# zju3dv/street_gaussians

Measured on AMD Instinct MI355X. Metric: train iters/s (fwd+bwd) @1M Gaussians 1920x1280 SH3, higher is better.
Workload: dtype f32

## Files before the change

### include/sgr.h

```cpp
#ifndef SGR_H_INCLUDED
#define SGR_H_INCLUDED

#include <stddef.h>
#include <stdint.h>

#ifdef __cplusplus
extern "C" {
#endif

#define SGR_E_INVALID 1
#define SGR_E_HIP 2
#define SGR_E_ALLOC 3
#define SGR_E_PREFILTER 4
#define SGR_E_LAZY 5

typedef char* (*sgr_alloc_fn)(size_t nbytes, void* user);

const char* sgr_last_error(void);
int sgr_version(void);

int sgr_forward(sgr_alloc_fn geometry_buffer, void* geometry_user, sgr_alloc_fn binning_buffer, void* binning_user,
                sgr_alloc_fn image_buffer, void* image_user, int P, int D, int M, int S, const float* background,
                int width, int height, const float* means3D, const float* shs, const float* colors_precomp,
                const float* semantics, const float* opacities, const float* scales, float scale_modifier,
                const float* rotations, const float* cov3D_precomp, const float* viewmatrix, const float* projmatrix,
                const float* cam_pos, float tan_fovx, float tan_fovy, int prefiltered, float* out_color,
                float* out_depth, float* out_alpha, float* out_semantic, int* radii, int debug, void* stream);

typedef struct sgr_forward_extras {
    int color_jacobian;
} sgr_forward_extras;
int sgr_forward_ex(sgr_alloc_fn geometry_buffer, void* geometry_user, sgr_alloc_fn binning_buffer, void* binning_user,
                   sgr_alloc_fn image_buffer, void* image_user, int P, int D, int M, int S, const float* background,
                   int width, int height, const float* means3D, const float* shs, const float* colors_precomp,
                   const float* semantics, const float* opacities, const float* scales, float scale_modifier,
                   const float* rotations, const float* cov3D_precomp, const float* viewmatrix, const float* projmatrix,
                   const float* cam_pos, float tan_fovx, float tan_fovy, int prefiltered, float* out_color,
                   float* out_depth, float* out_alpha, float* out_semantic, int* radii, int debug, void* stream,
                   const sgr_forward_extras* extras);

int sgr_backward(int P, int D, int M, int R, int S, const float* background, int width, int height,
                 const float* means3D, const float* shs, const float* colors_precomp, const float* semantics,
                 const float* alphas, const float* scales, float scale_modifier, const float* rotations,
                 const float* cov3D_precomp, const float* viewmatrix, const float* projmatrix, const float* campos,
                 float tan_fovx, float tan_fovy, const int* radii, char* geom_buffer, char* binning_buffer,
                 char* image_buffer, const float* dL_dpix, const float* dL_dpix_depth, const float* dL_dalphas,
                 const float* dL_dpix_semantic, float* dL_dmean2D, float* dL_dopacity, float* dL_dcolor,
                 float* dL_dmean3D, float* dL_dcov3D, float* dL_dsh, float* dL_dscale, float* dL_drot,
                 float* dL_dsemantic, sgr_alloc_fn scratch, void* scratch_user, int debug, void* stream);

#define SGR_MAX_STAT_SEGMENTS 128
typedef struct sgr_stat_segment {
    int src_start;
    int count;
    int dst_offset;
} sgr_stat_segment;
typedef struct sgr_backward_extras {
    float* xyz_gradient_accum;
    float* denom;
    float* max_radii2D;
    const sgr_stat_segment* segments;
    int n_segments;
    void* color_ready_event;
    int rows;
    float* masked_color_out;
    int skip_sh_grad;
    int skip_cov3d_grad;
} sgr_backward_extras;
int sgr_backward_ex(int P, int D, int M, int R, int S, const float* background, int width, int height,
                    const float* means3D, const float* shs, const float* colors_precomp, const float* semantics,
                    const float* alphas, const float* scales, float scale_modifier, const float* rotations,
                    const float* cov3D_precomp, const float* viewmatrix, const float* projmatrix, const float* campos,
                    float tan_fovx, float tan_fovy, const int* radii, char* geom_buffer, char* binning_buffer,
                    char* image_buffer, const float* dL_dpix, const float* dL_dpix_depth, const float* dL_dalphas,
                    const float* dL_dpix_semantic, float* dL_dmean2D, float* dL_dopacity, float* dL_dcolor,
                    float* dL_dmean3D, float* dL_dcov3D, float* dL_dsh, float* dL_dscale, float* dL_drot,
                    float* dL_dsemantic, sgr_alloc_fn scratch, void* scratch_user, int debug, void* stream,
                    const sgr_backward_extras* extras);

int sgr_masked_color_grad(int P, const char* geom_buffer, const float* dL_dcolor, float* dL_drgb, void* stream);
int sgr_sh_grad_from_views(int P, int D, int M, int V, const float* means3D, const float* campos, const float* dL_drgb,
                           float* dL_dsh, void* stream);
int sgr_sh_grad_from_views_ex(int P, int D, int M, int V, const float* means3D, size_t means_view_stride,
                              const float* campos, size_t campos_view_stride, const float* dL_drgb,
                              size_t drgb_view_stride, float* dL_dsh, void* stream);

int sgr_mark_visible(int P, const float* means3D, const float* viewmatrix, const float* projmatrix, uint8_t* present,
                     void* stream);

int sgr_visible_filter(int P, int width, int height, const float* means3D, const float* scales, float scale_modifier,
                       const float* rotations, const float* cov3D_precomp, const float* viewmatrix,
                       const float* projmatrix, float tan_fovx, float tan_fovy, int prefiltered, int* radii,
                       float* means2D, int debug, void* stream);

int sgr_knn(int P, const float* points, float* meanDists, sgr_alloc_fn scratch, void* scratch_user, void* stream);

size_t sgr_geometry_bytes(int P);
size_t sgr_binning_bytes(int R);
size_t sgr_image_bytes(int width, int height);
int sgr_partial_row_floats(int S);
size_t sgr_geometry_jac_offset(int P);

int sgr_profile_enable(int on);
int sgr_profile_read(double* sum_ms, int* counts);
int sgr_profile_select(int stage_mask);
int sgr_profile_sample(int every);

int sgr_export_internal(int which, int P, int R, int width, int height, char* geom_buffer, char* binning_buffer,
                        char* image_buffer, void* dst, void* stream);
int sgr_export_cov3d(int P, const float* scales, float scale_modifier, const float* rotations, float* dst, void* stream);

enum {
    SGR_SW_NO_CULL = 1 << 0,
    SGR_SW_NO_DPP = 1 << 1,
    SGR_SW_NO_DET = 1 << 2,
    SGR_SW_NO_HITS = 1 << 3,
    SGR_SW_USE_V2 = 1 << 4,
    SGR_SW_USE_ONESWEEP = 1 << 5,
    SGR_SW_PRE_STAGE_SH = 1 << 6,
    SGR_SW_EXACT = 1 << 7,
    SGR_SW_USE_SW = 1 << 8,
    SGR_SW_USE_RS_WAVE = 1 << 9,
    SGR_SW_REF_RECT = 1 << 10,
    SGR_SW_NO_TILE_MASK = 1 << 11,
    SGR_SW_TILE_SORT = 1 << 12,
    SGR_SW_REF_RECT_PLAIN = 1 << 13,
    SGR_SW_LPT = 1 << 14,
    SGR_SW_NO_LPT = 1 << 15,
    SGR_SW_NO_HLIST = 1 << 16,
    SGR_SW_HLIST_ALWAYS = 1 << 17,
    SGR_SW_KEY32 = 1 << 18
};
int sgr_test_switches(int mask);
int sgr_has_variants(void);
int sgr_set_lazy(int on);
int sgr_lazy_status(int* num_rendered, int* capacity, int* flags);

int sgr_profile_host_wait_us(int reset);

int sgr_test_scan(const uint32_t* in, uint32_t* out, size_t n, int inclusive, uint32_t* tmp, void* stream);
int sgr_test_sort(uint64_t* keys0, uint64_t* keys1, uint32_t* vals0, uint32_t* vals1, uint32_t n, int end_bit,
                  uint32_t* hist, uint32_t* scan_tmp, void* stream);
int sgr_test_sort32(uint32_t* keys0, uint32_t* keys1, uint32_t* vals0, uint32_t* vals1, uint32_t n, int end_bit,
                    int max_bits, uint32_t* hist, uint32_t* scan_tmp, void* stream);
size_t sgr_test_sort_hist_words(uint32_t n);
size_t sgr_test_scan_tmp_words(size_t n);
int sgr_test_wave_sum(const float* in, float* out_dpp, float* out_shfl, int nwaves, void* stream);
int sgr_test_lds_atomic_order(const uint32_t* pattern, uint32_t* out, int trials, void* stream);
int sgr_test_exact_math(int n, const float* x, float* exp_lib, float* exp_ref, const float* a, const float* b,
                        float* div_lib, float* div_ref, void* stream);

#ifdef __cplusplus
}
#endif
#endif
```

### street_gaussians_amd/_native.py

```python
from __future__ import annotations

import ctypes as C
import os

import torch

from . import _alloc

_HERE = os.path.dirname(os.path.abspath(__file__))
LIB_PATH = os.environ.get("SGR_LIB") or os.path.join(_HERE, "libsgr_hip.so")

ALLOC_FN = C.CFUNCTYPE(C.c_void_p, C.c_size_t, C.c_void_p)

_lib = None


def _signatures():
    vp, f, d, i, u32, i64, sz = C.c_void_p, C.c_float, C.c_double, C.c_int, C.c_uint32, C.c_int64, C.c_size_t
    i64p = C.POINTER(C.c_int64)
    bwd = [i, i, i, i, i, vp, i, i, vp, vp, vp, vp, vp, vp, f, vp, vp, vp, vp, vp, f, f, vp, vp, vp, vp, vp, vp, vp, vp,
           vp, vp, vp, vp, vp, vp, vp, vp, vp, ALLOC_FN, vp, i, vp]
    fwd = [ALLOC_FN, vp, ALLOC_FN, vp, ALLOC_FN, vp, i, i, i, i, vp, i, i, vp, vp, vp, vp, vp, vp, f, vp, vp, vp, vp, vp, f, f, i,
           vp, vp, vp, vp, vp, i, vp]
    return {
        "sgr_last_error": (C.c_char_p, []),
        "sgr_version": (i, []),
        "sgr_forward": (i, fwd),
        "sgr_forward_ex": (i, fwd + [vp]),
        "sgr_forward_layers": (i, fwd + [vp]),
        "sgr_layer_alpha_forward": (i, [i, i, i, i, i, vp, vp, vp, vp, vp, vp]),
        "sgr_layer_alpha_backward": (i, [i, i, i, i, i, vp, vp, f, vp, vp, vp] + [vp] * 11 + [ALLOC_FN, vp, i, vp]),
        "sgr_backward": (i, bwd),
        "sgr_backward_ex": (i, bwd + [vp]),
        "sgr_mark_visible": (i, [i, vp, vp, vp, vp, vp]),
        "sgr_visible_filter": (i, [i, i, i, vp, vp, f, vp, vp, vp, vp, f, f, i, vp, vp, i, vp]),
        "sgr_knn": (i, [i, vp, vp, ALLOC_FN, vp, vp]),
        "sgr_geometry_bytes": (sz, [i]),
        "sgr_binning_bytes": (sz, [i]),
        "sgr_image_bytes": (sz, [i, i]),
        "sgr_partial_row_floats": (i, [i]),
        "sgr_geometry_jac_offset": (sz, [i]),
        "sgr_export_internal": (i, [i, i, i, i, i, vp, vp, vp, vp, vp]),
        "sgr_export_cov3d": (i, [i, vp, f, vp, vp, vp]),
        "sgr_test_scan": (i, [vp, vp, sz, i, vp, vp]),
        "sgr_test_sort": (i, [vp, vp, vp, vp, u32, i, vp, vp, vp]),
        "sgr_test_sort32": (i, [vp, vp, vp, vp, u32, i, i, vp, vp, vp]),
        "sgr_test_sort_hist_words": (sz, [u32]),
        "sgr_test_scan_tmp_words": (sz, [sz]),
        "sgr_test_wave_sum": (i, [vp, vp, vp, i, vp]),
        "sgr_test_exact_math": (i, [i, vp, vp, vp, vp, vp, vp, vp, vp]),
        "sgr_test_lds_atomic_order": (i, [vp, vp, i, vp]),
        "sgr_test_switches": (i, [i]),
        "sgr_has_variants": (i, []),
        "sgr_set_lazy": (i, [i]),
        "sgr_lazy_status": (i, [vp, vp, vp]),
        "sgr_profile_host_wait_us": (i, [i]),
        "sgr_profile_enable": (i, [i]),
        "sgr_profile_select": (i, [i]),
        "sgr_profile_sample": (i, [i]),
        "sgr_profile_read": (i, [vp, vp]),
        "sgr_masked_color_grad": (i, [i, vp, vp, vp, vp]),
        "sgr_sh_grad_from_views": (i, [i, i, i, i, vp, vp, vp, vp, vp]),
        "sgr_sh_grad_from_views_ex": (i, [i, i, i, i, vp, sz, vp, sz, vp, sz, vp, vp]),
        "sgr_scene_compose_forward": (i, [i, vp, i, i, vp, vp, vp, vp, vp, vp, ALLOC_FN, vp, vp]),
        "sgr_scene_compose_backward": (i, [i, vp, vp, i, i, vp, vp, vp, vp, vp, vp, ALLOC_FN, vp, vp]),
        "sgr_scene_compose_forward_ex": (i, [i, vp, i, i, vp, vp, vp, vp, vp, vp, vp, ALLOC_FN, vp, vp]),
        "sgr_scene_compose_backward_ex": (i, [i, vp, vp, i, i, vp, vp, vp, vp, vp, vp, vp, ALLOC_FN, vp, vp]),
        "sgr_scene_compose_backward_step": (i, [i, vp, vp, vp, i, i, vp, vp, vp, vp, vp, vp, vp, d, d, f, ALLOC_FN, vp, vp]),
        "sgr_scene_densification_stats": (i, [i, vp, vp, vp, ALLOC_FN, vp, vp]),
        "sgr_ssim_workspace_floats": (sz, [i, i, i]),
        "sgr_ssim_forward": (i, [i, i, i, vp, vp, vp, vp, vp, vp, vp]),
        "sgr_ssim_backward": (i, [i, i, i, vp, vp, vp, vp, vp, vp, vp]),
        "sgr_l1_workspace_floats": (sz, [i, i, i]),
        "sgr_l1_forward": (i, [i, i, i, vp, vp, vp, vp, vp, vp]),
        "sgr_l1_backward": (i, [i, i, i, vp, vp, vp, vp, vp, vp, vp]),
        "sgr_color_loss_backward": (i, [i, i, i, vp, vp, vp, vp, vp, f, f, vp, vp, vp]),
        "sgr_bce_forward": (i, [i, i, vp, vp, vp, vp, vp]),
        "sgr_bce_backward": (i, [i, i, vp, vp, vp, vp, vp]),
        "sgr_lidar_work_bytes": (sz, [i]),
        "sgr_lidar_depth_forward": (i, [i, vp, vp, vp, vp, d, vp, vp, vp]),
        "sgr_lidar_depth_backward": (i, [i, vp, vp, vp, vp, vp, vp, vp, vp, vp]),
        "sgr_frame_loss_saved_bytes": (sz, [i, i, i]),
        "sgr_frame_loss_workspace_floats": (sz, [i, i, i]),
        "sgr_frame_loss_finish_span": (i, []),
        "sgr_frame_loss_forward": (i, [i, i, i, vp, vp, vp, vp, vp]),
        "sgr_frame_loss_backward": (i, [i, i, i] + [vp] * 10),
        "sgr_mse_workspace_floats": (sz, [i, i, i]),
        "sgr_mse_forward": (i, [i, i, i, vp, vp, vp, vp, vp, vp]),
        "sgr_densify_work_bytes": (sz, [i]),
        "sgr_densify_plan": (i, [i, vp, vp, vp, vp, vp, vp, i64p, vp]),
        "sgr_densify_map": (i, [i, vp, vp, vp, vp, vp, vp]),
        "sgr_densify_gather": (i, [i, i, vp, vp, vp, i, vp, vp]),
        "sgr_densify_split_children": (i, [i, i, vp, vp, vp, vp, vp, vp, vp, vp, vp, vp]),
        "sgr_densify_prune_mask": (i, [i, vp, i, vp, vp, vp, vp, vp, vp, vp, vp, i64p, vp]),
        "sgr_densify_compact": (i, [i, vp, vp, vp, i64p, vp]),
        "sgr_reset_opacity": (i, [i, vp, vp, vp, vp]),
        "sgr_densify_scene_work_bytes": (sz, [i, i]),
        "sgr_densify_scene_plan": (i, [i, i] + [vp] * 7 + [i64p, vp]),
        "sgr_densify_scene_layout": (i, [i, vp, i64p, i64p]),
        "sgr_densify_scene_map": (i, [i, i] + [vp] * 7),
        "sgr_densify_scene_prune": (i, [i, i] + [vp] * 14 + [i64p, vp]),
        "sgr_densify_scene_gather_ragged": (i, [i, vp, vp, i64p, vp, i, vp, vp, vp, i, vp, vp]),
        "sgr_texture_cube_workspace_bytes": (sz, [i, i, i, i, i64]),
        "sgr_texture_cube_forward": (i, [i, i, i, i, i64, vp, vp, vp, vp]),
        "sgr_texture_cube_backward": (i, [i, i, i, i, i64, vp, vp, vp, vp, vp]),
        "sgr_adam_span_elems": (i, []),
        "sgr_adam_max_blocks": (i, []),
        "sgr_adam_max_records": (i, []),
        "sgr_adam_step": (i, [vp, i, vp, i, i64, d, d, vp]),
        "sgr_sky_workspace_bytes": (sz, [i, i, i, i, i]),
        "sgr_sky_forward": (i, [i, i, i, i] + [vp] * 9 + [i, vp, vp, vp]),
        "sgr_sky_backward": (i, [i, i, i, i, vp, vp, vp, vp, i, vp, vp, vp, vp, vp, vp, vp]),
        "sgr_sky_step_block_texels": (i, []),
        "sgr_sky_step_workspace_bytes": (sz, [i, i, i]),
        "sgr_sky_backward_deferred": (i, [i, i, i, i, vp, vp, vp, vp, i, vp, vp, vp, vp, vp, vp, vp, vp]),
        "sgr_sky_adam_step": (i, [i, vp, vp, vp, vp, vp, f, f, f, d, d, vp]),
        "sgr_sky_test_rays": (i, [i, i, vp, vp, vp, vp, i, vp, vp, vp]),
        "sgr_actor_pose_forward": (i, [i, vp, i] + [vp] * 7 + [vp]),
        "sgr_actor_pose_backward_max_blocks": (i, []),
        "sgr_actor_pose_backward": (i, [i, vp, i] + [vp] * 9 + [vp]),
        "sgr_test_sort32_count": (i, [vp, vp, vp, vp, u32, i, i, vp, vp, vp, vp]),
    }


SIGNATURES = _signatures()
SYMBOLS = list(SIGNATURES)


class SgrError(RuntimeError):
    pass


class SgrLazyError(SgrError):
    """-SGR_E_LAZY (lazy mode, sgr_set_lazy): the PREVIOUS lazy forward of this thread was invalid (list capacity overflow,
    prefilter violation, a depth beyond the narrow depth sort) -- ITS outputs and the gradients computed from them must be
    discarded (redo that step; do not apply its optimiser update).  The call that raised this rendered nothing; the thread's
    next forward is a blocking one that re-seeds the capacity.  Check ``_C.lazy_status()`` after a synchronisation and BEFORE
    applying gradients when a one-step-late report is not acceptable."""


SGR_E_LAZY = 5


def lib():
    global _lib
    if _lib is None:
        if not os.path.exists(LIB_PATH):
            raise SgrError(f"{LIB_PATH} not found: build it with `python -m street_gaussians_amd.build` "
                           "(there is no CPU fallback)")
        L = C.CDLL(LIB_PATH)
        for name, (restype, argtypes) in SIGNATURES.items():
            fn = getattr(L, name)
            fn.restype, fn.argtypes = restype, argtypes
        _lib = L
    return _lib


def check(rc: int) -> int:
    if rc < 0:
        raise (SgrLazyError if rc == -SGR_E_LAZY else SgrError)(lib().sgr_last_error().decode())
    return rc


def stream(device) -> C.c_void_p:
    return C.c_void_p(torch.cuda.current_stream(device).cuda_stream)


def ptr(t):
    return None if t is None else C.c_void_p(t.data_ptr())


def launch(name: str, stream_, *args) -> int:
    return check(getattr(lib(), name)(*[ptr(a) if isinstance(a, torch.Tensor) else a for a in args], stream_))


def call(name: str, device, *args) -> int:
    with torch.cuda.device(device):
        return launch(name, stream(device), *args)


def require_hip(message: str, *tensors) -> None:
    if not all(t.is_cuda for t in tensors):
        raise SgrError(message)


class Grow:

    def __init__(self, device):
        holder = [torch.empty(0, dtype=torch.uint8, device=device)]

        def alloc(nbytes, _user, holder=holder, device=device):
            holder[0] = torch.empty(_alloc.ladder(int(nbytes)), dtype=torch.uint8, device=device)
            return holder[0].data_ptr()

        self._holder = holder
        self.cb = ALLOC_FN(alloc)

    @property
    def tensor(self):
        return self._holder[0]
```

### street_gaussians_amd/csrc/sgr_api.hip

```cpp
#include <cstdio>
#include <cstdlib>
#include <cstring>
#include <algorithm>
#include <atomic>
#include <chrono>
#include <mutex>
#include <string>
#include <thread>

#include "../../include/sgr.h"
#include "../../include/sgr_layers.h"
#include "../../include/sgr_object_alpha.h"
#include "sgr_launch.h"

static thread_local std::string g_err;

static bool env_flag(const char* name) {
    const char* v = getenv(name);
    return v && v[0] && v[0] != '0';
}

static std::atomic<int> g_switches{-1};
#ifndef SGR_WITH_VARIANTS
#define SGR_WITH_VARIANTS 0
#endif
#define SGR_VARIANT_BITS (SGR_SW_USE_V2 | SGR_SW_USE_ONESWEEP | SGR_SW_USE_SW | SGR_SW_USE_RS_WAVE)
static int switches() {
    int v = g_switches.load(std::memory_order_relaxed);
    if (v < 0) {
        static const struct { int bit; const char* names[2]; } env[] = {
            {SGR_SW_NO_CULL, {"SGR_NO_CULL"}}, {SGR_SW_NO_DPP, {"SGR_NO_DPP"}}, {SGR_SW_NO_DET, {"SGR_NO_DET"}},
            {SGR_SW_NO_HITS, {"SGR_NO_HITS"}}, {SGR_SW_USE_V2, {"SGR_V2"}}, {SGR_SW_PRE_STAGE_SH, {"SGR_PRE_STAGE"}},
            {SGR_SW_EXACT, {"SGR_EXACT"}}, {SGR_SW_USE_SW, {"SGR_SW", "SGR_SW8"}},
            {SGR_SW_USE_RS_WAVE, {"SGR_RS_WAVE", "SGR_SW9"}}, {SGR_SW_REF_RECT, {"SGR_REF_RECT"}},
            {SGR_SW_NO_TILE_MASK, {"SGR_NO_TILE_MASK"}}, {SGR_SW_TILE_SORT, {"SGR_TILE_SORT"}},
            {SGR_SW_REF_RECT_PLAIN, {"SGR_REF_RECT_PLAIN"}}, {SGR_SW_LPT, {"SGR_LPT"}}, {SGR_SW_NO_LPT, {"SGR_NO_LPT"}},
            {SGR_SW_NO_HLIST, {"SGR_NO_HLIST"}}, {SGR_SW_HLIST_ALWAYS, {"SGR_HLIST_ALWAYS"}}, {SGR_SW_KEY32, {"SGR_KEY32"}},
        };
        v = 0;
        for (const auto& e : env)
            for (const char* name : e.names)
                if (name && env_flag(name)) v |= e.bit;
        if (!SGR_WITH_VARIANTS) v &= ~SGR_VARIANT_BITS;
        g_switches.store(v, std::memory_order_relaxed);
    }
    return v;
}

#define SGR_PROF_STAGES 9
#define SGR_PROF_SLOTS 1024
struct SgrProf {
    std::atomic<bool> on{false};
    std::atomic<int> mask{(1 << SGR_PROF_STAGES) - 1};
    std::atomic<int> n{0};
    std::atomic<int> every{1};
    std::atomic<unsigned> seen[SGR_PROF_STAGES];
    hipEvent_t ev[SGR_PROF_SLOTS][2];
    int stage[SGR_PROF_SLOTS];
    bool created = false;
};
static SgrProf g_prof;
static thread_local int t_prof_slot = -1;
static void prof_begin(int stage, hipStream_t s) {
    t_prof_slot = -1;
    if (!g_prof.on.load(std::memory_order_relaxed)) return;
    if (!((g_prof.mask.load(std::memory_order_relaxed) >> stage) & 1)) return;
    const int every = g_prof.every.load(std::memory_order_relaxed);
    if (every > 1 && g_prof.seen[stage].fetch_add(1u, std::memory_order_relaxed) % (unsigned)every != 0) return;
    const int i = g_prof.n.fetch_add(1, std::memory_order_relaxed);
    if (i >= SGR_PROF_SLOTS) return;
    g_prof.stage[i] = stage;
    (void)hipEventRecord(g_prof.ev[i][0], s);
    t_prof_slot = i;
}
static void prof_end(hipStream_t s) {
    if (t_prof_slot < 0) return;
    (void)hipEventRecord(g_prof.ev[t_prof_slot][1], s);
    t_prof_slot = -1;
}

static int fail(int code, const std::string& msg) {
    g_err = msg;
    return -code;
}
int sgr_set_error(int code, const std::string& msg) { return fail(code, msg); }

#define SGR_STAGE(name)                                                                                   \
    do {                                                                                                  \
        if (debug && env_flag("SGR_TRACE")) { fprintf(stderr, "[sgr] stage %s launched\n", name); fflush(stderr); } \
        hipError_t e__ = hipGetLastError();                                                               \
        if (e__ == hipSuccess && debug) e__ = hipStreamSynchronize(stream);                               \
        if (e__ != hipSuccess) return fail(SGR_E_HIP, std::string("stage ") + name + ": " + hipGetErrorString(e__)); \
    } while (0)

static uint32_t* pinned_pair(int slot = 0) {
    static thread_local uint32_t* p[2] = {nullptr, nullptr};
    if (!p[slot] && hipHostMalloc((void**)&p[slot], 64, hipHostMallocPortable | hipHostMallocCoherent) != hipSuccess) p[slot] = nullptr;
    return p[slot];
}
static hipEvent_t readback_event(int slot = 0) {
    static thread_local hipEvent_t ev[2][64] = {};
    int dev = 0;
    if (hipGetDevice(&dev) != hipSuccess || dev < 0 || dev >= 64) return nullptr;
    if (!ev[slot][dev] && hipEventCreateWithFlags(&ev[slot][dev], hipEventDisableTiming) != hipSuccess) ev[slot][dev] = nullptr;
    return ev[slot][dev];
}

#define SGR_READBACK_PENDING 0xffffffffu
static std::atomic<unsigned long long> g_wait_ns{0};
static hipError_t wait_for_readback_(uint32_t* host_vals, hipEvent_t landed);
static hipError_t wait_for_readback(uint32_t* host_vals, hipEvent_t landed) {
    const auto t0 = std::chrono::steady_clock::now();
    const hipError_t e = wait_for_readback_(host_vals, landed);
    g_wait_ns.fetch_add((unsigned long long)std::chrono::duration_cast<std::chrono::nanoseconds>(std::chrono::steady_clock::now() - t0).count(),
                        std::memory_order_relaxed);
    return e;
}
static hipError_t wait_for_readback_(uint32_t* host_vals, hipEvent_t landed) {
    static const long spin_us = [] { const char* e = getenv("SGR_SPIN_US"); return e ? atol(e) : 2000L; }();
    if (spin_us > 0) {
        volatile uint32_t* hv = host_vals;
        const auto t0 = std::chrono::steady_clock::now();
        for (;;) {
            for (int i = 0; i < 256; i++) {
                if (hv[0] != SGR_READBACK_PENDING && hv[2] != SGR_READBACK_PENDING && hv[4] != SGR_READBACK_PENDING &&
                    hv[5] != SGR_READBACK_PENDING) {
                    std::atomic_thread_fence(std::memory_order_acquire);
                    return hipSuccess;
                }
#if defined(__x86_64__) || defined(__i386__)
                __builtin_ia32_pause();
#else
                std::this_thread::yield();
#endif
            }
            if (std::chrono::duration_cast<std::chrono::microseconds>(std::chrono::steady_clock::now() - t0).count() > spin_us)
                break;
        }
    }
    return hipEventSynchronize(landed);
}

static int depth9_max_p() {
    static const int v = [] { const char* e = getenv("SGR_DEPTH9_MAX_P"); return e ? atoi(e) : 750000; }();
    return v;
}
static int pre_stage_min_p() {
    static const int v = [] { const char* e = getenv("SGR_PRE_STAGE_MIN_P"); return e ? atoi(e) : 3000000; }();
    return v;
}

static std::atomic<int> g_lazy{-1};
static std::atomic<int> g_lazy_epoch{0};
static bool lazy_on() {
    int v = g_lazy.load(std::memory_order_relaxed);
    if (v < 0) {
        v = env_flag("SGR_LAZY") ? 1 : 0;
        g_lazy.store(v, std::memory_order_relaxed);
    }
    return v != 0;
}
struct ThreadState {
    int wide_left = 0;
    size_t r_hint = 0;
    int epoch = 0;
    bool pending = false;
    uint32_t cap = 0;
    uint32_t* host_vals = nullptr;
    hipEvent_t landed = nullptr;
    bool wide = false;
    int lazy_flags() const {
        return (host_vals[4] > cap ? 1 : 0) | ((host_vals[0] & 1u) ? 2 : 0) | (((host_vals[2] & 1u) && !wide) ? 4 : 0);
    }
};
static thread_local ThreadState t_state;

struct Switches {
    bool cull, dpp, det;
    bool use_hits;
    bool exact;
    bool v2, quad, rs_wave;
    int rect_mode;
    bool hit_list;
    bool hlist_walk;
    bool lazy_mode;
    bool tile_sort;
    bool lpt, lpt_force;
    bool pre_stage_forced, key32;
    bool pre_stage(int P) const { return pre_stage_forced || P >= pre_stage_min_p(); }
    int key16(size_t T) const { return (T < 65535u && !key32) ? 1 : 0; }
};
static Switches resolve_switches() {
    const int m = switches();
    const auto on = [m](int bits) { return (m & bits) != 0; };
    Switches s;
    s.cull = !on(SGR_SW_NO_CULL); s.dpp = !on(SGR_SW_NO_DPP); s.det = !on(SGR_SW_NO_DET); s.use_hits = !on(SGR_SW_NO_HITS);
    s.exact = on(SGR_SW_EXACT); s.v2 = on(SGR_SW_USE_V2); s.rs_wave = on(SGR_SW_USE_RS_WAVE);
    s.quad = SGR_WITH_VARIANTS && on(SGR_SW_USE_SW) &&
             !on(SGR_SW_NO_CULL | SGR_SW_NO_DPP | SGR_SW_NO_DET | SGR_SW_NO_HITS | SGR_SW_USE_V2);
    s.rect_mode = on(SGR_SW_REF_RECT) ? (on(SGR_SW_REF_RECT_PLAIN) ? 0 : 3) : (on(SGR_SW_NO_TILE_MASK) ? 1 : 2);
    s.hlist_walk = SGR_HLIST && !on(SGR_SW_NO_HLIST);
    s.hit_list = s.hlist_walk && on(SGR_SW_REF_RECT | SGR_SW_HLIST_ALWAYS);
    s.lazy_mode = lazy_on();
    s.tile_sort = on(SGR_SW_TILE_SORT) && !s.lazy_mode;
    s.lpt = !on(SGR_SW_NO_LPT); s.lpt_force = on(SGR_SW_LPT);
    s.pre_stage_forced = on(SGR_SW_PRE_STAGE_SH); s.key32 = on(SGR_SW_KEY32);
    return s;
}

static uint32_t getHigherMsb(uint32_t n) {
    uint32_t msb = sizeof(n) * 4;
    uint32_t step = msb;
    while (step > 1) {
        step /= 2;
        if (n >> msb) msb += step;
        else msb -= step;
    }
    if (n >> msb) msb++;
    return msb;
}

static uint32_t binning_ladder(size_t r) {
    size_t step = 1;
    while ((step << 1) <= r) step <<= 1;
    step = std::max<size_t>(step >> 4, 1024);
    return (uint32_t)std::min<size_t>((r + step - 1) / step * step, 0x7fffffffu);
}

struct TileGrid {
    int W, H, gx, gy;
    size_t N, T;
    bool too_large() const { return gx > SGR_MAX_GRID_DIM || gy > SGR_MAX_GRID_DIM; }
};
static TileGrid tile_grid(int W, int H) {
    const int gx = (W + SGR_BLOCK_X - 1) / SGR_BLOCK_X, gy = (H + SGR_BLOCK_Y - 1) / SGR_BLOCK_Y;
    return {W, H, gx, gy, (size_t)W * H, (size_t)gx * gy};
}

struct Frame {
    TileGrid g;
    SgrGeomView gv;
    SgrImgView iv;
    SgrBinView bv;
    const int* radii;
    int key16;
    int pair;
    const void* keys;
    const uint32_t* list;
    SgrTileLists tiles(bool frame_order) const { return {g.gx, frame_order ? -g.gy : g.gy, g.W, g.H, iv.ranges, list, gv.rec}; }
};
static Frame make_frame(int P, int R, int W, int H, char* geom, char* binning, char* image, const int* radii, const Switches& sw,
                        bool carve_empty_list = false) {
    Frame f = {};
    f.g = tile_grid(W, H);
    f.gv = sgr_geom_carve(geom, (size_t)P);
    f.iv = sgr_img_carve(image, f.g.N, f.g.T);
    f.radii = radii ? radii : f.gv.internal_radii;
    f.key16 = sw.key16(f.g.T);
    if (R > 0 || carve_empty_list) {
        f.bv = sgr_bin_carve(binning, (size_t)R);
        f.pair = R > 0 ? (sgr_sort_pass_count((int)getHigherMsb((uint32_t)f.g.T)) & 1) : 0;
        f.keys = f.bv.keys[f.pair];
        f.list = f.bv.vals[f.pair ^ (sw.tile_sort ? 1 : 0)];
    }
    return f;
}

struct BwdScratch { float4* cd; float* partials; char* extra; };
static bool bwd_scratch(sgr_alloc_fn scratch, void* user, int P, size_t rows, int stride, size_t extra_bytes, BwdScratch& out) {
    const size_t cd_bytes = sgr_align_up((size_t)P * sizeof(float4), 256);
    const size_t row_bytes = sgr_align_up(rows * stride * sizeof(float), 256);
    char* base = scratch(cd_bytes + row_bytes + extra_bytes, user);
    out = {reinterpret_cast<float4*>(base), reinterpret_cast<float*>(base + cd_bytes), base + cd_bytes + row_bytes};
    return base != nullptr;
}
static int clear_touched(const Frame& f, int R, bool odd_set, hipStream_t stream) {
    uint8_t* const touched = f.bv.touched;
    if (R > 0 && odd_set) SGR_HIP(hipMemsetAsync(touched, 0, (size_t)R, stream));
    return 0;
}
__global__ void __launch_bounds__(256)
sgr_pack_camera_kernel(SgrCam* cam, const float* view, const float* proj, const float* campos, float tan_fovx,
                       float tan_fovy, float focal_x, float focal_y, int W, int H, int gx, int gy, float scale_modifier,
                       uint32_t* header, uint2* ranges, int T, uint32_t rect_mode) {
    const int t = threadIdx.x;
    for (int i = blockIdx.x * 256 + t; i < T; i += gridDim.x * 256) ranges[i] = make_uint2(0u, 0u);
    if (blockIdx.x != 0) return;
    if (t < 16) {
        header[t] = t == 6 ? (rect_mode & 0xffu) : (t == 7 ? ((rect_mode >> 8) & 1u) : (t == SGR_HDR_JAC ? ((rect_mode >> 9) & 1u) : 0u));
        cam->view[t] = view[t];
        cam->proj[t] = proj ? proj[t] : 0.f;
    }
    if (t < 3) cam->campos[t] = campos ? campos[t] : 0.f;
    if (t == 0) {
        reinterpret_cast<uint32_t*>(ranges + T)[T] = 0u;
        cam->tan_fovx = tan_fovx; cam->tan_fovy = tan_fovy;
        cam->focal_x = focal_x; cam->focal_y = focal_y;
        cam->W = W; cam->H = H; cam->gx = gx; cam->gy = gy;
        cam->scale_modifier = scale_modifier;
    }
}

static SgrCam* cam_slot(const SgrGeomView& gv) { return reinterpret_cast<SgrCam*>(gv.header + 16); }
static_assert(sizeof(SgrCam) <= 48 * 4, "SgrCam must fit the geometry header");
static_assert(SGR_STAT_SEG_MAX == SGR_MAX_STAT_SEGMENTS, "sgr_common.h and include/sgr.h disagree");

static void pack_camera(const SgrGeomView& gv, const float* view, const float* proj, const float* campos,
                        float tan_fovx, float tan_fovy, int W, int H, float scale_modifier, uint2* ranges,
                        const TileGrid& g, const Switches& sw, bool jac, hipStream_t s) {
    const float focal_y = H / (2.0f * tan_fovy);
    const float focal_x = W / (2.0f * tan_fovx);
    const int T = (int)g.T, nb = std::max(1, std::min(64, (T + 255) / 256));
    sgr_pack_camera_kernel<<<nb, 256, 0, s>>>(cam_slot(gv), view, proj, campos, tan_fovx, tan_fovy, focal_x, focal_y, W, H,
                                             g.gx, g.gy, scale_modifier, gv.header, ranges, T,
                                             (uint32_t)sw.rect_mode | (sw.hit_list ? 0x100u : 0u) | (jac ? 0x200u : 0u));
}

static int gauss_bwd(const Switches& sw, SgrGaussBwdArgs& a, const Frame& f, hipStream_t stream) {
    a.cam = cam_slot(f.gv);
    a.gv = f.gv; a.radii = f.radii; a.W = f.g.W; a.H = f.g.H;
    a.exact = sw.exact ? 1 : 0; a.rs_wave = sw.rs_wave ? 1 : 0;
    return (sw.exact ? sgr_launch_gauss_bwd_strict : sgr_launch_gauss_bwd)(a, stream);
}

SgrFlagBlock sgr_acquire_flag_block() {
    static std::mutex mu;
    static uint32_t* blk[64] = {};
    SgrFlagBlock b;
    b.lock = std::unique_lock<std::mutex>(mu);
    int dev = 0;
    if (hipGetDevice(&dev) != hipSuccess || dev < 0 || dev >= 64) return b;
    if (!blk[dev] && hipMalloc((void**)&blk[dev], 256) != hipSuccess) blk[dev] = nullptr;
    b.ptr = blk[dev];
    return b;
}

extern "C" {

const char* sgr_last_error(void) { return g_err.c_str(); }
int sgr_version(void) { return 105; }

size_t sgr_geometry_bytes(int P) {
    return sgr_required([&](char* b, char** e) { sgr_geom_carve(b, (size_t)P, e); });
}
size_t sgr_binning_bytes(int R) {
    return sgr_required([&](char* b, char** e) { sgr_bin_carve(b, (size_t)R, e); });
}
size_t sgr_image_bytes(int width, int height) {
    const TileGrid g = tile_grid(width, height);
    return sgr_required([&](char* b, char** e) { sgr_img_carve(b, g.N, g.T, e); });
}
int sgr_partial_row_floats(int S) { return sgr_partial_row_stride(S); }
size_t sgr_geometry_jac_offset(int P) {
    char* base = (char*)4096;
    return (size_t)((char*)sgr_geom_carve(base, (size_t)P).jac - base);
}

static int queue_readback(int slot, const SgrGeomView& gv, bool watched, hipStream_t stream, uint32_t*& host_vals, hipEvent_t& landed) {
    host_vals = pinned_pair(slot);
    landed = readback_event(slot);
    if (!host_vals || !landed) return fail(SGR_E_HIP, "pinned readback slot / event creation failed");
    if (watched) host_vals[0] = host_vals[2] = host_vals[4] = host_vals[5] = SGR_READBACK_PENDING;
    SGR_HIP(hipMemcpyAsync(host_vals, gv.header, 6 * sizeof(uint32_t), hipMemcpyDeviceToHost, stream));
    if (watched) SGR_HIP(hipEventRecord(landed, stream));
    return 0;
}

static int forward_impl(sgr_alloc_fn geometry_buffer, void* geometry_user, sgr_alloc_fn binning_buffer, void* binning_user,
                        sgr_alloc_fn image_buffer, void* image_user, int P, int D, int M, int S, const float* background,
                        int width, int height, const float* means3D, const float* shs, const float* colors_precomp,
                        const float* semantics, const float* opacities, const float* scales, float scale_modifier,
                        const float* rotations, const float* cov3D_precomp, const float* viewmatrix, const float* projmatrix,
                        const float* cam_pos, float tan_fovx, float tan_fovy, int prefiltered, float* out_color,
                        float* out_depth, float* out_alpha, float* out_semantic, int* radii, int debug, void* stream_,
                        const sgr_layer_images* layers, const sgr_forward_extras* fx) {
    hipStream_t stream = (hipStream_t)stream_;
    const Switches sw = resolve_switches();
    const bool want_jac = fx && fx->color_jacobian && shs != nullptr && colors_precomp == nullptr;
    const int W = width, H = height;
    if (P < 0 || W <= 0 || H <= 0) return fail(SGR_E_INVALID, "P, width and height must be positive");
    const TileGrid g = tile_grid(W, H);
    if (g.too_large()) return fail(SGR_E_INVALID, "image larger than 16368 px per side is not supported");
    if (S < 0 || S > SGR_SEM_MAX) return fail(SGR_E_INVALID, "semantic channels must be in [0, 32]");
    if (D < 0 || D > 3) return fail(SGR_E_INVALID, "SH degree must be in [0, 3]");
    const size_t N = g.N, T = g.T;

    if (P == 0) {
        SGR_HIP(hipMemsetAsync(out_color, 0, 3 * N * sizeof(float), stream));
        SGR_HIP(hipMemsetAsync(out_depth, 0, N * sizeof(float), stream));
        SGR_HIP(hipMemsetAsync(out_alpha, 0, N * sizeof(float), stream));
        if (S) SGR_HIP(hipMemsetAsync(out_semantic, 0, (size_t)S * N * sizeof(float), stream));
        if (layers) {
            sgr_launch_layers_fill(W, H, layers->background, layers->clamp, layers->color, layers->alpha, stream);
            SGR_STAGE("layers_fill");
        }
        return 0;
    }
    if (!means3D || !opacities || !viewmatrix || !projmatrix || !background)
        return fail(SGR_E_INVALID, "means3D, opacities, viewmatrix, projmatrix and background are required");
    if ((shs == nullptr) == (colors_precomp == nullptr))
        return fail(SGR_E_INVALID, "provide exactly one of shs / colors_precomp");
    if (((scales == nullptr) || (rotations == nullptr)) == (cov3D_precomp == nullptr))
        return fail(SGR_E_INVALID, "provide exactly one of scales+rotations / cov3D_precomp");
    if (shs && (!cam_pos || M < (D + 1) * (D + 1))) return fail(SGR_E_INVALID, "shs need campos and M >= (D+1)^2");
    if (S > 0 && !semantics) return fail(SGR_E_INVALID, "S > 0 but semantics is NULL");

    char* gbase = geometry_buffer(sgr_geometry_bytes(P), geometry_user);
    if (!gbase) return fail(SGR_E_ALLOC, "geometry buffer allocation failed");
    const SgrGeomView gv = sgr_geom_carve(gbase, (size_t)P);
    char* ibase = image_buffer(sgr_image_bytes(W, H), image_user);
    if (!ibase) return fail(SGR_E_ALLOC, "image buffer allocation failed");
    uint2* const ranges = sgr_img_carve(ibase, N, T).ranges;
    int* radii_ptr = radii ? radii : gv.internal_radii;

    ThreadState& ts = t_state;
    bool wide_depth = ts.wide_left > 0;
    if (wide_depth) ts.wide_left--;
    uint32_t* host_vals = nullptr;
    hipEvent_t landed = nullptr;
    const uint32_t* order = nullptr;
    char* bbase = nullptr;

    hipStreamCaptureStatus cap_status = hipStreamCaptureStatusNone;
    (void)hipStreamIsCapturing(stream, &cap_status);
    const bool capturing = cap_status != hipStreamCaptureStatusNone;
    if (ts.pending) {
        ts.pending = false;
        SGR_HIP(wait_for_readback(ts.host_vals, ts.landed));
        const int fl = ts.lazy_flags();
        if (ts.host_vals[2] & 1u) ts.wide_left = 64;
        if (fl) {
            ts.r_hint = 0;
            return fail(SGR_E_LAZY, std::string("the PREVIOUS lazy forward of this thread was invalid (") +
                        ((fl & 1) ? "more tile instances than the list capacity; " : "") +
                        ((fl & 2) ? "a Gaussian failed the frustum test although prefiltered is set; " : "") +
                        ((fl & 4) ? "a view depth beyond the 27-bit depth keys; " : "") + "its outputs must be discarded)");
        }
        const size_t Rp = ts.host_vals[4];
        ts.r_hint = std::max(Rp + Rp / 16 + 1024, ts.r_hint - ts.r_hint / 64);
    }
    if (const int e = g_lazy_epoch.load(std::memory_order_relaxed); ts.epoch != e) {
        ts.epoch = e;
        ts.r_hint = 0;
    }
    const bool lazy = sw.lazy_mode && ts.r_hint > 0;
    const int aux16 = sw.rect_mode == 3 ? 1 : 0;
    const uint2* aux_emit = aux16 ? reinterpret_cast<const uint2*>(gv.aux_ref) : gv.aux;

    const auto preprocess = [&]() -> int {
        prof_begin(0, stream);
        pack_camera(gv, viewmatrix, projmatrix, cam_pos, tan_fovx, tan_fovy, W, H, scale_modifier, ranges, g, sw, want_jac, stream);
        SGR_STAGE("pack_camera");
        sgr_launch_preprocess(P, D, M, means3D, scales, rotations, opacities, shs, cov3D_precomp, colors_precomp,
                              cam_slot(gv), gv, radii_ptr, prefiltered, sw.pre_stage(P), sw.rect_mode, want_jac, stream);
        SGR_STAGE("preprocess");
        prof_end(stream);
        return 0;
    };
    const auto depth_sort_scan = [&]() -> int {
        prof_begin(1, stream);
        order = nullptr;
        const uint2* scanned = aux_emit;
        if (!sw.tile_sort) {
            const int dcur = sgr_launch_sort_pairs32(gv.dkeys, gv.dvals, (uint32_t)P, wide_depth ? 32 : SGR_DEPTH_KEY_BITS, gv.dhist,
                                                     gv.scan_tmp, stream, true, aux_emit, gv.aux_sorted, P < depth9_max_p() ? 9 : 8, aux16);
            order = gv.dvals[dcur];
            scanned = gv.aux_sorted;
        }
        sgr_launch_scan_head(reinterpret_cast<const uint32_t*>(scanned), reinterpret_cast<const uint32_t*>(gv.aux), (size_t)P,
                             aux16 ? 4 : 2, gv.scan_tmp, gv.sub_sums, stream, 2);
        SGR_STAGE("depth_sort+scan");
        prof_end(stream);
        return 0;
    };

    int R = 0;
    uint32_t cap = 0;
    if (lazy) {
        if (const int rc = preprocess()) return rc;
        if (const int rc = queue_readback(1, gv, !capturing, stream, host_vals, landed)) return rc;
        ts.pending = !capturing;
        ts.host_vals = host_vals;
        ts.landed = landed;
        ts.wide = wide_depth;
        ts.cap = 0x7fffffffu;
        if (const int rc = depth_sort_scan()) return rc;
        cap = binning_ladder(ts.r_hint);
        bbase = binning_buffer(sgr_binning_bytes((int)cap), binning_user);
        if (!bbase) return fail(SGR_E_ALLOC, "binning buffer allocation failed");
        R = (int)cap;
        ts.cap = cap;
    } else {
        size_t have_bytes = 0;
        for (int attempt = 0; attempt < 2; attempt++) {
            if (const int rc = preprocess()) return rc;
            if (const int rc = queue_readback(0, gv, true, stream, host_vals, landed)) return rc;
            struct ReadbackDrain {
                hipEvent_t ev;
                ~ReadbackDrain() { if (ev) (void)hipEventSynchronize(ev); }
            } drain{landed};
            if (const int rc = depth_sort_scan()) return rc;
            have_bytes = 0;
            bbase = nullptr;
            if (ts.r_hint > 0) {
                have_bytes = sgr_binning_bytes((int)binning_ladder(ts.r_hint));
                bbase = binning_buffer(have_bytes, binning_user);
                if (!bbase) return fail(SGR_E_ALLOC, "binning buffer allocation failed");
            }
            SGR_HIP(wait_for_readback(host_vals, landed));
            drain.ev = nullptr;

            if (!(host_vals[2] & 1u) || wide_depth || sw.tile_sort) break;
            wide_depth = true;
            ts.wide_left = 64;
        }
        if (host_vals[0] & 1u)
            return fail(SGR_E_PREFILTER, "Point is filtered although prefiltered is set. This shouldn't happen!");
        if (host_vals[4] > 0x7fffffffu) return fail(SGR_E_INVALID, "more than 2^31 tile instances");
        R = (int)host_vals[4];

        if (!bbase || sgr_binning_bytes(R) > have_bytes) {
            bbase = binning_buffer(sgr_binning_bytes(R), binning_user);
            if (!bbase) return fail(SGR_E_ALLOC, "binning buffer allocation failed");
        }
        ts.r_hint = std::max((size_t)R + (size_t)R / 4 + 1024, ts.r_hint - ts.r_hint / 16);
    }
    const Frame f = make_frame(P, R, W, H, gbase, bbase, ibase, radii, sw, true);
    const SgrBinView& bv = f.bv;
    prof_begin(2, stream);
    SgrGeomView gv_dup = gv;
    if (sw.tile_sort) gv_dup.aux_sorted = const_cast<uint2*>(aux_emit);
    sgr_launch_duplicate(P, gv_dup, order, gv.scan_tmp, gv.sub_sums, bv.keys[0], f.key16, bv.vals[0], g.gx, cap, aux16, stream);
    SGR_STAGE("duplicate");
    prof_end(stream);
    if (R > 0) {
        prof_begin(3, stream);
        const int bit = (int)getHigherMsb((uint32_t)T);
        if (f.key16) {
            uint16_t* const k16[2] = {reinterpret_cast<uint16_t*>(bv.keys[0]), reinterpret_cast<uint16_t*>(bv.keys[1])};
            sgr_launch_sort_pairs16(k16, bv.vals, (uint32_t)R, bit, bv.hist, bv.scan_tmp, stream);
        } else {
            sgr_launch_sort_pairs32(bv.keys, bv.vals, (uint32_t)R, bit, bv.hist, bv.scan_tmp, stream);
        }
        SGR_STAGE("sort");
        prof_end(stream);
        prof_begin(4, stream);
        sgr_launch_tile_ranges(R, f.keys, f.key16, f.iv.ranges, bv.touched, lazy ? (uint32_t)T : 0xffffffffu, stream);
        SGR_STAGE("tile_ranges");
        if (sw.tile_sort) {
            sgr_launch_tile_sort((int)T, f.iv.ranges, bv.vals[f.pair], bv.vals[f.pair ^ 1], gv.dkeys[0], gv.header, bv.keys[f.pair ^ 1], bv.tkeys, stream);
            SGR_STAGE("tile_sort");
        }
        prof_end(stream);
    }
    const SgrTileLists tl = f.tiles(sw.lpt);
    prof_begin(5, stream);
    if (sw.lpt) {
        sgr_launch_tile_order(f.iv.ranges, (int)T, sw.lpt_force ? 1 : 0, stream);
        SGR_STAGE("tile_order");
    }
    sgr_launch_blend_fwd(sw.cull, sw.exact, tl, S, semantics, background, out_color, out_depth, out_alpha, out_semantic,
                         f.iv.n_contrib, bv.hit4, sw.hit_list ? bv.hlist : nullptr, f.iv.n_contrib_k, stream);
    SGR_STAGE("blend_fwd");
    prof_end(stream);
    if (layers) {
        sgr_launch_blend_layers(sw.exact, tl, layers->split, P, layers->background, layers->clamp, layers->color, layers->alpha, stream);
        SGR_STAGE("blend_layers");
    }
    return R;
}

#define SGR_FORWARD_ARGS                                 \
    geometry_buffer, geometry_user, binning_buffer, binning_user, image_buffer, image_user, P, D, M, S, background, width, height, \
        means3D, shs, colors_precomp, semantics, opacities, scales, scale_modifier, rotations, cov3D_precomp, viewmatrix,        \
        projmatrix, cam_pos, tan_fovx, tan_fovy, prefiltered, out_color, out_depth, out_alpha, out_semantic, radii, debug, stream_
int sgr_forward(sgr_alloc_fn geometry_buffer, void* geometry_user, sgr_alloc_fn binning_buffer, void* binning_user,
                sgr_alloc_fn image_buffer, void* image_user, int P, int D, int M, int S, const float* background,
                int width, int height, const float* means3D, const float* shs, const float* colors_precomp,
                const float* semantics, const float* opacities, const float* scales, float scale_modifier,
                const float* rotations, const float* cov3D_precomp, const float* viewmatrix, const float* projmatrix,
                const float* cam_pos, float tan_fovx, float tan_fovy, int prefiltered, float* out_color,
                float* out_depth, float* out_alpha, float* out_semantic, int* radii, int debug, void* stream_) {
    return sgr_forward_ex(SGR_FORWARD_ARGS, nullptr);
}

int sgr_forward_ex(sgr_alloc_fn geometry_buffer, void* geometry_user, sgr_alloc_fn binning_buffer, void* binning_user,
                   sgr_alloc_fn image_buffer, void* image_user, int P, int D, int M, int S, const float* background,
                   int width, int height, const float* means3D, const float* shs, const float* colors_precomp,
                   const float* semantics, const float* opacities, const float* scales, float scale_modifier,
                   const float* rotations, const float* cov3D_precomp, const float* viewmatrix, const float* projmatrix,
                   const float* cam_pos, float tan_fovx, float tan_fovy, int prefiltered, float* out_color,
                   float* out_depth, float* out_alpha, float* out_semantic, int* radii, int debug, void* stream_,
                   const sgr_forward_extras* extras) {
    return forward_impl(SGR_FORWARD_ARGS, nullptr, extras);
}

int sgr_forward_layers(sgr_alloc_fn geometry_buffer, void* geometry_user, sgr_alloc_fn binning_buffer, void* binning_user,
                       sgr_alloc_fn image_buffer, void* image_user, int P, int D, int M, int S, const float* background,
                       int width, int height, const float* means3D, const float* shs, const float* colors_precomp,
                       const float* semantics, const float* opacities, const float* scales, float scale_modifier,
                       const float* rotations, const float* cov3D_precomp, const float* viewmatrix, const float* projmatrix,
                       const float* cam_pos, float tan_fovx, float tan_fovy, int prefiltered, float* out_color,
                       float* out_depth, float* out_alpha, float* out_semantic, int* radii, int debug, void* stream_,
                       const sgr_layer_images* layers) {
    if (layers) {
        if (layers->split < 0 || layers->split > P) return fail(SGR_E_INVALID, "layers: split must lie in [0, P]");
        if (!layers->background) return fail(SGR_E_INVALID, "layers: background is NULL");
        for (int l = 0; l < 2; l++) {
            if (!layers->color[l]) return fail(SGR_E_INVALID, "layers: color[" + std::to_string(l) + "] is NULL");
            if (!layers->alpha[l]) return fail(SGR_E_INVALID, "layers: alpha[" + std::to_string(l) + "] is NULL");
        }
    }
    return forward_impl(SGR_FORWARD_ARGS, layers, nullptr);
}
#undef SGR_FORWARD_ARGS

int sgr_backward(int P, int D, int M, int R, int S, const float* background, int width, int height,
                 const float* means3D, const float* shs, const float* colors_precomp, const float* semantics,
                 const float* alphas, const float* scales, float scale_modifier, const float* rotations,
                 const float* cov3D_precomp, const float* viewmatrix, const float* projmatrix, const float* campos,
                 float tan_fovx, float tan_fovy, const int* radii, char* geom_buffer, char* binning_buffer,
                 char* image_buffer, const float* dL_dpix, const float* dL_dpix_depth, const float* dL_dalphas,
                 const float* dL_dpix_semantic, float* dL_dmean2D, float* dL_dopacity, float* dL_dcolor,
                 float* dL_dmean3D, float* dL_dcov3D, float* dL_dsh, float* dL_dscale, float* dL_drot,
                 float* dL_dsemantic, sgr_alloc_fn scratch, void* scratch_user, int debug, void* stream_) {
    return sgr_backward_ex(P, D, M, R, S, background, width, height, means3D, shs, colors_precomp, semantics, alphas, scales,
                           scale_modifier, rotations, cov3D_precomp, viewmatrix, projmatrix, campos, tan_fovx, tan_fovy,
                           radii, geom_buffer, binning_buffer, image_buffer, dL_dpix, dL_dpix_depth, dL_dalphas,
                           dL_dpix_semantic, dL_dmean2D, dL_dopacity, dL_dcolor, dL_dmean3D, dL_dcov3D, dL_dsh, dL_dscale,
                           dL_drot, dL_dsemantic, scratch, scratch_user, debug, stream_, nullptr);
}

int sgr_backward_ex(int P, int D, int M, int R, int S, const float* background, int width, int height,
                    const float* means3D, const float* shs, const float* colors_precomp, const float* semantics,
                    const float* alphas, const float* scales, float scale_modifier, const float* rotations,
                    const float* cov3D_precomp, const float* viewmatrix, const float* projmatrix, const float* campos,
                    float tan_fovx, float tan_fovy, const int* radii, char* geom_buffer, char* binning_buffer,
                    char* image_buffer, const float* dL_dpix, const float* dL_dpix_depth, const float* dL_dalphas,
                    const float* dL_dpix_semantic, float* dL_dmean2D, float* dL_dopacity, float* dL_dcolor,
                    float* dL_dmean3D, float* dL_dcov3D, float* dL_dsh, float* dL_dscale, float* dL_drot,
                    float* dL_dsemantic, sgr_alloc_fn scratch, void* scratch_user, int debug, void* stream_,
                    const sgr_backward_extras* extras) {
    hipStream_t stream = (hipStream_t)stream_;
    const Switches sw = resolve_switches();
    SgrGaussBwdArgs ga;
    SgrStatSink& sink = ga.sink;
    if (extras && (extras->xyz_gradient_accum || extras->denom || extras->max_radii2D)) {
        if (!extras->xyz_gradient_accum || !extras->denom || !extras->max_radii2D)
            return fail(SGR_E_INVALID, "the statistics sink needs xyz_gradient_accum, denom and max_radii2D together");
        sink.accum = extras->xyz_gradient_accum;
        sink.denom = extras->denom;
        sink.max_radii = extras->max_radii2D;
        if (extras->segments != nullptr) {
            const int n = extras->n_segments;
            if (n < 0 || n > SGR_STAT_SEG_MAX)
                return fail(SGR_E_INVALID, "statistics sink: at most 128 segments per call");
            int end = 0;
            for (int i = 0; i < n; i++) {
                const sgr_stat_segment& sg = extras->segments[i];
                if (sg.src_start < end || sg.count < 0 || sg.dst_offset < 0 || (long)sg.src_start + sg.count > (long)P)
                    return fail(SGR_E_INVALID, "statistics sink: segments must be sorted, non-overlapping and inside [0, P)");
                end = sg.src_start + sg.count;
                sink.start[i] = sg.src_start;
                sink.count[i] = sg.count;
                sink.shift[i] = sg.dst_offset - sg.src_start;
            }
            for (int i = 0; i < n; i++) {
                const sgr_stat_segment& a = extras->segments[i];
                if (extras->rows > 0 && (long)a.dst_offset + a.count > (long)extras->rows)
                    return fail(SGR_E_INVALID, "statistics sink: a segment's destination lies outside the persistent arrays");
                for (int j = 0; j < i; j++) {
                    const sgr_stat_segment& b = extras->segments[j];
                    if (a.count > 0 && b.count > 0 && a.dst_offset < b.dst_offset + b.count && b.dst_offset < a.dst_offset + a.count)
                        return fail(SGR_E_INVALID, "statistics sink: two segments write the same persistent rows");
                }
            }
            sink.nseg = n;
            if (n == 0) sink.accum = sink.denom = sink.max_radii = nullptr;
        }
    }
    (void)colors_precomp; (void)scale_modifier; (void)viewmatrix; (void)projmatrix; (void)campos;
    (void)tan_fovx; (void)tan_fovy;
    if (P <= 0) return 0;
    const int W = width, H = height;
    if (S < 0 || S > SGR_SEM_MAX) return fail(SGR_E_INVALID, "semantic channels must be in [0, 32]");
    if (!geom_buffer || !image_buffer || (R > 0 && !binning_buffer))
        return fail(SGR_E_INVALID, "backward needs the buffers produced by forward");
    if (!means3D || !background || !alphas || !dL_dpix || !dL_dpix_depth || !dL_dalphas)
        return fail(SGR_E_INVALID, "means3D, background, alphas, dL_dpix, dL_dpix_depth and dL_dalphas are required");
    if (S > 0 && (!semantics || !dL_dpix_semantic || !dL_dsemantic))
        return fail(SGR_E_INVALID, "S > 0 needs semantics, dL_dpix_semantic and dL_dsemantic");
    const int skip_sh = (extras && extras->skip_sh_grad) ? 1 : 0;
    const int skip_cov = (extras && extras->skip_cov3d_grad) ? 1 : 0;
    if (!dL_dmean2D || !dL_dopacity || !dL_dcolor || !dL_dmean3D || (!dL_dcov3D && !skip_cov) || !dL_dscale || !dL_drot)
        return fail(SGR_E_INVALID, "all gradient outputs except dL_dsh / dL_dsemantic are required");
    if (shs && !dL_dsh && !skip_sh) return fail(SGR_E_INVALID, "shs given but dL_dsh is NULL");
    const Frame f = make_frame(P, R, W, H, geom_buffer, binning_buffer, image_buffer, radii, sw);
    const int stride = sgr_partial_row_stride(S);
    const bool quad = sw.quad && S == 0 && R > 0;
    BwdScratch sc;
    if (!bwd_scratch(scratch, scratch_user, P, (size_t)R * (quad ? 4u : 1u), stride, 0, sc))
        return fail(SGR_E_ALLOC, "backward scratch allocation failed");
    const bool odd_set = !sw.cull || !sw.use_hits || quad;
    if (R > 0) {
        prof_begin(6, stream);
        if (const int rc = clear_touched(f, R, odd_set, stream)) return rc;
        prof_end(stream);
        prof_begin(7, stream);
        SgrBlendBwdArgs ba;
        ba.cull = sw.cull; ba.dpp = sw.dpp; ba.det = sw.det; ba.v2 = sw.v2; ba.exact = sw.exact;
        ba.S = S; ba.bg = background; ba.u0 = f.gv.u0; ba.tmask = f.gv.tmask; ba.semantics = semantics; ba.alphas = alphas;
        ba.n_contrib = f.iv.n_contrib;
        ba.hit4 = sw.use_hits ? f.bv.hit4 : nullptr;
        ba.dL_dpix = dL_dpix; ba.dL_ddepth = dL_dpix_depth; ba.dL_dalpha = dL_dalphas; ba.dL_dsem = dL_dpix_semantic;
        ba.partials = sc.partials; ba.touched = f.bv.touched; ba.row_limit = (uint32_t)R;
        ba.hlist = sw.hlist_walk ? f.bv.hlist : nullptr; ba.n_contrib_k = f.iv.n_contrib_k; ba.hl_flag = f.gv.header + 7;
#if SGR_WITH_VARIANTS
        if (quad) sgr_launch_blend_bwd_sw(f.tiles(false), ba, stride, stream);
        else
#endif
            sgr_launch_blend_bwd(f.tiles(true), ba, stream);
        SGR_STAGE("blend_bwd");
        prof_end(stream);
    }
    prof_begin(8, stream);
    ga.P = P; ga.D = D; ga.M = M; ga.S = S;
    ga.means3D = means3D; ga.shs = shs; ga.scales = scales; ga.rotations = rotations; ga.cov3D_precomp = cov3D_precomp;
    ga.partials = sc.partials; ga.row_stride = stride; ga.touched = f.bv.touched; ga.cd = sc.cd;
    ga.dL_dmean2D = dL_dmean2D; ga.dL_dopacity = dL_dopacity; ga.dL_dcolor = dL_dcolor; ga.dL_dmean3D = dL_dmean3D;
    ga.dL_dcov3D = dL_dcov3D; ga.dL_dsh = dL_dsh; ga.dL_dscale = dL_dscale; ga.dL_drot = dL_drot; ga.dL_dsemantic = dL_dsemantic;
    ga.quad = quad ? 1 : 0; ga.row_limit = (uint32_t)R; ga.skip_sh = skip_sh; ga.skip_cov = skip_cov;
    if (extras) { ga.after_rows = (hipEvent_t)extras->color_ready_event; ga.masked_color_out = extras->masked_color_out; }
    const int ev_failed = gauss_bwd(sw, ga, f, stream);
    SGR_STAGE("gauss_bwd");
    prof_end(stream);
    if (ev_failed) return fail(SGR_E_HIP, "hipEventRecord(color_ready_event) failed: is it a valid event of this device?");
    return clear_touched(f, R, odd_set, stream);
}

static int layer_alpha_check(int P, int R, int width, int height, int split, const void* geom, const void* binning,
                             const void* image) {
    if (P < 0 || R < 0 || width <= 0 || height <= 0) return fail(SGR_E_INVALID, "layer alpha: P, R must not be negative, width and height positive");
    if (split < 0 || split > P) return fail(SGR_E_INVALID, "layer alpha: split must lie in [0, P]");
    if (tile_grid(width, height).too_large()) return fail(SGR_E_INVALID, "layer alpha: image larger than 16368 px per side is not supported");
    if (P > 0 && (!geom || !image || (R > 0 && !binning)))
        return fail(SGR_E_INVALID, "layer alpha: the buffers produced by sgr_forward are required");
    return 0;
}

int sgr_layer_alpha_forward(int P, int R, int width, int height, int split, const char* geom_buffer,
                            const char* binning_buffer, const char* image_buffer, float* out_alpha, uint32_t* out_last,
                            void* stream_) {
    hipStream_t stream = (hipStream_t)stream_;
    const int debug = 0;
    if (const int rc = layer_alpha_check(P, R, width, height, split, geom_buffer, binning_buffer, image_buffer)) return rc;
    if (!out_alpha || !out_last) return fail(SGR_E_INVALID, "layer alpha: out_alpha and out_last are required");
    const Switches sw = resolve_switches();
    const size_t N = tile_grid(width, height).N;
    if (P == 0 || split == P || R == 0) {
        SGR_HIP(hipMemsetAsync(out_alpha, 0, N * sizeof(float), stream));
        SGR_HIP(hipMemsetAsync(out_last, 0, N * sizeof(uint32_t), stream));
        return 0;
    }
    const Frame f = make_frame(P, R, width, height, const_cast<char*>(geom_buffer), const_cast<char*>(binning_buffer),
                               const_cast<char*>(image_buffer), nullptr, sw);
    sgr_launch_object_alpha_fwd(sw.exact, f.tiles(true), split, out_alpha, out_last, stream);
    SGR_STAGE("object_alpha_fwd");
    return 0;
}

int sgr_layer_alpha_backward(int P, int R, int width, int height, int split, const float* means3D, const float* scales,
                             float scale_modifier, const float* rotations, const float* cov3D_precomp, const int* radii,
                             char* geom_buffer, char* binning_buffer, char* image_buffer, const float* layer_alpha,
                             const uint32_t* layer_last, const float* dL_dlayer_alpha, float* dL_dmean3D,
                             float* dL_dopacity, float* dL_dscale, float* dL_drot, float* dL_dcov3D, sgr_alloc_fn scratch,
                             void* scratch_user, int debug, void* stream_) {
    hipStream_t stream = (hipStream_t)stream_;
    (void)scale_modifier;
    if (const int rc = layer_alpha_check(P, R, width, height, split, geom_buffer, binning_buffer, image_buffer)) return rc;
    if (P == 0) return 0;
    if (!means3D || !layer_alpha || !layer_last || !dL_dlayer_alpha)
        return fail(SGR_E_INVALID, "layer alpha: means3D, layer_alpha, layer_last and dL_dlayer_alpha are required");
    if (((scales == nullptr) || (rotations == nullptr)) == (cov3D_precomp == nullptr))
        return fail(SGR_E_INVALID, "layer alpha: provide exactly one of scales+rotations / cov3D_precomp");
    if (!dL_dmean3D || !dL_dopacity || !dL_dscale || !dL_drot)
        return fail(SGR_E_INVALID, "layer alpha: dL_dmean3D, dL_dopacity, dL_dscale and dL_drot are required");
    if (!scratch) return fail(SGR_E_INVALID, "layer alpha: the scratch callback is required");
    const Switches sw = resolve_switches();
    const Frame f = make_frame(P, R, width, height, geom_buffer, binning_buffer, image_buffer, radii, sw);
    const int stride = sgr_partial_row_stride(0);
    const size_t p3_bytes = sgr_align_up((size_t)P * 3 * sizeof(float), 256);
    BwdScratch sc;
    if (!bwd_scratch(scratch, scratch_user, P, (size_t)R, stride, 2 * p3_bytes, sc))
        return fail(SGR_E_ALLOC, "layer alpha: backward scratch allocation failed");
    if (const int rc = clear_touched(f, R, true, stream)) return rc;
    if (R > 0 && split < P) {
        sgr_launch_object_alpha_bwd(sw.exact, f.tiles(true), f.gv.u0, f.gv.tmask, split, layer_alpha, layer_last, dL_dlayer_alpha,
                                    sc.partials, stride, f.bv.touched, (uint32_t)R, stream);
        SGR_STAGE("object_alpha_bwd");
    }
    SgrGaussBwdArgs ga;
    ga.P = P; ga.means3D = means3D; ga.scales = scales; ga.rotations = rotations; ga.cov3D_precomp = cov3D_precomp;
    ga.partials = sc.partials; ga.row_stride = stride; ga.touched = f.bv.touched; ga.cd = sc.cd;
    ga.dL_dmean2D = reinterpret_cast<float*>(sc.extra); ga.dL_dcolor = reinterpret_cast<float*>(sc.extra + p3_bytes);
    ga.dL_dopacity = dL_dopacity; ga.dL_dmean3D = dL_dmean3D; ga.dL_dcov3D = dL_dcov3D; ga.dL_dscale = dL_dscale; ga.dL_drot = dL_drot;
    ga.row_limit = (uint32_t)R; ga.skip_sh = 1; ga.skip_cov = dL_dcov3D ? 0 : 1;
    gauss_bwd(sw, ga, f, stream);
    SGR_STAGE("object_alpha gauss_bwd");
    return clear_touched(f, R, true, stream);
}

int sgr_masked_color_grad(int P, const char* geom_buffer, const float* dL_dcolor, float* dL_drgb, void* stream_) {
    hipStream_t stream = (hipStream_t)stream_;
    const int debug = 0;
    if (P <= 0) return 0;
    if (!geom_buffer || !dL_dcolor || !dL_drgb) return fail(SGR_E_INVALID, "geom_buffer, dL_dcolor and dL_drgb are required");
    const SgrGeomView gv = sgr_geom_carve(const_cast<char*>(geom_buffer), (size_t)P);
    sgr_launch_masked_color_grad(P, gv.clamped, dL_dcolor, dL_drgb, stream);
    SGR_STAGE("masked_color_grad");
    return 0;
}

int sgr_sh_grad_from_views(int P, int D, int M, int V, const float* means3D, const float* campos, const float* dL_drgb,
                           float* dL_dsh, void* stream_) {
    hipStream_t stream = (hipStream_t)stream_;
    const int debug = 0;
    if (P <= 0) return 0;
    if (D < 0 || D > 3 || M < (D + 1) * (D + 1) || V < 0) return fail(SGR_E_INVALID, "need 0 <= D <= 3, M >= (D+1)^2, V >= 0");
    if (!means3D || !campos || !dL_drgb || !dL_dsh) return fail(SGR_E_INVALID, "means3D, campos, dL_drgb and dL_dsh are required");
    sgr_launch_sh_grad_from_views(P, D, M, V, means3D, 0, campos, 3, dL_drgb, (size_t)3 * P, dL_dsh, stream);
    SGR_STAGE("sh_grad_from_views");
    return 0;
}

int sgr_sh_grad_from_views_ex(int P, int D, int M, int V, const float* means3D, size_t means_view_stride,
                              const float* campos, size_t campos_view_stride, const float* dL_drgb,
                              size_t drgb_view_stride, float* dL_dsh, void* stream_) {
    hipStream_t stream = (hipStream_t)stream_;
    const int debug = 0;
    if (P <= 0) return 0;
    if (D < 0 || D > 3 || M < (D + 1) * (D + 1) || V < 0) return fail(SGR_E_INVALID, "need 0 <= D <= 3, M >= (D+1)^2, V >= 0");
    if (!means3D || !campos || !dL_drgb || !dL_dsh) return fail(SGR_E_INVALID, "means3D, campos, dL_drgb and dL_dsh are required");
    sgr_launch_sh_grad_from_views(P, D, M, V, means3D, means_view_stride, campos, campos_view_stride, dL_drgb,
                                  drgb_view_stride, dL_dsh, stream);
    SGR_STAGE("sh_grad_from_views_ex");
    return 0;
}

int sgr_set_lazy(int on) {
    const int prev = lazy_on() ? 1 : 0;
    if (on >= 0) {
        g_lazy.store(on ? 1 : 0, std::memory_order_relaxed);
        g_lazy_epoch.fetch_add(1, std::memory_order_relaxed);
    }
    return prev;
}

int sgr_lazy_status(int* num_rendered, int* capacity, int* flags) {
    const ThreadState& ts = t_state;
    if (!ts.host_vals || ts.cap == 0) return fail(SGR_E_INVALID, "no lazy forward has run on this thread");
    if (num_rendered) *num_rendered = (int)ts.host_vals[4];
    if (capacity) *capacity = (int)ts.cap;
    if (flags) *flags = ts.lazy_flags();
    return 0;
}

int sgr_profile_host_wait_us(int reset) {
    const unsigned long long ns = reset ? g_wait_ns.exchange(0, std::memory_order_relaxed) : g_wait_ns.load(std::memory_order_relaxed);
    return (int)std::min<unsigned long long>(ns / 1000ull, 0x7fffffffull);
}

int sgr_has_variants(void) { return SGR_WITH_VARIANTS ? 1 : 0; }

int sgr_test_switches(int mask) {
    const int prev = switches() | ((SGR_WITH_VARIANTS && sgr_sort_get_one_sweep()) ? SGR_SW_USE_ONESWEEP : 0);
    if (mask >= 0) {
        if (!SGR_WITH_VARIANTS) mask &= ~SGR_VARIANT_BITS;
        g_switches.store(mask & ~SGR_SW_USE_ONESWEEP, std::memory_order_relaxed);
        sgr_sort_set_one_sweep((mask & SGR_SW_USE_ONESWEEP) != 0);
    }
    return prev;
}

int sgr_profile_enable(int on) {
    if (on && !g_prof.created) {
        for (int i = 0; i < SGR_PROF_SLOTS; i++)
            for (int k = 0; k < 2; k++)
                if (hipEventCreate(&g_prof.ev[i][k]) != hipSuccess) return fail(SGR_E_HIP, "hipEventCreate failed");
        for (int i = 0; i < SGR_PROF_SLOTS; i++)
            for (int k = 0; k < 2; k++) (void)hipEventRecord(g_prof.ev[i][k], nullptr);
        (void)hipDeviceSynchronize();
        g_prof.created = true;
    }
    g_prof.n.store(0);
    g_prof.on.store(on != 0);
    return 0;
}

int sgr_profile_sample(int every) {
    const int prev = g_prof.every.load();
    if (every >= 1) {
        g_prof.every.store(every);
        for (int i = 0; i < SGR_PROF_STAGES; i++) g_prof.seen[i].store(0u);
    }
    return prev;
}

int sgr_profile_select(int stage_mask) {
    const int prev = g_prof.mask.load();
    if (stage_mask >= 0) g_prof.mask.store(stage_mask & ((1 << SGR_PROF_STAGES) - 1));
    return prev;
}

int sgr_profile_read(double* sum_ms, int* counts) {
    for (int i = 0; i < SGR_PROF_STAGES; i++) { sum_ms[i] = 0.0; counts[i] = 0; }
    if (!g_prof.created) return 0;
    SGR_HIP(hipDeviceSynchronize());
    const int n = std::min(g_prof.n.load(), SGR_PROF_SLOTS);
    for (int i = 0; i < n; i++) {
        float ms = 0.f;
        if (hipEventElapsedTime(&ms, g_prof.ev[i][0], g_prof.ev[i][1]) != hipSuccess) continue;
        sum_ms[g_prof.stage[i]] += ms;
        counts[g_prof.stage[i]]++;
    }
    g_prof.n.store(0);
    return n;
}

int sgr_mark_visible(int P, const float* means3D, const float* viewmatrix, const float* projmatrix, uint8_t* present,
                     void* stream_) {
    hipStream_t stream = (hipStream_t)stream_;
    const int debug = 0;
    (void)projmatrix;
    if (P <= 0) return 0;
    if (!means3D || !viewmatrix || !present) return fail(SGR_E_INVALID, "means3D, viewmatrix and present are required");
    sgr_launch_mark_visible(P, means3D, viewmatrix, present, stream);
    SGR_STAGE("mark_visible");
    return 0;
}

int sgr_visible_filter(int P, int width, int height, const float* means3D, const float* scales, float scale_modifier,
                       const float* rotations, const float* cov3D_precomp, const float* viewmatrix,
                       const float* projmatrix, float tan_fovx, float tan_fovy, int prefiltered, int* radii,
                       float* means2D, int debug, void* stream_) {
    hipStream_t stream = (hipStream_t)stream_;
    if (P <= 0) return 0;
    const int W = width, H = height;
    const TileGrid g = tile_grid(W, H);
    if (g.too_large()) return fail(SGR_E_INVALID, "image too large");
    if (!means3D || !viewmatrix || !projmatrix || !radii || !means2D)
        return fail(SGR_E_INVALID, "means3D, viewmatrix, projmatrix, radii and means2D are required");
    if (((scales == nullptr) || (rotations == nullptr)) == (cov3D_precomp == nullptr))
        return fail(SGR_E_INVALID, "provide exactly one of scales+rotations / cov3D_precomp");
    SgrCamArgs ca;
    ca.view = viewmatrix; ca.proj = projmatrix;
    ca.tan_fovx = tan_fovx; ca.tan_fovy = tan_fovy;
    ca.focal_y = H / (2.0f * tan_fovy); ca.focal_x = W / (2.0f * tan_fovx);
    ca.W = W; ca.H = H; ca.gx = g.gx; ca.gy = g.gy; ca.scale_modifier = scale_modifier;
    SgrGeomView gv;
    memset(&gv, 0, sizeof(gv));
    uint32_t* flag = nullptr;
    SgrFlagBlock fb;
    if (prefiltered) {
        fb = sgr_acquire_flag_block();
        flag = fb.ptr;
        if (!flag) return fail(SGR_E_HIP, "flag block allocation failed");
        SGR_HIP(hipMemsetAsync(flag, 0, 4, stream));
        gv.header = flag;
    }
    SGR_HIP(hipMemsetAsync(means2D, 0, (size_t)P * 2 * sizeof(float), stream));
    sgr_launch_filter(P, means3D, scales, rotations, cov3D_precomp, ca, gv, radii, means2D, prefiltered, stream);
    SGR_STAGE("filter");
    if (prefiltered) {
        uint32_t* host = pinned_pair();
        if (!host) return fail(SGR_E_HIP, "pinned readback slot creation failed");
        SGR_HIP(hipMemcpyAsync(host, flag, 4, hipMemcpyDeviceToHost, stream));
        SGR_HIP(hipStreamSynchronize(stream));
        if (host[0] & 1u) return fail(SGR_E_PREFILTER, "Point is filtered although prefiltered is set. This shouldn't happen!");
    }
    return 0;
}

int sgr_knn(int P, const float* points, float* meanDists, sgr_alloc_fn scratch, void* scratch_user, void* stream_) {
    std::string err;
    const int rc = sgr_knn_impl(P, points, meanDists, scratch, scratch_user, (hipStream_t)stream_, err);
    if (rc < 0) g_err = err;
    return rc;
}

__global__ void sgr_strip_dead_kernel(uint32_t* v, int n) {
    const int i = blockIdx.x * 256 + threadIdx.x;
    if (i < n) v[i] &= ~SGR_DEAD;
}
__global__ void sgr_export_kernel(int which, int P, SgrGeomView gv, void* dst) {
    const int i = blockIdx.x * 256 + threadIdx.x;
    if (i >= P) return;
    switch (which) {
        case 0: ((float*)dst)[i] = gv.rec[4 * (size_t)i + 2].w; break;
        case 1: {
            const uint32_t c = gv.clamped[i];
            ((uint8_t*)dst)[3 * i] = c & 1u; ((uint8_t*)dst)[3 * i + 1] = (c >> 1) & 1u; ((uint8_t*)dst)[3 * i + 2] = (c >> 2) & 1u;
        } break;
        case 2: { const float4 a = gv.rec[4 * (size_t)i]; ((float*)dst)[2 * i] = a.x; ((float*)dst)[2 * i + 1] = a.y; } break;
        case 4: ((float4*)dst)[i] = gv.rec[4 * (size_t)i + 1]; break;
        case 5: { const float4 c = gv.rec[4 * (size_t)i + 2]; ((float*)dst)[3 * i] = c.x; ((float*)dst)[3 * i + 1] = c.y; ((float*)dst)[3 * i + 2] = c.z; } break;
        case 6: ((uint32_t*)dst)[i] = gv.header[6] == 3u ? gv.aux_ref[i].x : gv.aux[i].x; break;
        case 7: ((uint32_t*)dst)[i] = gv.u0[i] + gv.aux[i].x; break;
        case 14: { const float4 a = gv.rec[4 * (size_t)i]; ((float*)dst)[2 * i] = a.z; ((float*)dst)[2 * i + 1] = a.w; } break;
        case 16: {
            const uint2 a = gv.header[6] == 3u ? make_uint2(gv.aux_ref[i].x, gv.aux_ref[i].y) : gv.aux[i];
            const uint32_t x0 = a.y & 1023u, y0 = (a.y >> 10) & 1023u, w = (a.y >> 20) & 1023u;
            uint32_t h = w ? a.x / w : 0u;
            if (a.y & SGR_RECT_MASKED) h = (63u - (uint32_t)__clzll((long long)gv.tmask[i])) / w + 1u;
            ((uint4*)dst)[i] = a.x ? make_uint4(x0, y0, x0 + w, y0 + h) : make_uint4(0u, 0u, 0u, 0u);
        } break;
        case 18:
            ((uint64_t*)dst)[i] = (gv.header[6] != 3u && gv.aux[i].x && (gv.aux[i].y & SGR_RECT_MASKED)) ? gv.tmask[i] : 0ull;
            break;
    }
}

int sgr_export_internal(int which, int P, int R, int width, int height, char* geom_buffer, char* binning_buffer,
                        char* image_buffer, void* dst, void* stream_) {
    hipStream_t stream = (hipStream_t)stream_;
    const Switches sw = resolve_switches();
    const int debug = 1;
    const Frame f = make_frame(std::max(P, 0), R, width, height, geom_buffer, binning_buffer, image_buffer, nullptr, sw);
    const SgrGeomView& gv = f.gv;
    const size_t N = f.g.N, T = f.g.T;
    if (which <= 7 || which == 14 || which == 16 || which == 17 || which == 18) {
        if (P <= 0) return 0;
        if (which == 17) { SGR_HIP(hipMemcpyAsync(dst, gv.header + 5, 4, hipMemcpyDeviceToDevice, stream)); return 0; }
        if (which == 3) return fail(SGR_E_INVALID, "cov3D is not materialised (the backward recomputes it): sgr_export_cov3d");
        if (which == 7) {
            uint32_t mode = 0;
            SGR_HIP(hipMemcpyAsync(&mode, gv.header + 6, 4, hipMemcpyDeviceToHost, stream));
            SGR_HIP(hipStreamSynchronize(stream));
            if (mode == 3u) {
                sgr_launch_scan(reinterpret_cast<const uint32_t*>(gv.aux_ref), (uint32_t*)dst, (size_t)P, gv.scan_tmp, true, stream,
                                nullptr, nullptr, 4);
                SGR_STAGE("export scan");
                return 0;
            }
        }
        sgr_export_kernel<<<(P + 255) / 256, 256, 0, stream>>>(which, P, gv, dst);
        SGR_STAGE("export");
        return 0;
    }
    if (which == 8 || which == 9 || which == 15 || which == 19) {
        if (R <= 0) return 0;
        if (which == 19) { SGR_HIP(hipMemcpyAsync(dst, f.bv.hlist, (size_t)R * 4, hipMemcpyDeviceToDevice, stream)); return 0; }
        if (which == 15) { SGR_HIP(hipMemcpyAsync(dst, f.bv.hit4, (size_t)R, hipMemcpyDeviceToDevice, stream)); return 0; }
        if (which == 8) {
            SGR_HIP(hipMemcpyAsync(dst, f.list, (size_t)R * 4, hipMemcpyDeviceToDevice, stream));
            sgr_strip_dead_kernel<<<(R + 255) / 256, 256, 0, stream>>>((uint32_t*)dst, R);
            SGR_STAGE("export point_list");
        } else {
            sgr_launch_compose_keys(R, f.keys, f.key16, f.list, gv.rec, (uint64_t*)dst, stream);
            SGR_STAGE("export keys");
        }
        return 0;
    }
    if (which == 12) { SGR_HIP(hipMemcpyAsync(dst, f.iv.ranges, T * 8, hipMemcpyDeviceToDevice, stream)); return 0; }
    if (which == 13) { SGR_HIP(hipMemcpyAsync(dst, f.iv.n_contrib, N * 4, hipMemcpyDeviceToDevice, stream)); return 0; }
    if (which == 20) { SGR_HIP(hipMemcpyAsync(dst, f.iv.n_contrib_k, N * 4, hipMemcpyDeviceToDevice, stream)); return 0; }
    return fail(SGR_E_INVALID, "unknown internal array");
}

__global__ void sgr_export_cov3d_kernel(int P, const float* __restrict__ scales, float mod, const float* __restrict__ rotations,
                                        float* __restrict__ dst) {
    const int i = blockIdx.x * 256 + threadIdx.x;
    if (i >= P) return;
    const float sc[3] = {scales[3 * (size_t)i], scales[3 * (size_t)i + 1], scales[3 * (size_t)i + 2]};
    const float rot[4] = {rotations[4 * (size_t)i], rotations[4 * (size_t)i + 1], rotations[4 * (size_t)i + 2],
                          rotations[4 * (size_t)i + 3]};
    float cov3D[6];
    sgr_cov3d(sc, mod, rot, cov3D);
#pragma unroll
    for (int k = 0; k < 6; k++) dst[6 * (size_t)i + k] = cov3D[k];
}
int sgr_export_cov3d(int P, const float* scales, float scale_modifier, const float* rotations, float* dst, void* stream_) {
    hipStream_t stream = (hipStream_t)stream_;
    const int debug = 1;
    if (P <= 0) return 0;
    if (!scales || !rotations || !dst) return fail(SGR_E_INVALID, "sgr_export_cov3d needs scales, rotations and a destination");
    sgr_export_cov3d_kernel<<<(P + 255) / 256, 256, 0, stream>>>(P, scales, scale_modifier, rotations, dst);
    SGR_STAGE("export cov3D");
    return 0;
}

static int sort_gave_up(uint32_t n, const uint32_t* hist, hipStream_t stream) {
    uint32_t e = 0;
    if (!sgr_sort_get_one_sweep() || !n) return 0;
    SGR_HIP(hipMemcpyAsync(&e, hist + SGR_SORT_MAX_PASS * 256 + SGR_SORT_MAX_PASS, 4, hipMemcpyDeviceToHost, stream));
    SGR_HIP(hipStreamSynchronize(stream));
    return e ? sgr_set_error(SGR_E_HIP, "radix sort: look-back gave up") : 0;
}
int sgr_test_scan(const uint32_t* in, uint32_t* out, size_t n, int inclusive, uint32_t* tmp, void* stream_) {
    hipStream_t stream = (hipStream_t)stream_;
    const int debug = 1;
    sgr_launch_scan(in, out, n, tmp, inclusive != 0, stream);
    SGR_STAGE("scan");
    return 0;
}
int sgr_test_sort(uint64_t* keys0, uint64_t* keys1, uint32_t* vals0, uint32_t* vals1, uint32_t n, int end_bit,
                  uint32_t* hist, uint32_t* scan_tmp, void* stream_) {
    hipStream_t stream = (hipStream_t)stream_;
    const int debug = 1;
    uint64_t* keys[2] = {keys0, keys1};
    uint32_t* vals[2] = {vals0, vals1};
    const int cur = sgr_launch_sort_pairs(keys, vals, n, end_bit, hist, scan_tmp, stream);
    SGR_STAGE("sort");
    if (const int rc = sort_gave_up(n, hist, stream)) return rc;
    return cur;
}
int sgr_test_sort32(uint32_t* keys0, uint32_t* keys1, uint32_t* vals0, uint32_t* vals1, uint32_t n, int end_bit,
                    int max_bits, uint32_t* hist, uint32_t* scan_tmp, void* stream_) {
    if (max_bits != 8 && max_bits != 9) return sgr_set_error(SGR_E_INVALID, "sgr_test_sort32: max_bits must be 8 or 9");
    hipStream_t stream = (hipStream_t)stream_;
    const int debug = 1;
    uint32_t* keys[2] = {keys0, keys1};
    uint32_t* vals[2] = {vals0, vals1};
    const int cur = sgr_launch_sort_pairs32(keys, vals, n, end_bit, hist, scan_tmp, stream, false, nullptr, nullptr, max_bits);
    SGR_STAGE("sort32");
    if (const int rc = sort_gave_up(n, hist, stream)) return rc;
    return cur;
}
size_t sgr_test_sort_hist_words(uint32_t n) { return sgr_sort_hist_words(n ? n : 1); }
size_t sgr_test_scan_tmp_words(size_t n) { return sgr_scan_tmp_count(n ? n : 1); }
__global__ void sgr_exact_math_test_kernel(int n, const float* x, float* exp_lib, float* exp_ref, const float* a,
                                           const float* b, float* div_lib, float* div_ref) {
    const int i = blockIdx.x * 256 + threadIdx.x;
    if (i >= n) return;
    exp_lib[i] = expf(x[i]);
    exp_ref[i] = sgr_expf_ref(x[i]);
    const SgrRcp rc = sgr_rcp_refined(b[i]);
    div_lib[i] = a[i] / b[i];
    div_ref[i] = sgr_div_by(a[i], b[i], rc.y);
}
int sgr_test_exact_math(int n, const float* x, float* exp_lib, float* exp_ref, const float* a, const float* b,
                        float* div_lib, float* div_ref, void* stream_) {
    hipStream_t stream = (hipStream_t)stream_;
    const int debug = 1;
    if (n <= 0) return 0;
    sgr_exact_math_test_kernel<<<(n + 255) / 256, 256, 0, stream>>>(n, x, exp_lib, exp_ref, a, b, div_lib, div_ref);
    SGR_STAGE("exact_math");
    return 0;
}
int sgr_test_lds_atomic_order(const uint32_t* pattern, uint32_t* out, int trials, void* stream_) {
    hipStream_t stream = (hipStream_t)stream_;
    const int debug = 1;
    sgr_launch_lds_atomic_order_test(pattern, out, trials, stream);
    SGR_STAGE("lds_atomic_order");
    return 0;
}
int sgr_test_wave_sum(const float* in, float* out_dpp, float* out_shfl, int nwaves, void* stream_) {
    hipStream_t stream = (hipStream_t)stream_;
    const int debug = 1;
    sgr_launch_wave_sum_test(in, out_dpp, out_shfl, nwaves, stream);
    SGR_STAGE("wave_sum");
    return 0;
}

}
```

### street_gaussians_amd/csrc/sgr_common.h

```cpp
#pragma once
#include <hip/hip_runtime.h>
#include <stdint.h>

#define SGR_BLOCK_X 16
#define SGR_BLOCK_Y 16
#define SGR_WAVE 64
#define SGR_MAX_GRID_DIM 1023
#define SGR_SEM_MAX 32
#define SGR_ROW_BASE_N 11
#define SGR_DEAD 0x80000000u
#define SGR_RECT_MASKED 0x80000000u

#define SGR_ALPHA_MIN (1.0f / 255.0f)
#define SGR_DEPTH_KEY_BIAS 0x3E4CCCCDu
#define SGR_DEPTH_KEY_BITS 27
#define SGR_LOG2E 1.4426950408889634f

struct SgrGeomView {
    float4* rec;
    uint2* aux;
    uint64_t* tmask;
    uint4* aux_ref;
    uint2* aux_sorted;
    uint32_t* u0;
    uint32_t* dkeys[2];
    uint32_t* dvals[2];
    uint32_t* sub_sums;
    uint32_t* dhist;
    uint32_t* clamped;
    int* internal_radii;
    uint32_t* scan_tmp;
    float* jac;
    uint32_t* header;
};

#ifndef SGR_HLIST
#define SGR_HLIST 1
#endif

struct SgrBinView {
    uint32_t* keys[2];
    uint32_t* vals[2];
    uint32_t* hist;
    uint32_t* scan_tmp;
    uint32_t* header;
    uint8_t* hit4;
    uint8_t* touched;
    uint32_t* hlist;
    uint32_t* tkeys;
};

#define SGR_STAT_SEG_MAX 128
struct SgrStatSink {
    float* accum = nullptr;
    float* denom = nullptr;
    float* max_radii = nullptr;
    int nseg = 0;
    int start[SGR_STAT_SEG_MAX];
    int count[SGR_STAT_SEG_MAX];
    int shift[SGR_STAT_SEG_MAX];
};

struct SgrImgView {
    uint32_t* n_contrib;
    uint2* ranges;
    uint32_t* n_contrib_k;
};

#define SGR_HDR_JAC 8

static inline size_t sgr_align_up(size_t v, size_t a) { return (v + a - 1) / a * a; }

template <typename T>
static inline void sgr_carve(char*& p, T*& out, size_t count) {
    p = (char*)sgr_align_up((size_t)p, 256);
    out = (T*)p;
    p += count * sizeof(T);
}

#define SGR_SCAN_ITEMS 2048
#ifndef SGR_SORT_IPT
#define SGR_SORT_IPT 8
#endif
#define SGR_SORT_ITEMS (256 * SGR_SORT_IPT)
#define SGR_SORT_MAX_PASS 8

static inline size_t sgr_scan_tmp_count(size_t n) { return (n + SGR_SCAN_ITEMS - 1) / SGR_SCAN_ITEMS + 1; }
#define SGR_SORT_CTRL_WORDS (SGR_SORT_MAX_PASS * 256 + 64)
static inline size_t sgr_sort_hist_words(size_t n) {
    return (size_t)SGR_SORT_CTRL_WORDS + (size_t)512 * ((n + SGR_SORT_ITEMS - 1) / SGR_SORT_ITEMS);
}

static inline SgrGeomView sgr_geom_carve(char* base, size_t P, char** end = nullptr) {
    SgrGeomView v;
    char* p = base;
    size_t Pn = P ? P : 1;
    sgr_carve(p, v.header, 64);
    sgr_carve(p, v.rec, Pn * 4);
    sgr_carve(p, v.aux, Pn);
    sgr_carve(p, v.aux_sorted, 2 * Pn);
    sgr_carve(p, v.aux_ref, Pn);
    sgr_carve(p, v.tmask, Pn);
    sgr_carve(p, v.u0, Pn);
    sgr_carve(p, v.clamped, Pn);
    sgr_carve(p, v.internal_radii, Pn);
    sgr_carve(p, v.dkeys[0], Pn);
    sgr_carve(p, v.dkeys[1], Pn);
    sgr_carve(p, v.dvals[0], Pn);
    sgr_carve(p, v.dvals[1], Pn);
    sgr_carve(p, v.sub_sums, 2 * 8 * ((Pn + SGR_SCAN_ITEMS - 1) / SGR_SCAN_ITEMS));
    {
        const size_t nh = sgr_sort_hist_words(Pn);
        sgr_carve(p, v.dhist, nh);
        sgr_carve(p, v.scan_tmp, 2 * sgr_scan_tmp_count(nh > Pn ? nh : Pn));
    }
    sgr_carve(p, v.jac, 9 * Pn);
    if (end) *end = p;
    return v;
}

static inline SgrBinView sgr_bin_carve(char* base, size_t R, char** end = nullptr) {
    SgrBinView v;
    char* p = base;
    size_t Rn = R ? R : 1;
    size_t nh = sgr_sort_hist_words(Rn);
    sgr_carve(p, v.header, 64);
    sgr_carve(p, v.keys[0], Rn);
    sgr_carve(p, v.keys[1], Rn);
    sgr_carve(p, v.vals[0], Rn);
    sgr_carve(p, v.vals[1], Rn);
    sgr_carve(p, v.hist, nh);
    sgr_carve(p, v.scan_tmp, sgr_scan_tmp_count(nh));
    sgr_carve(p, v.hit4, Rn);
    sgr_carve(p, v.touched, Rn);
    sgr_carve(p, v.tkeys, Rn);
    sgr_carve(p, v.hlist, Rn);
    if (end) *end = p;
    return v;
}

static inline SgrImgView sgr_img_carve(char* base, size_t N, size_t T, char** end = nullptr) {
    SgrImgView v;
    char* p = base;
    sgr_carve(p, v.n_contrib, N ? N : 1);
    sgr_carve(p, v.ranges, (T ? T : 1) + ((T ? T : 1) + 2) / 2);
    sgr_carve(p, v.n_contrib_k, N ? N : 1);
    if (end) *end = p;
    return v;
}

template <typename F>
static inline size_t sgr_required(F carve) {
    char* end = nullptr;
    char* base = (char*)4096;
    carve(base, &end);
    return (size_t)(end - base) + 256;
}

#ifdef __HIPCC__
#include <mutex>
#include <string>
#include <type_traits>

constexpr int sgr_smax(int S) { return S == 0 ? 0 : S <= 4 ? 4 : S <= 24 ? (S + 3) / 4 * 4 : SGR_SEM_MAX; }
template <int N = 0, typename F>
static inline void sgr_with_smax(int S, F&& f) {
    if (sgr_smax(S) == N) f(std::integral_constant<int, N>{});
    else if constexpr (N < SGR_SEM_MAX) sgr_with_smax<sgr_smax(N + 1)>(S, f);
}

int sgr_set_error(int code, const std::string& msg);
#define SGR_HIP(call)                                                                                                \
    do {                                                                                                             \
        hipError_t e__ = (call);                                                                                     \
        if (e__ != hipSuccess) return sgr_set_error(SGR_E_HIP, std::string(#call) + ": " + hipGetErrorString(e__)); \
    } while (0)

struct SgrFlagBlock {
    uint32_t* ptr = nullptr;
    std::unique_lock<std::mutex> lock;
};
SgrFlagBlock sgr_acquire_flag_block();
void sgr_launch_scan(const uint32_t* in, uint32_t* out, size_t n, uint32_t* tmp, bool inclusive, hipStream_t s,
                     uint32_t* total_out = nullptr, const uint32_t* gather = nullptr, int in_stride = 1,
                     const uint32_t* in2 = nullptr, uint32_t* out2 = nullptr);
void sgr_launch_scan_head(const uint32_t* in, const uint32_t* in2, size_t n, int in_stride, uint32_t* tmp, uint32_t* sub,
                          hipStream_t s, int in2_stride = 0);
int sgr_sort_get_one_sweep();
void sgr_sort_set_one_sweep(int on);
int sgr_launch_sort_pairs(uint64_t* const keys[2], uint32_t* const vals[2], uint32_t n, int end_bit, uint32_t* hist,
                          uint32_t* scan_tmp, hipStream_t s);
int sgr_launch_sort_pairs32(uint32_t* const keys[2], uint32_t* const vals[2], uint32_t n, int end_bit, uint32_t* hist,
                            uint32_t* scan_tmp, hipStream_t s, bool iota = false, const uint2* aux_in = nullptr,
                            uint2* aux_out = nullptr, int max_bits = 8, int aux16 = 0,
                            const uint32_t* dev_n = nullptr);
int sgr_launch_sort_pairs16(uint16_t* const keys[2], uint32_t* const vals[2], uint32_t n, int end_bit, uint32_t* hist,
                            uint32_t* scan_tmp, hipStream_t s);
int sgr_sort_pass_count(int end_bit);
void sgr_launch_tile_sort(int T, const uint2* ranges, uint32_t* vals_in, uint32_t* vals_out, const uint32_t* dkeys,
                          const uint32_t* header, uint32_t* gk0, uint32_t* gk1, hipStream_t s);

__device__ __forceinline__ uint32_t sgr_wave_incl_scan(uint32_t v, int lane) {
#pragma unroll
    for (int d = 1; d < 64; d <<= 1) {
        uint32_t t = __shfl_up(v, d, 64);
        if (lane >= d) v += t;
    }
    return v;
}

__device__ __forceinline__ uint32_t sgr_block_excl_scan256(uint32_t v, uint32_t* lds4, uint32_t& total) {
    const int lane = threadIdx.x & 63, wave = threadIdx.x >> 6;
    const uint32_t inc = sgr_wave_incl_scan(v, lane);
    if (lane == 63) lds4[wave] = inc;
    __syncthreads();
    const uint32_t w0 = lds4[0], w1 = lds4[1], w2 = lds4[2], w3 = lds4[3];
    __syncthreads();
    const uint32_t base = (wave > 0 ? w0 : 0) + (wave > 1 ? w1 : 0) + (wave > 2 ? w2 : 0);
    total = w0 + w1 + w2 + w3;
    return base + inc - v;
}

#define SGR_ST 8
static inline unsigned sgr_xcd_grid_blocks(int gx, int gy) {
    const unsigned nst = (unsigned)((gx + SGR_ST - 1) / SGR_ST) * (unsigned)((gy + SGR_ST - 1) / SGR_ST);
    return ((nst + 7u) / 8u) * 8u * (SGR_ST * SGR_ST);
}
__device__ __forceinline__ bool sgr_xcd_tile(uint32_t b, uint32_t gx, uint32_t gy, uint32_t& tx, uint32_t& ty) {
    const uint32_t x = b & 7u, q = b >> 3;
    const uint32_t st = (q / (SGR_ST * SGR_ST)) * 8u + x, within = q % (SGR_ST * SGR_ST);
    const uint32_t sgx = (gx + SGR_ST - 1) / SGR_ST;
    tx = (st % sgx) * SGR_ST + (within % SGR_ST);
    ty = (st / sgx) * SGR_ST + (within / SGR_ST);
    return tx < gx && ty < gy;
}

__device__ __forceinline__ bool sgr_wg_tile(uint32_t b, int gx, int gy, const uint2* __restrict__ ranges, uint32_t& tx, uint32_t& ty) {
    if (gy >= 0) return sgr_xcd_tile(b, (uint32_t)gx, (uint32_t)gy, tx, ty);
    const uint32_t T = (uint32_t)gx * (uint32_t)(-gy);
    const uint32_t* order = reinterpret_cast<const uint32_t*>(ranges + T);
    if (order[T] == 0u) return sgr_xcd_tile(b, (uint32_t)gx, (uint32_t)(-gy), tx, ty);
    if (b >= T) return false;
    const uint32_t t = order[b];
    tx = t % (uint32_t)gx;
    ty = t / (uint32_t)gx;
    return true;
}

__device__ __forceinline__ uint64_t sgr_uniform_u64(uint64_t v) {
    const uint32_t lo = (uint32_t)__builtin_amdgcn_readfirstlane((int)(uint32_t)v);
    const uint32_t hi = (uint32_t)__builtin_amdgcn_readfirstlane((int)(uint32_t)(v >> 32));
    return ((uint64_t)hi << 32) | (uint64_t)lo;
}
__device__ __forceinline__ int sgr_pop_lowest(uint64_t& m) {
    const int b = __builtin_ctzll(m);
    asm("s_bitset0_b64 %0, %1" : "+s"(m) : "s"(b));
    return b;
}
__device__ __forceinline__ uint64_t sgr_bitset1(uint64_t m, int b) {
    asm("s_bitset1_b64 %0, %1" : "+s"(m) : "s"(b));
    return m;
}
#endif
```

### street_gaussians_amd/csrc/sgr_launch.h

```cpp
#pragma once
#include "../../include/sgr.h"
#include "sgr_math.h"

struct SgrTileLists {
    int gx = 0, gy = 0;
    int W = 0, H = 0;
    const uint2* ranges = nullptr;
    const uint32_t* point_list = nullptr;
    const float4* rec = nullptr;
    unsigned blocks() const { return (gx <= 0 || gy == 0) ? 0u : sgr_xcd_grid_blocks(gx, gy < 0 ? -gy : gy); }
};
template <typename F> static inline void sgr_with_flag(bool on, F&& f) { if (on) f(std::true_type{}); else f(std::false_type{}); }

void sgr_launch_mark_visible(int P, const float* means3D, const float* viewmatrix, uint8_t* present, hipStream_t s);
void sgr_launch_preprocess(int P, int D, int M, const float* means3D, const float* scales, const float* rotations,
                           const float* opacities, const float* shs, const float* cov3D_precomp, const float* colors_precomp,
                           const SgrCam* cam, const SgrGeomView& gv, int* radii, int prefiltered, bool stage_sh, int tight,
                           bool want_jac, hipStream_t s);
void sgr_launch_filter(int P, const float* means3D, const float* scales, const float* rotations, const float* cov3D_precomp,
                       const SgrCamArgs& ca, const SgrGeomView& gv, int* radii, float* means2D, int prefiltered, hipStream_t s);
void sgr_launch_duplicate(int P, const SgrGeomView& gv, const uint32_t* order, const uint32_t* bsum, const uint32_t* sub, void* keys,
                          int key16, uint32_t* vals, int gx, uint32_t cap, int marks, hipStream_t s);
void sgr_launch_tile_ranges(int L, const void* keys, int key16, uint2* ranges, uint8_t* touched, uint32_t T, hipStream_t s);
void sgr_launch_tile_order(const uint2* ranges, int T, int force, hipStream_t s);
void sgr_launch_compose_keys(int L, const void* tile_keys, int key16, const uint32_t* point_list, const float4* rec, uint64_t* out,
                             hipStream_t s);
void sgr_launch_blend_fwd(bool cull, bool exact, const SgrTileLists& tl, int S, const float* semantics, const float* bg,
                          float* out_color, float* out_depth, float* out_alpha, float* out_semantic, uint32_t* n_contrib,
                          uint8_t* hit4, uint32_t* hlist, uint32_t* n_contrib_k, hipStream_t s);
void sgr_launch_blend_layers(bool exact, const SgrTileLists& tl, int split, int P, const float* bg, int clamp,
                             float* const color[2], float* const alpha[2], hipStream_t s);
void sgr_launch_layers_fill(int W, int H, const float* bg, int clamp, float* const color[2], float* const alpha[2], hipStream_t s);
void sgr_launch_object_alpha_fwd(bool exact, const SgrTileLists& tl, int split, float* out_alpha, uint32_t* out_last, hipStream_t s);
void sgr_launch_object_alpha_bwd(bool exact, const SgrTileLists& tl, const uint32_t* u0, const uint64_t* tmask, int split,
                                 const float* layer_alpha, const uint32_t* layer_last, const float* dL_dlayer_alpha,
                                 float* partials, int row_stride, uint8_t* touched, uint32_t row_limit, hipStream_t s);

int sgr_partial_row_stride(int S);
struct SgrBlendBwdArgs {
    bool cull = true, dpp = true, det = true;
    bool v2 = false, exact = false;
    int S = 0;
    const float *bg = nullptr, *semantics = nullptr, *alphas = nullptr;
    const uint64_t* tmask = nullptr;
    const uint32_t *u0 = nullptr, *n_contrib = nullptr, *n_contrib_k = nullptr;
    const uint8_t* hit4 = nullptr;
    const uint32_t* hlist = nullptr;
    const uint32_t* hl_flag = nullptr;
    const float *dL_dpix = nullptr, *dL_ddepth = nullptr, *dL_dalpha = nullptr, *dL_dsem = nullptr;
    float* partials = nullptr;
    uint8_t* touched = nullptr;
    uint32_t row_limit = 0;
};
void sgr_launch_blend_bwd(const SgrTileLists& tl, const SgrBlendBwdArgs& a, hipStream_t s);
void sgr_launch_blend_bwd_sw(const SgrTileLists& tl, const SgrBlendBwdArgs& a, int row_stride, hipStream_t s);

struct SgrGaussBwdArgs {
    int P = 0, D = 0, M = 0, S = 0;
    const float *means3D = nullptr, *shs = nullptr, *scales = nullptr, *rotations = nullptr, *cov3D_precomp = nullptr;
    const int* radii = nullptr;
    const SgrCam* cam = nullptr;
    SgrGeomView gv = {};
    const float* partials = nullptr;
    int row_stride = 0, W = 0, H = 0;
    const uint8_t* touched = nullptr;
    float4* cd = nullptr;
    float *dL_dmean2D = nullptr, *dL_dopacity = nullptr, *dL_dcolor = nullptr, *dL_dmean3D = nullptr, *dL_dcov3D = nullptr,
          *dL_dsh = nullptr, *dL_dscale = nullptr, *dL_drot = nullptr, *dL_dsemantic = nullptr;
    SgrStatSink sink;
    int quad = 0;
    int exact = 0, rs_wave = 0;
    hipEvent_t after_rows = nullptr;
    uint32_t row_limit = 0;
    float* masked_color_out = nullptr;
    int skip_sh = 0, skip_cov = 0;
};
typedef int SgrGaussBwdLauncher(const SgrGaussBwdArgs& a, hipStream_t s);
SgrGaussBwdLauncher sgr_launch_gauss_bwd, sgr_launch_gauss_bwd_strict;
void sgr_launch_masked_color_grad(int P, const uint32_t* clamped, const float* dL_dcolor, float* out, hipStream_t s);
void sgr_launch_sh_grad_from_views(int P, int D, int M, int V, const float* means3D, size_t means_stride, const float* campos,
                                   size_t campos_stride, const float* drgb, size_t drgb_stride, float* dL_dsh, hipStream_t s);
void sgr_launch_wave_sum_test(const float* in, float* out_dpp, float* out_shfl, int nwaves, hipStream_t s);
void sgr_launch_lds_atomic_order_test(const uint32_t* pattern, uint32_t* out, int trials, hipStream_t s);
int sgr_knn_impl(int P, const float* points, float* meanDists, sgr_alloc_fn scratch, void* scratch_user, hipStream_t s,
                 std::string& err);
```

### street_gaussians_amd/csrc/sgr_preprocess.hip

```cpp
#include "sgr_math.h"
#include "sgr_launch.h"

#include <cstdlib>

#ifndef SGR_PRE_THREADS
#define SGR_PRE_THREADS 256
#endif

__device__ __forceinline__ uint32_t sgr_pack_rect(uint32_t x0, uint32_t y0, uint32_t w) {
    return x0 | (y0 << 10) | (w << 20);
}

__global__ void __launch_bounds__(SGR_PRE_THREADS)
sgr_mark_visible_kernel(int P, const float* __restrict__ means3D, const float* __restrict__ v, uint8_t* __restrict__ present) {
#pragma clang fp contract(off)
    const int idx = blockIdx.x * SGR_PRE_THREADS + threadIdx.x;
    if (idx >= P) return;
    const float x = means3D[3 * idx], y = means3D[3 * idx + 1], z = means3D[3 * idx + 2];
    const float tz = v[2] * x + v[6] * y + v[10] * z + v[14];
    present[idx] = tz <= 0.2f ? 0 : 1;
}

__device__ __forceinline__ SgrProj
sgr_preprocess_geom(const int idx, const float (&p)[3], const float* __restrict__ scales, const float* __restrict__ rotations,
                    const float* __restrict__ cov3D_precomp, const SgrCam& cam, uint32_t* __restrict__ header,
                    int prefiltered) {
    float tz;
    {
#pragma clang fp contract(off)
        const float* v = cam.view;
        tz = v[2] * p[0] + v[6] * p[1] + v[10] * p[2] + v[14];
    }
    SgrProj pr;
    pr.ok = false;
    if (tz > 0.2f) {
        float cov3D[6];
        if (cov3D_precomp != nullptr) {
#pragma unroll
            for (int i = 0; i < 6; i++) cov3D[i] = cov3D_precomp[6 * (size_t)idx + i];
        } else {
            const float sc[3] = {scales[3 * idx], scales[3 * idx + 1], scales[3 * idx + 2]};
            const float4 q = *reinterpret_cast<const float4*>(rotations + 4 * (size_t)idx);
            const float rot[4] = {q.x, q.y, q.z, q.w};
            sgr_cov3d(sc, cam.scale_modifier, rot, cov3D);
        }
        pr = sgr_project(p, cov3D, cam);
    } else if (prefiltered) {
        if (header) atomicOr(&header[0], 1u);
    }
    return pr;
}

__global__ void __launch_bounds__(SGR_PRE_THREADS)
sgr_filter_kernel(int P, const float* __restrict__ means3D, const float* __restrict__ scales,
                  const float* __restrict__ rotations, const float* __restrict__ cov3D_precomp, uint32_t* __restrict__ header,
                  int* __restrict__ radii, float* __restrict__ filter_means2D, int prefiltered, SgrCamArgs ca) {
    const int idx = blockIdx.x * SGR_PRE_THREADS + threadIdx.x;
    SgrCam cam;
#pragma unroll
    for (int i = 0; i < 16; i++) { cam.view[i] = ca.view[i]; cam.proj[i] = ca.proj[i]; }
    cam.campos[0] = cam.campos[1] = cam.campos[2] = 0.f;
    cam.tan_fovx = ca.tan_fovx; cam.tan_fovy = ca.tan_fovy; cam.focal_x = ca.focal_x; cam.focal_y = ca.focal_y;
    cam.W = ca.W; cam.H = ca.H; cam.gx = ca.gx; cam.gy = ca.gy; cam.scale_modifier = ca.scale_modifier;
    if (idx >= P) return;
    const float p[3] = {means3D[3 * idx], means3D[3 * idx + 1], means3D[3 * idx + 2]};
    const SgrProj pr = sgr_preprocess_geom(idx, p, scales, rotations, cov3D_precomp, cam, header, prefiltered);
    if (!pr.ok) { radii[idx] = 0; return; }
    radii[idx] = pr.radius;
    filter_means2D[2 * idx] = pr.px;
    filter_means2D[2 * idx + 1] = pr.py;
}

__device__ __forceinline__ void sgr_store_color_jacobian(int D, float x, float y, float z, const float* row,
                                                         float* __restrict__ dst) {
    float J[9];
    sgr_sh_color_jacobian(D, x, y, z, row, J);
#pragma unroll
    for (int e = 0; e < 9; e++) dst[e] = J[e];
}

__global__ void __launch_bounds__(SGR_PRE_THREADS)
sgr_preprocess_kernel(int P, int D, int M, const float* __restrict__ means3D, const float* __restrict__ scales,
                      const float* __restrict__ rotations, const float* __restrict__ opacities,
                      const float* __restrict__ shs, const float* __restrict__ cov3D_precomp,
                      const float* __restrict__ colors_precomp, const SgrCam* __restrict__ camp, SgrGeomView gv,
                      int* __restrict__ radii, int prefiltered, int stage_sh, int tight, int want_jac) {
    extern __shared__ float4 sSHdyn[];
    float4 (*sSH)[32 * 13] = reinterpret_cast<float4 (*)[32 * 13]>(sSHdyn);
    __shared__ uint32_t wave_sum[2 * (SGR_PRE_THREADS / 64)];
    const SgrCam& cam = *camp;
    const int gidx = blockIdx.x * SGR_PRE_THREADS + threadIdx.x;
    const bool live = gidx < P;
    const int idx = live ? gidx : P - 1;
    const int lane = threadIdx.x & 63, wave = threadIdx.x >> 6;
    const float p[3] = {means3D[3 * idx], means3D[3 * idx + 1], means3D[3 * idx + 2]};
    SgrProj pr = sgr_preprocess_geom(idx, p, scales, rotations, cov3D_precomp, cam, live ? gv.header : nullptr, prefiltered);
    const bool ok = live && pr.ok;

    const bool stage = stage_sh && shs != nullptr && colors_precomp == nullptr && M == 16;
    float rgb_s[3] = {0.f, 0.f, 0.f};
    if (stage) {
#pragma clang fp contract(off)
        float Y[16];
        float dx = p[0] - cam.campos[0], dy = p[1] - cam.campos[1], dz = p[2] - cam.campos[2];
        {
            const float t0 = dx * dx, t1 = dy * dy, t2 = dz * dz;
            const float len = sqrtf(t0 + t1 + t2);
            dx = dx / len; dy = dy / len; dz = dz / len;
            sgr_sh_basis(D, dx, dy, dz, Y);
        }
        const int ncoef = (D + 1) * (D + 1);
        const int n4 = (ncoef * 3 + 3) >> 2;
        const uint64_t vis = __ballot(ok);
        const int g0 = blockIdx.x * SGR_PRE_THREADS + wave * 64;
        const int nrow4 = max(0, min(64, P - g0)) * 12;
        const float4* src = reinterpret_cast<const float4*>(shs) + (size_t)g0 * 12;
#pragma unroll
        for (int h = 0; h < 2; h++) {
#pragma unroll
            for (int it = 0; it < 6; it++) {
                const int f = h * 384 + it * 64 + lane;
                const int row = f / 12;
                if (f < nrow4 && ((vis >> row) & 1ull)) sSH[wave][f - h * 384 + (row - 32 * h)] = src[f];
            }
            __builtin_amdgcn_wave_barrier();
            if ((lane >> 5) == h && ok) {
#pragma unroll
                for (int i = 0; i < 12; i++) {
                    if (i < n4) {
                        const float4 t = sSH[wave][(lane & 31) * 13 + i];
                        const float e[4] = {t.x, t.y, t.z, t.w};
#pragma unroll
                        for (int j = 0; j < 4; j++) {
                            const int k = (4 * i + j) / 3, ch = (4 * i + j) % 3;
                            if (k < ncoef) rgb_s[ch] = (k == 0) ? Y[0] * e[j] : rgb_s[ch] + Y[k] * e[j];
                        }
                    }
                }
                if (want_jac)
                    sgr_store_color_jacobian(D, dx, dy, dz, reinterpret_cast<const float*>(&sSH[wave][(lane & 31) * 13]),
                                             gv.jac + 9 * (size_t)idx);
            }
            __builtin_amdgcn_wave_barrier();
        }
    }

    uint32_t n = 0, nref = 0;
    if (live && !ok) {
        radii[idx] = 0;
        gv.aux[idx] = make_uint2(0u, 0u);
        if (tight == 3) gv.aux_ref[idx] = make_uint4(0u, 0u, 0u, 0u);
        gv.dkeys[0][idx] = 0xffffffffu;
    }
    if (ok) {
        float rgb[3];
        uint32_t clamped = 0;
        if (colors_precomp != nullptr) {
            rgb[0] = colors_precomp[3 * idx];
            rgb[1] = colors_precomp[3 * idx + 1];
            rgb[2] = colors_precomp[3 * idx + 2];
        } else {
#pragma clang fp contract(off)
            float dx = p[0] - cam.campos[0], dy = p[1] - cam.campos[1], dz = p[2] - cam.campos[2];
            const float t0 = dx * dx, t1 = dy * dy, t2 = dz * dz;
            const float len = sqrtf(t0 + t1 + t2);
            dx = dx / len; dy = dy / len; dz = dz / len;
            float Y[16];
            sgr_sh_basis(D, dx, dy, dz, Y);
            const int ncoef = (D + 1) * (D + 1);
            const float* sh = shs + (size_t)idx * M * 3;
            float r = 0.f, g = 0.f, b = 0.f;
            if (stage) {
                r = rgb_s[0]; g = rgb_s[1]; b = rgb_s[2];
            } else if (((M * 3) & 3) == 0 && M <= 16) {
                const float4* sh4 = reinterpret_cast<const float4*>(sh);
                const int n4 = (ncoef * 3 + 3) >> 2;
                float buf[48];
#pragma unroll
                for (int i = 0; i < 12; i++) {
                    if (i < n4) {
                        const float4 t = sh4[i];
                        buf[4 * i] = t.x; buf[4 * i + 1] = t.y; buf[4 * i + 2] = t.z; buf[4 * i + 3] = t.w;
                    }
                }
#pragma unroll
                for (int k = 0; k < 16; k++) {
                    if (k < ncoef) {
                        if (k == 0) { r = Y[0] * buf[0]; g = Y[0] * buf[1]; b = Y[0] * buf[2]; }
                        else { r = r + Y[k] * buf[3 * k]; g = g + Y[k] * buf[3 * k + 1]; b = b + Y[k] * buf[3 * k + 2]; }
                    }
                }
                if (want_jac) sgr_store_color_jacobian(D, dx, dy, dz, buf, gv.jac + 9 * (size_t)idx);
            } else {
                for (int k = 0; k < ncoef; k++) {
                    if (k == 0) { r = Y[0] * sh[0]; g = Y[0] * sh[1]; b = Y[0] * sh[2]; }
                    else { r = r + Y[k] * sh[3 * k]; g = g + Y[k] * sh[3 * k + 1]; b = b + Y[k] * sh[3 * k + 2]; }
                }
                if (want_jac) sgr_store_color_jacobian(D, dx, dy, dz, sh, gv.jac + 9 * (size_t)idx);
            }
            r += 0.5f; g += 0.5f; b += 0.5f;
            clamped = (r < 0 ? 1u : 0u) | (g < 0 ? 2u : 0u) | (b < 0 ? 4u : 0u);
            rgb[0] = fmaxf(r, 0.0f); rgb[1] = fmaxf(g, 0.0f); rgb[2] = fmaxf(b, 0.0f);
        }

        const float opacity = opacities[idx];
        float hx, hy;
        sgr_extent(opacity, pr.cov_a, pr.cov_c, pr.con_x, pr.con_y, pr.con_z, hx, hy);
        uint32_t x0 = pr.rx0, x1 = pr.rx1, y0 = pr.ry0, y1 = pr.ry1;
        const uint32_t rn = (x1 - x0) * (y1 - y0);
        if (tight) {
            const float inv = 1.0f / SGR_BLOCK_X;
            static_assert(SGR_BLOCK_X == SGR_BLOCK_Y, "square tiles");
            float fx0 = fmaxf(floorf((pr.px - hx) * inv), (float)x0), fx1 = fminf(floorf((pr.px + hx) * inv) + 1.0f, (float)x1);
            float fy0 = fmaxf(floorf((pr.py - hy) * inv), (float)y0), fy1 = fminf(floorf((pr.py + hy) * inv) + 1.0f, (float)y1);
            if (!(fx0 < fx1)) { fx0 = fminf(fmaxf(floorf(pr.px * inv), (float)x0), (float)(x1 - 1)); fx1 = fx0 + 1.0f; }
            if (!(fy0 < fy1)) { fy0 = fminf(fmaxf(floorf(pr.py * inv), (float)y0), (float)(y1 - 1)); fy1 = fy0 + 1.0f; }
            x0 = (uint32_t)fx0; x1 = (uint32_t)fx1; y0 = (uint32_t)fy0; y1 = (uint32_t)fy1;
        }
        const uint32_t w = x1 - x0, h = y1 - y0;
        uint32_t rect = sgr_pack_rect(x0, y0, w);
        uint32_t nemit = w * h;
        if (tight > 1 && w >= 2u && h >= 2u && nemit <= 64u) {
            uint64_t tm = sgr_tile_mask(pr.px, pr.py, pr.con_x, pr.con_y, pr.con_z, opacity, x0, y0, x1, y1);
            if (tm == 0) {
                const uint32_t cx = (uint32_t)fminf(fmaxf(floorf(pr.px * (1.0f / SGR_BLOCK_X)), (float)x0), (float)(x1 - 1));
                const uint32_t cy = (uint32_t)fminf(fmaxf(floorf(pr.py * (1.0f / SGR_BLOCK_Y)), (float)y0), (float)(y1 - 1));
                tm = 1ull << ((cy - y0) * w + (cx - x0));
            }
            const uint32_t cnt = (uint32_t)__builtin_popcountll(tm);
            if (cnt != nemit) {
                rect |= SGR_RECT_MASKED;
                gv.tmask[idx] = tm;
                nemit = cnt;
            }
        }
        nref = rn;
        float4* rec = gv.rec + 4 * (size_t)idx;
        rec[0] = make_float4(pr.px, pr.py, hx, hy);
        rec[1] = make_float4(pr.con_x, pr.con_y, pr.con_z, opacity);
        rec[2] = make_float4(rgb[0], rgb[1], rgb[2], pr.depth);
        const float4 st = sgr_stage_conic(make_float4(pr.con_x, pr.con_y, pr.con_z, opacity));
        rec[3] = make_float4(st.x, __uint_as_float(rect), st.y, st.z);
        gv.clamped[idx] = clamped;
        gv.aux[idx] = make_uint2(nemit, rect);
        if (tight == 3) gv.aux_ref[idx] = make_uint4(rn, sgr_pack_rect(pr.rx0, pr.ry0, pr.rx1 - pr.rx0), nemit, rect);
        const uint32_t dkey = __float_as_uint(pr.depth) - SGR_DEPTH_KEY_BIAS;
        if (dkey >> SGR_DEPTH_KEY_BITS) atomicOr(&gv.header[2], 1u);
        gv.dkeys[0][idx] = dkey;
        radii[idx] = pr.radius;
        n = tight == 3 ? rn : nemit;
    }
#pragma unroll
    for (int m = 32; m >= 1; m >>= 1) { n += __shfl_xor(n, m, 64); nref += __shfl_xor(nref, m, 64); }
    if (lane == 0) { wave_sum[wave] = n; wave_sum[SGR_PRE_THREADS / 64 + wave] = nref; }
    __syncthreads();
    if (threadIdx.x == 0) {
        uint32_t t = 0, tr = 0;
#pragma unroll
        for (int i = 0; i < SGR_PRE_THREADS / 64; i++) { t += wave_sum[i]; tr += wave_sum[SGR_PRE_THREADS / 64 + i]; }
        if (tr) atomicAdd(reinterpret_cast<unsigned long long*>(gv.header + 4), (unsigned long long)t | ((unsigned long long)tr << 32));
    }
}

static_assert(SGR_PRE_THREADS == 256 && SGR_SCAN_ITEMS == 8 * SGR_PRE_THREADS, "one workgroup = one sub-block of the scan");
template <typename K>
__global__ void __launch_bounds__(SGR_PRE_THREADS)
sgr_duplicate_kernel(int P, SgrGeomView gv, const uint32_t* __restrict__ order, const uint32_t* __restrict__ bsum,
                     const uint32_t* __restrict__ sub, uint32_t nb, K* __restrict__ keys, uint32_t* __restrict__ vals,
                     int gx, uint32_t cap, int marks) {
    if (cap != 0) {
        const uint32_t R = bsum[nb];
        for (uint32_t s = R + blockIdx.x * SGR_PRE_THREADS + threadIdx.x; s < cap; s += gridDim.x * SGR_PRE_THREADS) {
            keys[s] = (K)~(K)0;
            vals[s] = 0u;
        }
    }
    __shared__ uint32_t sOff[SGR_PRE_THREADS / 64][64];
    __shared__ uint32_t sRect[SGR_PRE_THREADS / 64][64];
    __shared__ uint32_t sIdx[SGR_PRE_THREADS / 64][64];
    __shared__ uint64_t sMask[SGR_PRE_THREADS / 64][64];
    __shared__ uint32_t sLive[SGR_PRE_THREADS / 64][64];
    __shared__ uint32_t sLiveN[SGR_PRE_THREADS / 64][64];
    __shared__ uint32_t lds4[4];
    const int i = blockIdx.x * SGR_PRE_THREADS + threadIdx.x;
    const int lane = threadIdx.x & 63, wave = threadIdx.x >> 6;
    uint32_t off = 0xffffffffu, incl = 0, idx = 0, rect = 0, live_rect = 0, live_n = 0;
    uint64_t tmask = 0;
    uint2 as = make_uint2(0u, 0u), lv = make_uint2(0u, 0u);
    if (i < P) {
        if (marks) {
            const uint4 t = reinterpret_cast<const uint4*>(gv.aux_sorted)[i];
            as = make_uint2(t.x, t.y);
            lv = make_uint2(t.z, t.w);
        } else as = gv.aux_sorted[i];
    }
    const uint32_t t2 = (i < P) ? gv.aux[i].x : 0u;
    uint32_t total;
    const uint32_t ex1 = sgr_block_excl_scan256(as.x, lds4, total) + bsum[blockIdx.x >> 3] + sub[blockIdx.x];
    const uint32_t ex2 = sgr_block_excl_scan256(t2, lds4, total) + bsum[nb + 1 + (blockIdx.x >> 3)] + sub[8 * nb + blockIdx.x];
    if (i < P) {
        gv.u0[i] = ex2;
        idx = order ? order[i] : (uint32_t)i;
        off = ex1;
        incl = ex1 + as.x;
        if (incl != off) {
            rect = as.y;
            if (marks) {
                live_rect = lv.y;
                live_n = lv.x;
                if (live_rect & SGR_RECT_MASKED) tmask = gv.tmask[idx];
            } else if (rect & SGR_RECT_MASKED) tmask = gv.tmask[idx];
        }
    }
    sOff[wave][lane] = off;
    sRect[wave][lane] = rect;
    sIdx[wave][lane] = idx;
    sMask[wave][lane] = tmask;
    if (marks) { sLive[wave][lane] = live_rect; sLiveN[wave][lane] = live_n; }
    const uint32_t start = __builtin_amdgcn_readfirstlane(off);
    const int last = min(63, P - 1 - (blockIdx.x * SGR_PRE_THREADS + wave * 64));
    if (last < 0) return;
    uint32_t end = __builtin_amdgcn_readlane(incl, last);
    if (cap != 0 && end > cap) end = cap;
    __builtin_amdgcn_wave_barrier();
    for (uint32_t s = start + lane; s < end; s += 64) {
        int o = 0;
#pragma unroll
        for (int step = 32; step >= 1; step >>= 1)
            if (sOff[wave][o + step] <= s) o += step;
        const uint32_t r = sRect[wave][o];
        const uint32_t x0 = r & 1023u, y0 = (r >> 10) & 1023u, w = (r >> 20) & 1023u;
        uint32_t k = s - sOff[wave][o];
        if (!marks && (r & SGR_RECT_MASKED)) k = sgr_select_bit(sMask[wave][o], k);
        uint32_t q = (uint32_t)((float)k * __builtin_amdgcn_rcpf((float)w));
        int rem = (int)k - (int)(q * w);
        if (rem < 0) { q--; rem += (int)w; }
        if (rem >= (int)w) { q++; rem -= (int)w; }
        const uint32_t tx = x0 + (uint32_t)rem, ty = y0 + q;
        keys[s] = (K)(ty * (uint32_t)gx + tx);
        uint32_t v = sIdx[wave][o];
        if (marks) {
            const uint32_t lr = sLive[wave][o];
            const uint32_t lx0 = lr & 1023u, ly0 = (lr >> 10) & 1023u, lw = (lr >> 20) & 1023u;
            const uint32_t dxl = tx - lx0, dyl = ty - ly0;
            const uint32_t j = dyl * lw + dxl;
            bool live = dxl < lw && ty >= ly0;
            if (lr & SGR_RECT_MASKED) live = live && j < 64u && ((sMask[wave][o] >> (j & 63u)) & 1ull);
            else live = live && j < sLiveN[wave][o];
            if (!live) v |= SGR_DEAD;
        }
        vals[s] = v;
    }
}

#define SGR_RANGES_PER_THREAD 8
template <typename K>
__global__ void __launch_bounds__(256)
sgr_tile_ranges_kernel(int L, const K* __restrict__ keys, uint2* __restrict__ ranges, uint8_t* __restrict__ touched,
                       uint32_t T) {
    constexpr int E = SGR_RANGES_PER_THREAD;
    const int i0 = (blockIdx.x * 256 + threadIdx.x) * E;
    if (i0 >= L) return;
    K k[E];
    if (i0 + E <= L) {
        struct alignas(sizeof(K) * E) Pack { K v[E]; };
        const Pack p = *reinterpret_cast<const Pack*>(keys + i0);
#pragma unroll
        for (int e = 0; e < E; e++) k[e] = p.v[e];
        *reinterpret_cast<uint2*>(touched + i0) = make_uint2(0u, 0u);
    } else {
#pragma unroll
        for (int e = 0; e < E; e++) {
            k[e] = i0 + e < L ? keys[i0 + e] : (K)0;
            if (i0 + e < L) touched[i0 + e] = 0;
        }
    }
    uint32_t prevtile = i0 > 0 ? (uint32_t)keys[i0 - 1] : 0u;
#pragma unroll
    for (int e = 0; e < E; e++) {
        const int idx = i0 + e;
        if (idx >= L) break;
        const uint32_t currtile = k[e];
        if (idx == 0) {
            if (currtile < T) ranges[currtile].x = 0;
        } else if (currtile != prevtile) {
            if (prevtile < T) ranges[prevtile].y = idx;
            if (currtile < T) ranges[currtile].x = idx;
        }
        if (idx == L - 1 && currtile < T) ranges[currtile].y = L;
        prevtile = currtile;
    }
}

__global__ void __launch_bounds__(1024)
sgr_tile_order_kernel(const uint2* __restrict__ ranges, uint32_t T, uint32_t* __restrict__ order, uint32_t ratio_x16, int force) {
    __shared__ uint32_t hist[1024];
    __shared__ uint32_t smax;
    __shared__ unsigned long long ssum;
    __shared__ uint32_t sw[16];
    const int tid = threadIdx.x, lane = tid & 63, wave = tid >> 6;
    hist[tid] = 0u;
    if (tid == 0) { smax = 0u; ssum = 0ull; }
    __syncthreads();
    uint32_t mx = 0;
    unsigned long long sm = 0;
    for (uint32_t t = tid; t < T; t += 1024) {
        const uint32_t len = ranges[t].y - ranges[t].x;
        mx = max(mx, len);
        sm += len;
    }
#pragma unroll
    for (int o = 32; o >= 1; o >>= 1) {
        mx = max(mx, (uint32_t)__shfl_xor((int)mx, o, 64));
        sm += (unsigned long long)__shfl_xor((long long)sm, o, 64);
    }
    if (lane == 0) { atomicMax(&smax, mx); atomicAdd(&ssum, sm); }
    __syncthreads();
    const bool lpt = force || (unsigned long long)smax * T * 16ull > (unsigned long long)ratio_x16 * ssum;
    if (tid == 0) order[T] = lpt ? 1u : 0u;
    if (!lpt) return;
    const float sc = 1023.0f / (float)max(smax, 1u);
    for (uint32_t t = tid; t < T; t += 1024) {
        const uint32_t len = ranges[t].y - ranges[t].x;
        atomicAdd(&hist[1023u - min(1023u, (uint32_t)((float)len * sc))], 1u);
    }
    __syncthreads();
    const uint32_t c = hist[tid];
    const uint32_t inc = sgr_wave_incl_scan(c, lane);
    if (lane == 63) sw[wave] = inc;
    __syncthreads();
    uint32_t base = 0;
    for (int w = 0; w < wave; w++) base += sw[w];
    __syncthreads();
    hist[tid] = base + inc - c;
    __syncthreads();
    for (uint32_t t = tid; t < T; t += 1024) {
        const uint32_t len = ranges[t].y - ranges[t].x;
        order[atomicAdd(&hist[1023u - min(1023u, (uint32_t)((float)len * sc))], 1u)] = t;
    }
}
void sgr_launch_tile_order(const uint2* ranges, int T, int force, hipStream_t s) {
    if (T <= 0) return;
    static const uint32_t ratio_x16 = [] { const char* e = getenv("SGR_LPT_RATIO_X16"); return e ? (uint32_t)atoi(e) : 40u; }();
    sgr_tile_order_kernel<<<1, 1024, 0, s>>>(ranges, (uint32_t)T, reinterpret_cast<uint32_t*>(const_cast<uint2*>(ranges) + T), ratio_x16, force);
}

template <typename K>
__global__ void __launch_bounds__(256)
sgr_compose_keys_kernel(int L, const K* __restrict__ tile_keys, const uint32_t* __restrict__ point_list,
                        const float4* __restrict__ rec, uint64_t* __restrict__ out) {
    const int i = blockIdx.x * 256 + threadIdx.x;
    if (i >= L) return;
    out[i] = ((uint64_t)tile_keys[i] << 32) | (uint64_t)__float_as_uint(rec[4 * (size_t)(point_list[i] & ~SGR_DEAD) + 2].w);
}

void sgr_launch_mark_visible(int P, const float* means3D, const float* viewmatrix, uint8_t* present, hipStream_t s) {
    if (P <= 0) return;
    sgr_mark_visible_kernel<<<(P + SGR_PRE_THREADS - 1) / SGR_PRE_THREADS, SGR_PRE_THREADS, 0, s>>>(P, means3D, viewmatrix,
                                                                                                 present);
}

void sgr_launch_preprocess(int P, int D, int M, const float* means3D, const float* scales, const float* rotations,
                           const float* opacities, const float* shs, const float* cov3D_precomp,
                           const float* colors_precomp, const SgrCam* cam, const SgrGeomView& gv, int* radii,
                           int prefiltered, bool stage_sh, int tight, bool want_jac, hipStream_t s) {
    if (P <= 0) return;
    const bool stage = stage_sh && shs != nullptr && colors_precomp == nullptr && M == 16;
    const size_t lds = stage ? (size_t)(SGR_PRE_THREADS / 64) * 32 * 13 * sizeof(float4) : 0;
    sgr_preprocess_kernel<<<(P + SGR_PRE_THREADS - 1) / SGR_PRE_THREADS, SGR_PRE_THREADS, lds, s>>>(
        P, D, M, means3D, scales, rotations, opacities, shs, cov3D_precomp, colors_precomp, cam, gv, radii, prefiltered,
        stage ? 1 : 0, tight, (want_jac && shs != nullptr && colors_precomp == nullptr) ? 1 : 0);
}

void sgr_launch_filter(int P, const float* means3D, const float* scales, const float* rotations,
                       const float* cov3D_precomp, const SgrCamArgs& ca, const SgrGeomView& gv, int* radii,
                       float* means2D, int prefiltered, hipStream_t s) {
    if (P <= 0) return;
    sgr_filter_kernel<<<(P + SGR_PRE_THREADS - 1) / SGR_PRE_THREADS, SGR_PRE_THREADS, 0, s>>>(
        P, means3D, scales, rotations, cov3D_precomp, gv.header, radii, means2D, prefiltered, ca);
}

void sgr_launch_duplicate(int P, const SgrGeomView& gv, const uint32_t* order, const uint32_t* bsum, const uint32_t* sub,
                          void* keys, int key16, uint32_t* vals, int gx, uint32_t cap, int marks, hipStream_t s) {
    if (P <= 0) return;
    const uint32_t nb = (uint32_t)(((size_t)P + SGR_SCAN_ITEMS - 1) / SGR_SCAN_ITEMS);
    const unsigned grid = (P + SGR_PRE_THREADS - 1) / SGR_PRE_THREADS;
    if (key16) sgr_duplicate_kernel<uint16_t><<<grid, SGR_PRE_THREADS, 0, s>>>(P, gv, order, bsum, sub, nb, (uint16_t*)keys, vals, gx, cap, marks);
    else sgr_duplicate_kernel<uint32_t><<<grid, SGR_PRE_THREADS, 0, s>>>(P, gv, order, bsum, sub, nb, (uint32_t*)keys, vals, gx, cap, marks);
}

void sgr_launch_tile_ranges(int L, const void* keys, int key16, uint2* ranges, uint8_t* touched, uint32_t T, hipStream_t s) {
    if (L <= 0) return;
    const unsigned grid = (unsigned)((L + 256 * SGR_RANGES_PER_THREAD - 1) / (256 * SGR_RANGES_PER_THREAD));
    if (key16) sgr_tile_ranges_kernel<uint16_t><<<grid, 256, 0, s>>>(L, (const uint16_t*)keys, ranges, touched, T);
    else sgr_tile_ranges_kernel<uint32_t><<<grid, 256, 0, s>>>(L, (const uint32_t*)keys, ranges, touched, T);
}

void sgr_launch_compose_keys(int L, const void* tile_keys, int key16, const uint32_t* point_list, const float4* rec, uint64_t* out,
                             hipStream_t s) {
    if (L <= 0) return;
    if (key16) sgr_compose_keys_kernel<uint16_t><<<(L + 255) / 256, 256, 0, s>>>(L, (const uint16_t*)tile_keys, point_list, rec, out);
    else sgr_compose_keys_kernel<uint32_t><<<(L + 255) / 256, 256, 0, s>>>(L, (const uint32_t*)tile_keys, point_list, rec, out);
}
```

### street_gaussians_amd/csrc/sgr_scan_sort.hip

```cpp
#include "sgr_common.h"

#include <atomic>
#include <cstdlib>

#ifndef SGR_WITH_VARIANTS
#define SGR_WITH_VARIANTS 0
#endif


__global__ void __launch_bounds__(256) sgr_scan_reduce_kernel(const uint32_t* __restrict__ in, size_t n,
                                                              uint32_t* __restrict__ block_sums,
                                                              const uint32_t* __restrict__ gather, int stride,
                                                              const uint32_t* __restrict__ in2, unsigned nb,
                                                              uint32_t* __restrict__ sub, int stride2) {
    __shared__ uint32_t lds4[4];
    unsigned b = blockIdx.x;
    if (b >= nb) { b -= nb; in = in2; gather = nullptr; block_sums += nb + 1; if (sub) sub += 8 * nb; stride = stride2; }
    const size_t base = (size_t)b * SGR_SCAN_ITEMS + (size_t)threadIdx.x * 8;
    uint32_t s = 0;
#pragma unroll
    for (int i = 0; i < 8; i++)
        if (base + i < n) s += gather ? in[(size_t)gather[base + i] * stride] : in[(base + i) * stride];
    uint32_t total;
    const uint32_t ex = sgr_block_excl_scan256(s, lds4, total);
    if (threadIdx.x == 0) block_sums[b] = total;
    if (sub != nullptr && (threadIdx.x & 31) == 0) sub[8 * b + (threadIdx.x >> 5)] = ex;
}

__global__ void __launch_bounds__(256) sgr_scan_spine_kernel(uint32_t* __restrict__ block_sums, size_t nb,
                                                             uint32_t* __restrict__ total_out) {
    __shared__ uint32_t lds4[4];
    if (blockIdx.x) { block_sums += nb + 1; total_out = nullptr; }
    uint32_t carry = 0;
    for (size_t start = 0; start < nb; start += 256) {
        const size_t i = start + threadIdx.x;
        const uint32_t v = i < nb ? block_sums[i] : 0;
        uint32_t total;
        const uint32_t ex = sgr_block_excl_scan256(v, lds4, total);
        if (i < nb) block_sums[i] = carry + ex;
        carry += total;
    }
    if (threadIdx.x == 0) {
        block_sums[nb] = carry;
        if (total_out) *total_out = carry;
    }
}

__global__ void __launch_bounds__(256) sgr_scan_final_kernel(const uint32_t* __restrict__ in, uint32_t* __restrict__ out,
                                                             size_t n, const uint32_t* __restrict__ block_sums,
                                                             const uint32_t* __restrict__ gather, int stride, bool inclusive,
                                                             const uint32_t* __restrict__ in2, uint32_t* __restrict__ out2,
                                                             unsigned nb) {
    __shared__ uint32_t lds4[4];
    unsigned b = blockIdx.x;
    if (b >= nb) { b -= nb; in = in2; out = out2; gather = nullptr; block_sums += nb + 1; inclusive = false; }
    const size_t base = (size_t)b * SGR_SCAN_ITEMS + (size_t)threadIdx.x * 8;
    uint32_t v[8];
    uint32_t s = 0;
#pragma unroll
    for (int i = 0; i < 8; i++) {
        v[i] = (base + i < n) ? (gather ? in[(size_t)gather[base + i] * stride] : in[(base + i) * stride]) : 0;
        s += v[i];
    }
    uint32_t total;
    uint32_t run = sgr_block_excl_scan256(s, lds4, total) + block_sums[b];
#pragma unroll
    for (int i = 0; i < 8; i++) {
        if (inclusive) run += v[i];
        if (base + i < n) out[base + i] = run;
        if (!inclusive) run += v[i];
    }
}

void sgr_launch_scan(const uint32_t* in, uint32_t* out, size_t n, uint32_t* tmp, bool inclusive, hipStream_t s,
                     uint32_t* total_out, const uint32_t* gather, int in_stride, const uint32_t* in2, uint32_t* out2) {
    if (n == 0) return;
    const size_t nb = (n + SGR_SCAN_ITEMS - 1) / SGR_SCAN_ITEMS;
    const unsigned seqs = in2 ? 2u : 1u;

    sgr_scan_reduce_kernel<<<(unsigned)nb * seqs, 256, 0, s>>>(in, n, tmp, gather, in_stride, in2, (unsigned)nb, nullptr, in_stride);
    sgr_scan_spine_kernel<<<seqs, 256, 0, s>>>(tmp, nb, total_out);
    sgr_scan_final_kernel<<<(unsigned)nb * seqs, 256, 0, s>>>(in, out, n, tmp, gather, in_stride, inclusive, in2, out2,
                                                             (unsigned)nb);
}

void sgr_launch_scan_head(const uint32_t* in, const uint32_t* in2, size_t n, int in_stride, uint32_t* tmp, uint32_t* sub,
                          hipStream_t s, int in2_stride) {
    if (in2_stride <= 0) in2_stride = in_stride;
    if (n == 0) return;
    const size_t nb = (n + SGR_SCAN_ITEMS - 1) / SGR_SCAN_ITEMS;
    sgr_scan_reduce_kernel<<<(unsigned)nb * 2u, 256, 0, s>>>(in, n, tmp, nullptr, in_stride, in2, (unsigned)nb, sub, in2_stride);
    sgr_scan_spine_kernel<<<2, 256, 0, s>>>(tmp, nb, nullptr);
}

template <typename K, int IPT>
__global__ void __launch_bounds__(256)
sgr_sort_hist_kernel(const K* __restrict__ keys, uint32_t n, int shift, uint32_t mask, uint32_t nblocks,
                     uint32_t* __restrict__ hist, const uint32_t* __restrict__ dev_n) {
    if (dev_n) {
        n = min(n, *dev_n);
        if (blockIdx.x * (256u * IPT) >= n) {
            for (uint32_t d = threadIdx.x; d <= mask; d += 256) hist[(size_t)d * nblocks + blockIdx.x] = 0u;
            return;
        }
    }
    __shared__ uint32_t h[4][512];
#pragma unroll
    for (int w = 0; w < 4; w++) { h[w][threadIdx.x] = 0; h[w][256 + threadIdx.x] = 0; }
    __syncthreads();
    const int wave = threadIdx.x >> 6;
    const uint32_t base = blockIdx.x * (256u * IPT);
    constexpr int V = 16 / (int)sizeof(K);
    static_assert(IPT % V == 0, "keys per thread must be a multiple of the vector width");
    struct alignas(16) Vec { K k[V]; };
#pragma unroll
    for (int s = 0; s < IPT / V; s++) {
        const uint32_t i = base + (s * 256 + threadIdx.x) * V;
        if (i + V <= n) {
            const Vec v = *reinterpret_cast<const Vec*>(keys + i);
#pragma unroll
            for (int e = 0; e < V; e++) atomicAdd(&h[wave][(uint32_t)(v.k[e] >> shift) & mask], 1u);
        } else {
#pragma unroll
            for (int e = 0; e < V; e++)
                if (i + e < n) atomicAdd(&h[wave][(uint32_t)(keys[i + e] >> shift) & mask], 1u);
        }
    }
    __syncthreads();
    for (uint32_t d = threadIdx.x; d <= mask; d += 256)
        hist[(size_t)d * nblocks + blockIdx.x] = h[0][d] + h[1][d] + h[2][d] + h[3][d];
}

__global__ void __launch_bounds__(256)
sgr_sort_rowscan_kernel(uint32_t* __restrict__ hist, uint32_t nblocks, uint32_t* __restrict__ totals) {
    __shared__ uint32_t lds4[4];
    uint32_t* row = hist + (size_t)blockIdx.x * nblocks;
    uint32_t carry = 0;
    for (uint32_t start = 0; start < nblocks; start += 256 * 8) {
        const uint32_t base = start + threadIdx.x * 8;
        uint32_t v[8], s = 0;
#pragma unroll
        for (int i = 0; i < 8; i++) {
            v[i] = (base + i < nblocks) ? row[base + i] : 0u;
            s += v[i];
        }
        uint32_t total;
        uint32_t run = carry + sgr_block_excl_scan256(s, lds4, total);
#pragma unroll
        for (int i = 0; i < 8; i++) {
            if (base + i < nblocks) row[base + i] = run;
            run += v[i];
        }
        carry += total;
    }
    if (threadIdx.x == 0) totals[blockIdx.x] = carry;
}

#define SGR_OS_AGG (1ull << 48)
#define SGR_OS_PREFIX (2ull << 48)
#define SGR_OS_VALUE ((1ull << 48) - 1ull)
template <typename K, int BITS, int IPT, bool ONE>
__global__ void __launch_bounds__(256)
sgr_sort_scatter_kernel(const K* __restrict__ kin, const uint32_t* __restrict__ vin, K* __restrict__ kout,
                        uint32_t* __restrict__ vout, uint32_t n, int shift, uint32_t nblocks,
                        const uint32_t* __restrict__ hist_scanned, const uint32_t* __restrict__ totals,
                        unsigned long long* __restrict__ status, uint32_t* __restrict__ ticket, uint32_t* __restrict__ err,
                        uint32_t pass_tag, const uint2* __restrict__ aux_in, uint2* __restrict__ aux_out, int aux16,
                        const uint32_t* __restrict__ dev_n) {
    constexpr int NB = 1 << BITS;
    constexpr int BPT = NB > 256 ? NB / 256 : 1;
    static_assert(!(ONE && NB > 256), "the one-sweep form has one status word per thread");
    constexpr uint32_t ITEMS = 256u * IPT;
    __shared__ uint32_t cnt[4][NB];
    __shared__ uint32_t lstart[NB];
    __shared__ uint32_t gbase[NB];
    __shared__ uint32_t lds4[4];
    __shared__ K sK[ITEMS];
    __shared__ uint32_t sV[ITEMS];
    const int tid = threadIdx.x, lane = tid & 63, wave = tid >> 6;
    if (!ONE && dev_n) {
        n = min(n, *dev_n);
        if (blockIdx.x * ITEMS >= n) return;
    }
    if (ONE && tid == 0) lds4[0] = atomicAdd(ticket, 1u);
    for (int b = tid; b < NB; b += 256) {
#pragma unroll
        for (int w = 0; w < 4; w++) cnt[w][b] = 0;
    }
    __syncthreads();
    const uint32_t block = ONE ? lds4[0] : blockIdx.x;

    constexpr int BPL = NB > 64 ? NB / 64 : 1;
    uint32_t pre_before[BPL], pre_total[BPL];
    if (!ONE && wave == 0) {
#pragma unroll
        for (int j = 0; j < BPL; j++) {
            const int bin = lane * BPL + j;
            pre_before[j] = bin < NB ? hist_scanned[(size_t)bin * nblocks + block] : 0u;
            pre_total[j] = bin < NB ? totals[bin] : 0u;
        }
    }

    const uint32_t base = block * ITEMS + wave * (64 * IPT);
    K key[IPT];
    uint32_t val[IPT], rnk[IPT];
#pragma unroll
    for (int s = 0; s < IPT; s++) {
        const uint32_t i = base + s * 64 + lane;
        const bool valid = i < n;
        key[s] = valid ? kin[i] : (K)0;
        val[s] = valid ? (vin ? vin[i] : i) : 0u;
    }
#pragma unroll
    for (int s = 0; s < IPT; s++) {
        const bool valid = base + s * 64 + lane < n;
        const uint32_t d = (uint32_t)(key[s] >> shift) & (uint32_t)(NB - 1);
        const uint64_t vm = __builtin_amdgcn_ballot_w64(valid);
        uint32_t mlo = (uint32_t)vm, mhi = (uint32_t)(vm >> 32);
#pragma unroll
        for (int b = 0; b < BITS; b++) {
            const int y = __builtin_amdgcn_sbfe((int)d, b, 1);
            const uint64_t bal = __builtin_amdgcn_ballot_w64(y != 0);
            mlo &= ~((uint32_t)bal ^ (uint32_t)y);
            mhi &= ~((uint32_t)(bal >> 32) ^ (uint32_t)y);
        }
        const uint32_t prefix = __builtin_amdgcn_mbcnt_hi(mhi, __builtin_amdgcn_mbcnt_lo(mlo, 0u));
        const uint32_t prev = valid ? cnt[wave][d] : 0u;
        __builtin_amdgcn_wave_barrier();
        if (valid && prefix == 0) cnt[wave][d] = prev + (uint32_t)(__builtin_popcount(mlo) + __builtin_popcount(mhi));
        rnk[s] = prev + prefix;
        __builtin_amdgcn_wave_barrier();
    }
    __syncthreads();
    if constexpr (!ONE) {
        if (wave == 0) {
            uint32_t c[BPL][4], tot[BPL];
            uint32_t sum_t = 0, sum_g = 0;
#pragma unroll
            for (int j = 0; j < BPL; j++) {
                const int bin = lane * BPL + j;
#pragma unroll
                for (int w = 0; w < 4; w++) c[j][w] = bin < NB ? cnt[w][bin] : 0u;
                tot[j] = c[j][0] + c[j][1] + c[j][2] + c[j][3];
                sum_t += tot[j];
                sum_g += pre_total[j];
            }
            uint32_t g = sgr_wave_incl_scan(sum_g, lane) - sum_g;
            uint32_t ls = sgr_wave_incl_scan(sum_t, lane) - sum_t;
#pragma unroll
            for (int j = 0; j < BPL; j++) {
                const int bin = lane * BPL + j;
                if (bin < NB) {
                    gbase[bin] = pre_before[j] + g;
                    lstart[bin] = ls;
                    cnt[0][bin] = ls;
                    cnt[1][bin] = ls + c[j][0];
                    cnt[2][bin] = ls + c[j][0] + c[j][1];
                    cnt[3][bin] = ls + c[j][0] + c[j][1] + c[j][2];
                }
                g += pre_total[j];
                ls += tot[j];
            }
        }
    } else
    if constexpr (BPT == 1) {
        const bool bin = tid < NB;
        const uint32_t c0 = bin ? cnt[0][tid] : 0u, c1 = bin ? cnt[1][tid] : 0u, c2 = bin ? cnt[2][tid] : 0u,
                       c3 = bin ? cnt[3][tid] : 0u;
        uint32_t all;
        uint32_t before = 0;
        if (ONE) {
            const unsigned long long tag = (unsigned long long)pass_tag << 56;
            const uint32_t c = c0 + c1 + c2 + c3;
            unsigned long long* mine = status + (size_t)block * 256 + tid;
            __hip_atomic_store(mine, tag | (block == 0 ? SGR_OS_PREFIX : SGR_OS_AGG) | c, __ATOMIC_RELAXED,
                               __HIP_MEMORY_SCOPE_AGENT);
            unsigned long long sum = 0;
            uint32_t spins = 0;
            for (uint32_t pb = block; pb > 0;) {
                const unsigned long long w = __hip_atomic_load(status + (size_t)(pb - 1) * 256 + tid, __ATOMIC_RELAXED,
                                                               __HIP_MEMORY_SCOPE_AGENT);
                if ((w >> 56) != pass_tag) {
                    __builtin_amdgcn_s_sleep(1);
                    if (++spins > (1u << 22)) { atomicOr(err, 1u); break; }
                    continue;
                }
                sum += w & SGR_OS_VALUE;
                if (w & SGR_OS_PREFIX) break;
                pb--;
            }
            if (block > 0)
                __hip_atomic_store(mine, tag | SGR_OS_PREFIX | (sum + c), __ATOMIC_RELAXED, __HIP_MEMORY_SCOPE_AGENT);
            before = (uint32_t)sum;
        } else if (bin) {
            before = hist_scanned[(size_t)tid * nblocks + block];
        }
        const uint32_t g = before + sgr_block_excl_scan256(bin ? totals[tid] : 0u, lds4, all);
        const uint32_t ls = sgr_block_excl_scan256(c0 + c1 + c2 + c3, lds4, all);
        if (bin) {
            gbase[tid] = g;
            lstart[tid] = ls;
            cnt[0][tid] = ls;
            cnt[1][tid] = ls + c0;
            cnt[2][tid] = ls + c0 + c1;
            cnt[3][tid] = ls + c0 + c1 + c2;
        }
    } else {
        uint32_t c[BPT][4], tot[BPT], gt[BPT], before[BPT];
        uint32_t sum_t = 0, sum_g = 0, all;
#pragma unroll
        for (int j = 0; j < BPT; j++) {
            const int bin = tid * BPT + j;
#pragma unroll
            for (int w = 0; w < 4; w++) c[j][w] = cnt[w][bin];
            tot[j] = c[j][0] + c[j][1] + c[j][2] + c[j][3];
            gt[j] = totals[bin];
            before[j] = hist_scanned[(size_t)bin * nblocks + block];
            sum_t += tot[j];
            sum_g += gt[j];
        }
        uint32_t g = sgr_block_excl_scan256(sum_g, lds4, all);
        uint32_t ls = sgr_block_excl_scan256(sum_t, lds4, all);
#pragma unroll
        for (int j = 0; j < BPT; j++) {
            const int bin = tid * BPT + j;
            gbase[bin] = before[j] + g;
            lstart[bin] = ls;
            cnt[0][bin] = ls;
            cnt[1][bin] = ls + c[j][0];
            cnt[2][bin] = ls + c[j][0] + c[j][1];
            cnt[3][bin] = ls + c[j][0] + c[j][1] + c[j][2];
            g += gt[j];
            ls += tot[j];
        }
    }
    __syncthreads();
#pragma unroll
    for (int s = 0; s < IPT; s++) {
        const uint32_t i = base + s * 64 + lane;
        if (i < n) {
            const uint32_t d = (uint32_t)(key[s] >> shift) & (uint32_t)(NB - 1);
            const uint32_t lp = cnt[wave][d] + rnk[s];
            sK[lp] = key[s];
            sV[lp] = val[s];
        }
    }
    __syncthreads();
    const uint32_t first = block * ITEMS;
    const uint32_t nloc = min(ITEMS, n - first);
#pragma unroll
    for (int s = 0; s < IPT; s++) {
        const uint32_t li = s * 256 + tid;
        if (li < nloc) {
            const K k = sK[li];
            const uint32_t d = (uint32_t)(k >> shift) & (uint32_t)(NB - 1);
            const uint32_t pos = gbase[d] + (li - lstart[d]);
            const uint32_t v = sV[li];
            kout[pos] = k;
            vout[pos] = v;
            if (aux_in != nullptr) {
                if (aux16) reinterpret_cast<uint4*>(aux_out)[pos] = reinterpret_cast<const uint4*>(aux_in)[v];
                else aux_out[pos] = aux_in[v];
            }
        }
    }
}

#if SGR_WITH_VARIANTS
template <typename K>
__global__ void __launch_bounds__(256)
sgr_sort_hist_all_kernel(const K* __restrict__ keys, uint32_t n, int npass, uint32_t* __restrict__ ghist,
                         unsigned long long* __restrict__ status, size_t status_words) {
    __shared__ uint32_t h[SGR_SORT_MAX_PASS][256];
    for (int p = 0; p < npass; p++) h[p][threadIdx.x] = 0;
    __syncthreads();
    for (size_t i = (size_t)blockIdx.x * 256 + threadIdx.x; i < status_words; i += (size_t)gridDim.x * 256) status[i] = 0ull;
    for (uint32_t chunk = blockIdx.x; (size_t)chunk * 4096 < n; chunk += gridDim.x) {
#pragma unroll 4
        for (int s = 0; s < 16; s++) {
            const uint32_t i = chunk * 4096u + s * 256 + threadIdx.x;
            if (i < n) {
                const K k = keys[i];
                for (int p = 0; p < npass; p++) atomicAdd(&h[p][(uint32_t)(k >> (8 * p)) & 255u], 1u);
            }
        }
    }
    __syncthreads();
    for (int p = 0; p < npass; p++) {
        const uint32_t c = h[p][threadIdx.x];
        if (c) atomicAdd(&ghist[p * 256 + threadIdx.x], c);
    }
}

#endif

static std::atomic<int> g_sort_one_sweep{-1};
void sgr_sort_set_one_sweep(int on) { g_sort_one_sweep.store(on ? 1 : 0, std::memory_order_relaxed); }
int sgr_sort_get_one_sweep() {
    int v = g_sort_one_sweep.load(std::memory_order_relaxed);
    if (v < 0) {
        const char* e = getenv("SGR_ONESWEEP");
        v = (e && *e && *e != '0') ? 1 : 0;
        g_sort_one_sweep.store(v, std::memory_order_relaxed);
    }
    return v;
}

static inline int sort_passes(int end_bit, int max_bits) {
    static const int forced = [] { const char* e = getenv("SGR_SORT_BITS"); return e ? atoi(e) : 0; }();
    const int maxb = forced == 8 ? 8 : max_bits;
    return (end_bit + maxb - 1) / maxb;
}
static inline int sort_pass_bits(int end_bit, int max_bits) {
    const int npass = sort_passes(end_bit, max_bits);
    return npass ? (end_bit + npass - 1) / npass : 8;
}
static inline int sort_ipt(uint32_t n, size_t key_bytes) {
    static const int forced = [] { const char* e = getenv("SGR_SORT_IPT"); return e ? atoi(e) : 0; }();
    if (forced == 8 || forced == 16) return forced;
    if (key_bytes == 2) return n >= 500000u ? 16 : 8;
    return n >= 3000000u ? 16 : 8;
}

int sgr_sort_pass_count(int end_bit) { return (end_bit + 7) / 8; }

template <typename K, int BITS, int IPT>
static void sort_pass(const K* kin, const uint32_t* vin, K* kout, uint32_t* vout, uint32_t n, int shift, uint32_t* hist,
                      const uint2* aux_in, uint2* aux_out, int aux16, hipStream_t s, const uint32_t* dev_n) {
    const uint32_t nblocks = (n + 256u * IPT - 1) / (256u * IPT);
    constexpr int NB = 1 << BITS;
    sgr_sort_hist_kernel<K, IPT><<<nblocks, 256, 0, s>>>(kin, n, shift, (uint32_t)(NB - 1), nblocks, hist, dev_n);
    uint32_t* totals = hist + (size_t)NB * nblocks;
    sgr_sort_rowscan_kernel<<<NB, 256, 0, s>>>(hist, nblocks, totals);
    sgr_sort_scatter_kernel<K, BITS, IPT, false><<<nblocks, 256, 0, s>>>(kin, vin, kout, vout, n, shift, nblocks, hist, totals,
                                                                         nullptr, nullptr, nullptr, 0u, aux_in, aux_out, aux16,
                                                                         dev_n);
}

template <typename K>
static int sort_pairs_impl(K* const keys[2], uint32_t* const vals[2], uint32_t n, int end_bit, uint32_t* hist,
                           uint32_t* scan_tmp, hipStream_t s, bool iota = false, const uint2* aux_in = nullptr,
                           uint2* aux_out = nullptr, int max_bits = 8, int aux16 = 0, const uint32_t* dev_n = nullptr) {
    if (n == 0) return 0;
    int npass = (end_bit + 7) / 8;
    int cur = 0;
#if SGR_WITH_VARIANTS
    if (sgr_sort_get_one_sweep() && npass <= SGR_SORT_MAX_PASS && !iota && !aux_in && !dev_n) {
        const uint32_t nblocks = (n + SGR_SORT_ITEMS - 1) / SGR_SORT_ITEMS;
        uint32_t* ghist = hist;
        uint32_t* tickets = hist + SGR_SORT_MAX_PASS * 256;
        uint32_t* err = tickets + SGR_SORT_MAX_PASS;
        unsigned long long* status = reinterpret_cast<unsigned long long*>(hist + SGR_SORT_CTRL_WORDS);
        (void)hipMemsetAsync(hist, 0, SGR_SORT_CTRL_WORDS * sizeof(uint32_t), s);
        const uint32_t chunks = (n + 4095u) / 4096u;
        sgr_sort_hist_all_kernel<K><<<chunks < 1024u ? chunks : 1024u, 256, 0, s>>>(keys[0], n, npass, ghist, status,
                                                                                   (size_t)nblocks * 256);
        for (int p = 0; p < npass; p++) {
            sgr_sort_scatter_kernel<K, 8, SGR_SORT_IPT, true><<<nblocks, 256, 0, s>>>(
                keys[cur], vals[cur], keys[cur ^ 1], vals[cur ^ 1], n, 8 * p, nblocks, nullptr, ghist + p * 256, status,
                tickets + p, err, (uint32_t)p + 1u, nullptr, nullptr, 0, nullptr);
            cur ^= 1;
        }
        return cur;
    }
#endif
    const int bits = sizeof(K) == 8 ? 8 : sort_pass_bits(end_bit, max_bits);
    const int ipt = sizeof(K) == 8 ? 8 : sort_ipt(n, sizeof(K));
    if (sizeof(K) <= 4) npass = sort_passes(end_bit, max_bits);
    for (int p = 0; p < npass; p++) {
        const uint32_t* vin = (iota && p == 0) ? nullptr : vals[cur];
        const bool last = p == npass - 1;
        const uint2* ai = last ? aux_in : nullptr;
        uint2* ao = last ? aux_out : nullptr;
        const int shift = bits * p;
#define SGR_PASS(B, I) sort_pass<K, B, I>(keys[cur], vin, keys[cur ^ 1], vals[cur ^ 1], n, shift, hist, ai, ao, aux16, s, dev_n)
        if constexpr (sizeof(K) == 8) { SGR_PASS(8, 8); }
        else if (ipt == 16 && bits <= 8) {
            if (bits <= 5) SGR_PASS(5, 16); else if (bits == 6) SGR_PASS(6, 16); else if (bits == 7) SGR_PASS(7, 16); else SGR_PASS(8, 16);
        } else {
            if (bits <= 5) SGR_PASS(5, 8); else if (bits == 6) SGR_PASS(6, 8); else if (bits == 7) SGR_PASS(7, 8);
            else if (bits == 8) SGR_PASS(8, 8); else SGR_PASS(9, 8);
        }
#undef SGR_PASS
        cur ^= 1;
    }
    return cur;
}
int sgr_launch_sort_pairs(uint64_t* const keys[2], uint32_t* const vals[2], uint32_t n, int end_bit, uint32_t* hist,
                          uint32_t* scan_tmp, hipStream_t s) {
    return sort_pairs_impl<uint64_t>(keys, vals, n, end_bit, hist, scan_tmp, s);
}
int sgr_launch_sort_pairs32(uint32_t* const keys[2], uint32_t* const vals[2], uint32_t n, int end_bit, uint32_t* hist,
                            uint32_t* scan_tmp, hipStream_t s, bool iota, const uint2* aux_in, uint2* aux_out, int max_bits, int aux16,
                            const uint32_t* dev_n) {
    return sort_pairs_impl<uint32_t>(keys, vals, n, end_bit, hist, scan_tmp, s, iota, aux_in, aux_out, max_bits, aux16, dev_n);
}
int sgr_launch_sort_pairs16(uint16_t* const keys[2], uint32_t* const vals[2], uint32_t n, int end_bit, uint32_t* hist,
                            uint32_t* scan_tmp, hipStream_t s) {
    return sort_pairs_impl<uint16_t>(keys, vals, n, end_bit > 16 ? 16 : end_bit, hist, scan_tmp, s);
}
```

Before: 659.8.

## Fold radix-sort row scan and scan-head block sums into consumer kernels

Adds an optional grouped-histogram sort pass. Per-group digit tables are reduced inside the scatter kernel, which removes the separate rowscan launch. Also adds a raw-sums scan-head mode where the duplicate kernel reduces unscanned block sums itself instead of reading a second-level scan. Both aim to cut kernel launches and small serial scan stages, at the cost of redundant per-block reductions and a larger histogram scratch. The sort fold is off unless an environment variable sets it.

```diff
diff --git a/include/sgr.h b/include/sgr.h
--- a/include/sgr.h
+++ b/include/sgr.h
@@ -144,6 +144,14 @@
 int sgr_test_sort32(uint32_t* keys0, uint32_t* keys1, uint32_t* vals0, uint32_t* vals1, uint32_t n, int end_bit,
                     int max_bits, uint32_t* hist, uint32_t* scan_tmp, void* stream);
 size_t sgr_test_sort_hist_words(uint32_t n);
+int sgr_test_sort_fold(int g);
+int sgr_test_scan_fold(int on);
+int sgr_test_sort_ex(int key_bytes, void* keys0, void* keys1, uint32_t* vals0, uint32_t* vals1, uint32_t n, int end_bit,
+                     int max_bits, int iota, const void* aux_in, void* aux_out, int aux16, const uint32_t* dev_n, uint32_t* hist,
+                     void* stream);
+int sgr_test_fold_layout(uint32_t n, uint32_t items, uint32_t NB, uint32_t G, uint64_t* out);
+int sgr_test_fold_replay(const uint32_t* counts, uint32_t nblocks, uint32_t NB, uint32_t G, uint32_t* scratch, size_t scratch_words,
+                         uint32_t* before, uint32_t* totals);
 size_t sgr_test_scan_tmp_words(size_t n);
 int sgr_test_wave_sum(const float* in, float* out_dpp, float* out_shfl, int nwaves, void* stream);
 int sgr_test_lds_atomic_order(const uint32_t* pattern, uint32_t* out, int trials, void* stream);
diff --git a/street_gaussians_amd/_native.py b/street_gaussians_amd/_native.py
--- a/street_gaussians_amd/_native.py
+++ b/street_gaussians_amd/_native.py
@@ -46,6 +46,11 @@
         "sgr_test_sort": (i, [vp, vp, vp, vp, u32, i, vp, vp, vp]),
         "sgr_test_sort32": (i, [vp, vp, vp, vp, u32, i, i, vp, vp, vp]),
         "sgr_test_sort_hist_words": (sz, [u32]),
+        "sgr_test_sort_fold": (i, [i]),
+        "sgr_test_scan_fold": (i, [i]),
+        "sgr_test_sort_ex": (i, [i, vp, vp, vp, vp, u32, i, i, i, vp, vp, i, vp, vp, vp]),
+        "sgr_test_fold_layout": (i, [u32, u32, u32, u32, vp]),
+        "sgr_test_fold_replay": (i, [vp, u32, u32, u32, vp, sz, vp, vp]),
         "sgr_test_scan_tmp_words": (sz, [sz]),
         "sgr_test_wave_sum": (i, [vp, vp, vp, i, vp]),
         "sgr_test_exact_math": (i, [i, vp, vp, vp, vp, vp, vp, vp, vp]),
diff --git a/street_gaussians_amd/csrc/sgr_api.hip b/street_gaussians_amd/csrc/sgr_api.hip
--- a/street_gaussians_amd/csrc/sgr_api.hip
+++ b/street_gaussians_amd/csrc/sgr_api.hip
@@ -7,6 +7,7 @@
 #include <mutex>
 #include <string>
 #include <thread>
+#include <vector>
 
 #include "../../include/sgr.h"
 #include "../../include/sgr_layers.h"
@@ -457,6 +458,7 @@
         prof_end(stream);
         return 0;
     };
+    const bool raw_sums = sgr_scan_head_folds((size_t)P);
     const auto depth_sort_scan = [&]() -> int {
         prof_begin(1, stream);
         order = nullptr;
@@ -468,7 +470,7 @@
             scanned = gv.aux_sorted;
         }
         sgr_launch_scan_head(reinterpret_cast<const uint32_t*>(scanned), reinterpret_cast<const uint32_t*>(gv.aux), (size_t)P,
-                             aux16 ? 4 : 2, gv.scan_tmp, gv.sub_sums, stream, 2);
+                             aux16 ? 4 : 2, gv.scan_tmp, gv.sub_sums, stream, 2, raw_sums);
         SGR_STAGE("depth_sort+scan");
         prof_end(stream);
         return 0;
@@ -530,7 +532,7 @@
     prof_begin(2, stream);
     SgrGeomView gv_dup = gv;
     if (sw.tile_sort) gv_dup.aux_sorted = const_cast<uint2*>(aux_emit);
-    sgr_launch_duplicate(P, gv_dup, order, gv.scan_tmp, gv.sub_sums, bv.keys[0], f.key16, bv.vals[0], g.gx, cap, aux16, stream);
+    sgr_launch_duplicate(P, gv_dup, order, gv.scan_tmp, gv.sub_sums, bv.keys[0], f.key16, bv.vals[0], g.gx, cap, aux16, raw_sums, stream);
     SGR_STAGE("duplicate");
     prof_end(stream);
     if (R > 0) {
@@ -1127,6 +1129,83 @@
     return cur;
 }
 size_t sgr_test_sort_hist_words(uint32_t n) { return sgr_sort_hist_words(n ? n : 1); }
+int sgr_test_sort_fold(int g) { return sgr_sort_set_fold(g); }
+int sgr_test_scan_fold(int on) { return sgr_scan_set_fold(on); }
+int sgr_test_sort_ex(int key_bytes, void* keys0, void* keys1, uint32_t* vals0, uint32_t* vals1, uint32_t n, int end_bit,
+                     int max_bits, int iota, const void* aux_in, void* aux_out, int aux16, const uint32_t* dev_n, uint32_t* hist,
+                     void* stream_) {
+    if (max_bits != 8 && max_bits != 9) return sgr_set_error(SGR_E_INVALID, "sgr_test_sort_ex: max_bits must be 8 or 9");
+    if (key_bytes != 2 && key_bytes != 4) return sgr_set_error(SGR_E_INVALID, "sgr_test_sort_ex: key_bytes must be 2 or 4");
+    if (key_bytes == 2 && (iota || aux_in || dev_n || max_bits != 8))
+        return sgr_set_error(SGR_E_INVALID, "sgr_test_sort_ex: 16-bit keys sort plain pairs with 8-bit digits");
+    if ((aux_in == nullptr) != (aux_out == nullptr)) return sgr_set_error(SGR_E_INVALID, "sgr_test_sort_ex: aux_in and aux_out go together");
+    hipStream_t stream = (hipStream_t)stream_;
+    const int debug = 1;
+    uint32_t* vals[2] = {vals0, vals1};
+    int cur;
+    if (key_bytes == 2) {
+        uint16_t* keys[2] = {(uint16_t*)keys0, (uint16_t*)keys1};
+        cur = sgr_launch_sort_pairs16(keys, vals, n, end_bit, hist, nullptr, stream);
+    } else {
+        uint32_t* keys[2] = {(uint32_t*)keys0, (uint32_t*)keys1};
+        cur = sgr_launch_sort_pairs32(keys, vals, n, end_bit, hist, nullptr, stream, iota != 0, (const uint2*)aux_in, (uint2*)aux_out,
+                                      max_bits, aux16, dev_n);
+    }
+    SGR_STAGE("sort_ex");
+    if (const int rc = sort_gave_up(n, hist, stream)) return rc;
+    return cur;
+}
+int sgr_test_fold_layout(uint32_t n, uint32_t items, uint32_t NB, uint32_t G, uint64_t* out) {
+    if (!items || !NB || !G || !out) return sgr_set_error(SGR_E_INVALID, "sgr_test_fold_layout: zero argument");
+    const uint32_t nblocks = sgr_fold_nblocks(n, items), ngroups = sgr_fold_ngroups(nblocks, G);
+    out[0] = nblocks;
+    out[1] = ngroups;
+    out[2] = nblocks ? sgr_fold_group(nblocks - 1, G) : 0;
+    out[3] = nblocks ? sgr_fold_table_off(NB - 1, nblocks - 1, nblocks) : 0;
+    out[4] = sgr_fold_gsum_off(0, 0, nblocks, NB);
+    out[5] = ngroups ? sgr_fold_gsum_off(ngroups - 1, NB - 1, nblocks, NB) : 0;
+    out[6] = sgr_fold_words(nblocks, G, NB);
+    out[7] = sgr_sort_hist_words(n ? n : 1);
+    return 0;
+}
+int sgr_test_fold_replay(const uint32_t* counts, uint32_t nblocks, uint32_t NB, uint32_t G, uint32_t* scratch, size_t scratch_words,
+                         uint32_t* before, uint32_t* totals) {
+    if (!counts || !scratch || !before || !totals || !NB || !G) return sgr_set_error(SGR_E_INVALID, "sgr_test_fold_replay: null argument");
+    const uint32_t ngroups = sgr_fold_ngroups(nblocks, G);
+    std::vector<uint32_t> run(NB);
+    for (uint32_t g = 0; g < ngroups; g++) {
+        std::fill(run.begin(), run.end(), 0u);
+        for (uint32_t b = g * G; b < nblocks && b < (g + 1) * G; b++) {
+            if (sgr_fold_group(b, G) != g) return sgr_set_error(SGR_E_INVALID, "sgr_test_fold_replay: block outside its group");
+            for (uint32_t d = 0; d < NB; d++) {
+                const size_t o = sgr_fold_table_off(d, b, nblocks);
+                if (o >= scratch_words) return sgr_set_error(SGR_E_INVALID, "sgr_test_fold_replay: table offset outside the scratch");
+                scratch[o] = run[d];
+                run[d] += counts[(size_t)b * NB + d];
+            }
+        }
+        for (uint32_t d = 0; d < NB; d++) {
+            const size_t o = sgr_fold_gsum_off(g, d, nblocks, NB);
+            if (o >= scratch_words) return sgr_set_error(SGR_E_INVALID, "sgr_test_fold_replay: group-sum offset outside the scratch");
+            scratch[o] = run[d];
+        }
+    }
+    for (uint32_t b = 0; b < nblocks; b++) {
+        const uint32_t mine = sgr_fold_group(b, G);
+        for (uint32_t d = 0; d < NB; d++) {
+            uint32_t fb = 0, ft = 0;
+            for (uint32_t g = 0; g < ngroups; g++) {
+                const uint32_t v = scratch[sgr_fold_gsum_off(g, d, nblocks, NB)];
+                ft += v;
+                if (g < mine) fb += v;
+            }
+            before[(size_t)b * NB + d] = scratch[sgr_fold_table_off(d, b, nblocks)] + fb;
+            if (b == 0) totals[d] = ft;
+            else if (totals[d] != ft) return sgr_set_error(SGR_E_INVALID, "sgr_test_fold_replay: blocks disagree on a total");
+        }
+    }
+    return 0;
+}
 size_t sgr_test_scan_tmp_words(size_t n) { return sgr_scan_tmp_count(n ? n : 1); }
 __global__ void sgr_exact_math_test_kernel(int n, const float* x, float* exp_lib, float* exp_ref, const float* a,
                                            const float* b, float* div_lib, float* div_ref) {
diff --git a/street_gaussians_amd/csrc/sgr_common.h b/street_gaussians_amd/csrc/sgr_common.h
--- a/street_gaussians_amd/csrc/sgr_common.h
+++ b/street_gaussians_amd/csrc/sgr_common.h
@@ -88,7 +88,23 @@
 static inline size_t sgr_scan_tmp_count(size_t n) { return (n + SGR_SCAN_ITEMS - 1) / SGR_SCAN_ITEMS + 1; }
 #define SGR_SORT_CTRL_WORDS (SGR_SORT_MAX_PASS * 256 + 64)
 static inline size_t sgr_sort_hist_words(size_t n) {
-    return (size_t)SGR_SORT_CTRL_WORDS + (size_t)512 * ((n + SGR_SORT_ITEMS - 1) / SGR_SORT_ITEMS);
+    return (size_t)SGR_SORT_CTRL_WORDS + (size_t)1024 * ((n + SGR_SORT_ITEMS - 1) / SGR_SORT_ITEMS);
+}
+
+#ifdef __HIPCC__
+#define SGR_HD __host__ __device__ __forceinline__
+#else
+#define SGR_HD inline
+#endif
+SGR_HD uint32_t sgr_fold_nblocks(uint32_t n, uint32_t items) { return n / items + (n % items ? 1u : 0u); }
+SGR_HD uint32_t sgr_fold_group(uint32_t block, uint32_t G) { return block / G; }
+SGR_HD uint32_t sgr_fold_ngroups(uint32_t nblocks, uint32_t G) { return nblocks / G + (nblocks % G ? 1u : 0u); }
+SGR_HD size_t sgr_fold_table_off(uint32_t bin, uint32_t block, uint32_t nblocks) { return (size_t)bin * nblocks + block; }
+SGR_HD size_t sgr_fold_gsum_off(uint32_t group, uint32_t bin, uint32_t nblocks, uint32_t NB) {
+    return (size_t)NB * nblocks + (size_t)group * NB + bin;
+}
+SGR_HD size_t sgr_fold_words(uint32_t nblocks, uint32_t G, uint32_t NB) {
+    return (size_t)NB * nblocks + (size_t)sgr_fold_ngroups(nblocks, G) * NB;
 }
 
 static inline SgrGeomView sgr_geom_carve(char* base, size_t P, char** end = nullptr) {
@@ -185,7 +201,11 @@
                      uint32_t* total_out = nullptr, const uint32_t* gather = nullptr, int in_stride = 1,
                      const uint32_t* in2 = nullptr, uint32_t* out2 = nullptr);
 void sgr_launch_scan_head(const uint32_t* in, const uint32_t* in2, size_t n, int in_stride, uint32_t* tmp, uint32_t* sub,
-                          hipStream_t s, int in2_stride = 0);
+                          hipStream_t s, int in2_stride = 0,
+                          bool raw_sums = false);
+bool sgr_scan_head_folds(size_t n);
+int sgr_sort_set_fold(int g);
+int sgr_scan_set_fold(int on);
 int sgr_sort_get_one_sweep();
 void sgr_sort_set_one_sweep(int on);
 int sgr_launch_sort_pairs(uint64_t* const keys[2], uint32_t* const vals[2], uint32_t n, int end_bit, uint32_t* hist,
diff --git a/street_gaussians_amd/csrc/sgr_launch.h b/street_gaussians_amd/csrc/sgr_launch.h
--- a/street_gaussians_amd/csrc/sgr_launch.h
+++ b/street_gaussians_amd/csrc/sgr_launch.h
@@ -20,7 +20,7 @@
 void sgr_launch_filter(int P, const float* means3D, const float* scales, const float* rotations, const float* cov3D_precomp,
                        const SgrCamArgs& ca, const SgrGeomView& gv, int* radii, float* means2D, int prefiltered, hipStream_t s);
 void sgr_launch_duplicate(int P, const SgrGeomView& gv, const uint32_t* order, const uint32_t* bsum, const uint32_t* sub, void* keys,
-                          int key16, uint32_t* vals, int gx, uint32_t cap, int marks, hipStream_t s);
+                          int key16, uint32_t* vals, int gx, uint32_t cap, int marks, bool raw_sums, hipStream_t s);
 void sgr_launch_tile_ranges(int L, const void* keys, int key16, uint2* ranges, uint8_t* touched, uint32_t T, hipStream_t s);
 void sgr_launch_tile_order(const uint2* ranges, int T, int force, hipStream_t s);
 void sgr_launch_compose_keys(int L, const void* tile_keys, int key16, const uint32_t* point_list, const float4* rec, uint64_t* out,
diff --git a/street_gaussians_amd/csrc/sgr_preprocess.hip b/street_gaussians_amd/csrc/sgr_preprocess.hip
--- a/street_gaussians_amd/csrc/sgr_preprocess.hip
+++ b/street_gaussians_amd/csrc/sgr_preprocess.hip
@@ -263,12 +263,12 @@
 }
 
 static_assert(SGR_PRE_THREADS == 256 && SGR_SCAN_ITEMS == 8 * SGR_PRE_THREADS, "one workgroup = one sub-block of the scan");
-template <typename K>
+template <typename K, bool RAW>
 __global__ void __launch_bounds__(SGR_PRE_THREADS)
 sgr_duplicate_kernel(int P, SgrGeomView gv, const uint32_t* __restrict__ order, const uint32_t* __restrict__ bsum,
                      const uint32_t* __restrict__ sub, uint32_t nb, K* __restrict__ keys, uint32_t* __restrict__ vals,
                      int gx, uint32_t cap, int marks) {
-    if (cap != 0) {
+    if (!RAW && cap != 0) {
         const uint32_t R = bsum[nb];
         for (uint32_t s = R + blockIdx.x * SGR_PRE_THREADS + threadIdx.x; s < cap; s += gridDim.x * SGR_PRE_THREADS) {
             keys[s] = (K)~(K)0;
@@ -296,8 +296,39 @@
     }
     const uint32_t t2 = (i < P) ? gv.aux[i].x : 0u;
     uint32_t total;
-    const uint32_t ex1 = sgr_block_excl_scan256(as.x, lds4, total) + bsum[blockIdx.x >> 3] + sub[blockIdx.x];
-    const uint32_t ex2 = sgr_block_excl_scan256(t2, lds4, total) + bsum[nb + 1 + (blockIdx.x >> 3)] + sub[8 * nb + blockIdx.x];
+    uint32_t ex1, ex2;
+    if constexpr (RAW) {
+        __shared__ uint32_t red[4][3];
+        const uint32_t mine = blockIdx.x >> 3;
+        uint32_t s1 = 0, s2 = 0, t1 = 0;
+#pragma unroll 2
+        for (uint32_t j = threadIdx.x; j < nb; j += SGR_PRE_THREADS) {
+            const uint32_t v1 = bsum[j], v2 = bsum[nb + 1 + j];
+            t1 += v1;
+            s1 += j < mine ? v1 : 0u;
+            s2 += j < mine ? v2 : 0u;
+        }
+#pragma unroll
+        for (int d = 32; d >= 1; d >>= 1) {
+            s1 += __shfl_xor(s1, d, 64);
+            s2 += __shfl_xor(s2, d, 64);
+            t1 += __shfl_xor(t1, d, 64);
+        }
+        if (lane == 0) { red[wave][0] = s1; red[wave][1] = s2; red[wave][2] = t1; }
+        ex1 = sgr_block_excl_scan256(as.x, lds4, total);
+        const uint32_t R = red[0][2] + red[1][2] + red[2][2] + red[3][2];
+        ex1 += red[0][0] + red[1][0] + red[2][0] + red[3][0] + sub[blockIdx.x];
+        ex2 = sgr_block_excl_scan256(t2, lds4, total) + red[0][1] + red[1][1] + red[2][1] + red[3][1] + sub[8 * nb + blockIdx.x];
+        if (cap != 0) {
+            for (uint32_t s = R + blockIdx.x * SGR_PRE_THREADS + threadIdx.x; s < cap; s += gridDim.x * SGR_PRE_THREADS) {
+                keys[s] = (K)~(K)0;
+                vals[s] = 0u;
+            }
+        }
+    } else {
+        ex1 = sgr_block_excl_scan256(as.x, lds4, total) + bsum[blockIdx.x >> 3] + sub[blockIdx.x];
+        ex2 = sgr_block_excl_scan256(t2, lds4, total) + bsum[nb + 1 + (blockIdx.x >> 3)] + sub[8 * nb + blockIdx.x];
+    }
     if (i < P) {
         gv.u0[i] = ex2;
         idx = order ? order[i] : (uint32_t)i;
@@ -481,12 +512,15 @@
 }
 
 void sgr_launch_duplicate(int P, const SgrGeomView& gv, const uint32_t* order, const uint32_t* bsum, const uint32_t* sub,
-                          void* keys, int key16, uint32_t* vals, int gx, uint32_t cap, int marks, hipStream_t s) {
+                          void* keys, int key16, uint32_t* vals, int gx, uint32_t cap, int marks, bool raw_sums, hipStream_t s) {
     if (P <= 0) return;
     const uint32_t nb = (uint32_t)(((size_t)P + SGR_SCAN_ITEMS - 1) / SGR_SCAN_ITEMS);
     const unsigned grid = (P + SGR_PRE_THREADS - 1) / SGR_PRE_THREADS;
-    if (key16) sgr_duplicate_kernel<uint16_t><<<grid, SGR_PRE_THREADS, 0, s>>>(P, gv, order, bsum, sub, nb, (uint16_t*)keys, vals, gx, cap, marks);
-    else sgr_duplicate_kernel<uint32_t><<<grid, SGR_PRE_THREADS, 0, s>>>(P, gv, order, bsum, sub, nb, (uint32_t*)keys, vals, gx, cap, marks);
+    if (raw_sums) {
+        if (key16) sgr_duplicate_kernel<uint16_t, true><<<grid, SGR_PRE_THREADS, 0, s>>>(P, gv, order, bsum, sub, nb, (uint16_t*)keys, vals, gx, cap, marks);
+        else sgr_duplicate_kernel<uint32_t, true><<<grid, SGR_PRE_THREADS, 0, s>>>(P, gv, order, bsum, sub, nb, (uint32_t*)keys, vals, gx, cap, marks);
+    } else if (key16) sgr_duplicate_kernel<uint16_t, false><<<grid, SGR_PRE_THREADS, 0, s>>>(P, gv, order, bsum, sub, nb, (uint16_t*)keys, vals, gx, cap, marks);
+    else sgr_duplicate_kernel<uint32_t, false><<<grid, SGR_PRE_THREADS, 0, s>>>(P, gv, order, bsum, sub, nb, (uint32_t*)keys, vals, gx, cap, marks);
 }
 
 void sgr_launch_tile_ranges(int L, const void* keys, int key16, uint2* ranges, uint8_t* touched, uint32_t T, hipStream_t s) {
diff --git a/street_gaussians_amd/csrc/sgr_scan_sort.hip b/street_gaussians_amd/csrc/sgr_scan_sort.hip
--- a/street_gaussians_amd/csrc/sgr_scan_sort.hip
+++ b/street_gaussians_amd/csrc/sgr_scan_sort.hip
@@ -85,12 +85,32 @@
 }
 
 void sgr_launch_scan_head(const uint32_t* in, const uint32_t* in2, size_t n, int in_stride, uint32_t* tmp, uint32_t* sub,
-                          hipStream_t s, int in2_stride) {
+                          hipStream_t s, int in2_stride, bool raw_sums) {
     if (in2_stride <= 0) in2_stride = in_stride;
     if (n == 0) return;
     const size_t nb = (n + SGR_SCAN_ITEMS - 1) / SGR_SCAN_ITEMS;
     sgr_scan_reduce_kernel<<<(unsigned)nb * 2u, 256, 0, s>>>(in, n, tmp, nullptr, in_stride, in2, (unsigned)nb, sub, in2_stride);
-    sgr_scan_spine_kernel<<<2, 256, 0, s>>>(tmp, nb, nullptr);
+    if (!raw_sums) sgr_scan_spine_kernel<<<2, 256, 0, s>>>(tmp, nb, nullptr);
+}
+
+static std::atomic<int> g_scan_fold{-3};
+static int scan_fold_mode() {
+    int v = g_scan_fold.load(std::memory_order_relaxed);
+    if (v == -3) {
+        const char* e = getenv("SGR_SCAN_FOLD");
+        v = (e && *e) ? (atoi(e) > 0 ? 1 : atoi(e) == 0 ? 0 : -1) : -1;
+        g_scan_fold.store(v, std::memory_order_relaxed);
+    }
+    return v;
+}
+int sgr_scan_set_fold(int on) {
+    const int prev = scan_fold_mode();
+    if (on >= -1) g_scan_fold.store(on > 0 ? 1 : on, std::memory_order_relaxed);
+    return prev;
+}
+bool sgr_scan_head_folds(size_t n) {
+    (void)n;
+    return scan_fold_mode() > 0;
 }
 
 template <typename K, int IPT>
@@ -156,20 +176,98 @@
     if (threadIdx.x == 0) totals[blockIdx.x] = carry;
 }
 
+template <typename K, int IPT, int TEAMS, int TS>
+__global__ void __launch_bounds__(TS * TEAMS)
+sgr_sort_hist_group_kernel(const K* __restrict__ keys, uint32_t n, int shift, uint32_t mask, uint32_t nblocks, uint32_t G,
+                           uint32_t* __restrict__ hist) {
+    constexpr int T = TS * TEAMS;
+    constexpr int BPT = (512 + T - 1) / T;
+    constexpr int WPT = TS / 64;
+    constexpr int KPT = 256 * IPT / TS;
+    __shared__ uint32_t h[TEAMS][WPT][512];
+    const uint32_t NB = mask + 1u;
+    const int team = threadIdx.x / TS, t = threadIdx.x % TS, wave = t >> 6;
+    const uint32_t group = blockIdx.x;
+    const uint32_t b0 = group * G, bend = min(b0 + G, nblocks);
+    constexpr int V = 16 / (int)sizeof(K);
+    constexpr int NV = KPT / V;
+    static_assert(KPT % V == 0 && TS % 64 == 0, "keys per thread must be a multiple of the vector width");
+    struct alignas(16) Vec { K k[V]; };
+    const auto load = [&](Vec (&v)[NV], uint32_t rb) {
+        const uint32_t block = rb + team;
+        if (block >= bend) return;
+        const uint32_t base = block * (256u * IPT);
+#pragma unroll
+        for (int s = 0; s < NV; s++) {
+            const uint32_t i = base + (s * TS + t) * V;
+            if (i + V <= n) v[s] = *reinterpret_cast<const Vec*>(keys + i);
+            else {
+#pragma unroll
+                for (int e = 0; e < V; e++) v[s].k[e] = i + e < n ? keys[i + e] : (K)0;
+            }
+        }
+    };
+    Vec cur[NV], nxt[NV];
+    load(cur, b0);
+    for (int d = t; d < WPT * 512; d += TS) (&h[team][0][0])[d] = 0;
+    uint32_t run[BPT];
+#pragma unroll
+    for (int j = 0; j < BPT; j++) run[j] = 0u;
+    __syncthreads();
+    for (uint32_t rb = b0; rb < bend; rb += TEAMS) {
+        if (rb + TEAMS < bend) load(nxt, rb + TEAMS);
+        const uint32_t block = rb + team;
+        if (block < bend) {
+            const uint32_t base = block * (256u * IPT);
+#pragma unroll
+            for (int s = 0; s < NV; s++) {
+                const uint32_t i = base + (s * TS + t) * V;
+#pragma unroll
+                for (int e = 0; e < V; e++)
+                    if (i + e < n) atomicAdd(&h[team][wave][(uint32_t)(cur[s].k[e] >> shift) & mask], 1u);
+            }
+        }
+        __syncthreads();
+#pragma unroll
+        for (int j = 0; j < BPT; j++) {
+            const uint32_t d = threadIdx.x + j * T;
+            if (d < NB) {
+#pragma unroll
+                for (int tm = 0; tm < TEAMS; tm++) {
+                    if (rb + tm < bend) {
+                        hist[sgr_fold_table_off(d, rb + tm, nblocks)] = run[j];
+#pragma unroll
+                        for (int w = 0; w < WPT; w++) { run[j] += h[tm][w][d]; h[tm][w][d] = 0; }
+                    }
+                }
+            }
+        }
+        __syncthreads();
+#pragma unroll
+        for (int s = 0; s < NV; s++) cur[s] = nxt[s];
+    }
+#pragma unroll
+    for (int j = 0; j < BPT; j++) {
+        const uint32_t d = threadIdx.x + j * T;
+        if (d < NB) hist[sgr_fold_gsum_off(group, d, nblocks, NB)] = run[j];
+    }
+}
+
 #define SGR_OS_AGG (1ull << 48)
 #define SGR_OS_PREFIX (2ull << 48)
 #define SGR_OS_VALUE ((1ull << 48) - 1ull)
-template <typename K, int BITS, int IPT, bool ONE>
+template <typename K, int BITS, int IPT, bool ONE, bool FOLD = false>
 __global__ void __launch_bounds__(256)
 sgr_sort_scatter_kernel(const K* __restrict__ kin, const uint32_t* __restrict__ vin, K* __restrict__ kout,
                         uint32_t* __restrict__ vout, uint32_t n, int shift, uint32_t nblocks,
                         const uint32_t* __restrict__ hist_scanned, const uint32_t* __restrict__ totals,
                         unsigned long long* __restrict__ status, uint32_t* __restrict__ ticket, uint32_t* __restrict__ err,
                         uint32_t pass_tag, const uint2* __restrict__ aux_in, uint2* __restrict__ aux_out, int aux16,
-                        const uint32_t* __restrict__ dev_n) {
+                        const uint32_t* __restrict__ dev_n, uint32_t G = 0u) {
     constexpr int NB = 1 << BITS;
     constexpr int BPT = NB > 256 ? NB / 256 : 1;
     static_assert(!(ONE && NB > 256), "the one-sweep form has one status word per thread");
+    static_assert(!(ONE && FOLD), "the one-sweep form has no tables to fold");
     constexpr uint32_t ITEMS = 256u * IPT;
     __shared__ uint32_t cnt[4][NB];
     __shared__ uint32_t lstart[NB];
@@ -177,6 +275,7 @@
     __shared__ uint32_t lds4[4];
     __shared__ K sK[ITEMS];
     __shared__ uint32_t sV[ITEMS];
+    __shared__ uint32_t fold_before[FOLD ? NB : 1], fold_total[FOLD ? NB : 1];
     const int tid = threadIdx.x, lane = tid & 63, wave = tid >> 6;
     if (!ONE && dev_n) {
         n = min(n, *dev_n);
@@ -186,6 +285,7 @@
     for (int b = tid; b < NB; b += 256) {
 #pragma unroll
         for (int w = 0; w < 4; w++) cnt[w][b] = 0;
+        if constexpr (FOLD) { fold_before[b] = 0; fold_total[b] = 0; }
     }
     __syncthreads();
     const uint32_t block = ONE ? lds4[0] : blockIdx.x;
@@ -197,7 +297,24 @@
         for (int j = 0; j < BPL; j++) {
             const int bin = lane * BPL + j;
             pre_before[j] = bin < NB ? hist_scanned[(size_t)bin * nblocks + block] : 0u;
-            pre_total[j] = bin < NB ? totals[bin] : 0u;
+            pre_total[j] = (!FOLD && bin < NB) ? totals[bin] : 0u;
+        }
+    }
+
+    constexpr int FB = !FOLD ? 1 : BPL >= 8 ? 8 : 16;
+    struct alignas(4 * BPL) FoldRow { uint32_t v[BPL]; };
+    FoldRow frow[FB];
+    uint32_t fold_ngroups = 0u, fold_mine = 0u;
+    const FoldRow* fold_rows = nullptr;
+    const bool fold_lane = lane * BPL < NB;
+    if constexpr (FOLD) {
+        fold_ngroups = sgr_fold_ngroups(nblocks, G);
+        fold_mine = sgr_fold_group(block, G);
+        fold_rows = reinterpret_cast<const FoldRow*>(totals + lane * BPL);
+#pragma unroll
+        for (int k = 0; k < FB; k++) {
+            const uint32_t g = wave + 4 * k;
+            frow[k] = (fold_lane && g < fold_ngroups) ? fold_rows[(size_t)g * (NB / BPL)] : FoldRow{};
         }
     }
 
@@ -231,6 +348,37 @@
         rnk[s] = prev + prefix;
         __builtin_amdgcn_wave_barrier();
     }
+    if constexpr (FOLD) {
+        uint32_t fb[BPL], ft[BPL];
+#pragma unroll
+        for (int j = 0; j < BPL; j++) { fb[j] = 0u; ft[j] = 0u; }
+        for (uint32_t g0 = wave;;) {
+#pragma unroll
+            for (int k = 0; k < FB; k++) {
+                const uint32_t g = g0 + 4 * k;
+#pragma unroll
+                for (int j = 0; j < BPL; j++) {
+                    ft[j] += frow[k].v[j];
+                    fb[j] += g < fold_mine ? frow[k].v[j] : 0u;
+                }
+            }
+            g0 += 4 * FB;
+            if (g0 >= fold_ngroups) break;
+#pragma unroll
+            for (int k = 0; k < FB; k++) {
+                const uint32_t g = g0 + 4 * k;
+                frow[k] = (fold_lane && g < fold_ngroups) ? fold_rows[(size_t)g * (NB / BPL)] : FoldRow{};
+            }
+        }
+#pragma unroll
+        for (int j = 0; j < BPL; j++) {
+            const int bin = lane * BPL + j;
+            if (bin < NB) {
+                if (ft[j]) atomicAdd(&fold_total[bin], ft[j]);
+                if (fb[j]) atomicAdd(&fold_before[bin], fb[j]);
+            }
+        }
+    }
     __syncthreads();
     if constexpr (!ONE) {
         if (wave == 0) {
@@ -241,6 +389,9 @@
                 const int bin = lane * BPL + j;
 #pragma unroll
                 for (int w = 0; w < 4; w++) c[j][w] = bin < NB ? cnt[w][bin] : 0u;
+                if constexpr (FOLD) {
+                    if (bin < NB) { pre_before[j] += fold_before[bin]; pre_total[j] = fold_total[bin]; }
+                }
                 tot[j] = c[j][0] + c[j][1] + c[j][2] + c[j][3];
                 sum_t += tot[j];
                 sum_g += pre_total[j];
@@ -421,14 +572,49 @@
     if (key_bytes == 2) return n >= 500000u ? 16 : 8;
     return n >= 3000000u ? 16 : 8;
 }
+#define SGR_FOLD_TEAMS 8
+#define SGR_FOLD_TEAM_THREADS 128
+static std::atomic<int> g_sort_fold{-3};
+static int sort_fold_mode() {
+    int v = g_sort_fold.load(std::memory_order_relaxed);
+    if (v == -3) {
+        const char* e = getenv("SGR_SORT_FOLD");
+        v = (e && *e) ? atoi(e) : -1;
+        if (v < -1) v = -1;
+        g_sort_fold.store(v, std::memory_order_relaxed);
+    }
+    return v;
+}
+int sgr_sort_set_fold(int g) {
+    const int prev = sort_fold_mode();
+    if (g >= -1) g_sort_fold.store(g, std::memory_order_relaxed);
+    return prev;
+}
+static inline uint32_t sort_fold_g(uint32_t n, size_t key_bytes, bool dev_n) {
+    if (key_bytes > 4 || dev_n) return 0u;
+    const int m = sort_fold_mode();
+    (void)n;
+    return m > 0 ? (uint32_t)m : 0u;
+}
 
 int sgr_sort_pass_count(int end_bit) { return (end_bit + 7) / 8; }
 
 template <typename K, int BITS, int IPT>
 static void sort_pass(const K* kin, const uint32_t* vin, K* kout, uint32_t* vout, uint32_t n, int shift, uint32_t* hist,
-                      const uint2* aux_in, uint2* aux_out, int aux16, hipStream_t s, const uint32_t* dev_n) {
-    const uint32_t nblocks = (n + 256u * IPT - 1) / (256u * IPT);
+                      const uint2* aux_in, uint2* aux_out, int aux16, hipStream_t s, const uint32_t* dev_n, uint32_t G) {
+    const uint32_t nblocks = sgr_fold_nblocks(n, 256u * IPT);
     constexpr int NB = 1 << BITS;
+    if constexpr (sizeof(K) <= 4) {
+        if (G != 0u && dev_n == nullptr) {
+            sgr_sort_hist_group_kernel<K, IPT, SGR_FOLD_TEAMS, SGR_FOLD_TEAM_THREADS>
+                <<<sgr_fold_ngroups(nblocks, G), SGR_FOLD_TEAM_THREADS * SGR_FOLD_TEAMS, 0, s>>>(
+                kin, n, shift, (uint32_t)(NB - 1), nblocks, G, hist);
+            sgr_sort_scatter_kernel<K, BITS, IPT, false, true><<<nblocks, 256, 0, s>>>(
+                kin, vin, kout, vout, n, shift, nblocks, hist, hist + sgr_fold_gsum_off(0u, 0u, nblocks, NB), nullptr, nullptr,
+                nullptr, 0u, aux_in, aux_out, aux16, nullptr, G);
+            return;
+        }
+    }
     sgr_sort_hist_kernel<K, IPT><<<nblocks, 256, 0, s>>>(kin, n, shift, (uint32_t)(NB - 1), nblocks, hist, dev_n);
     uint32_t* totals = hist + (size_t)NB * nblocks;
     sgr_sort_rowscan_kernel<<<NB, 256, 0, s>>>(hist, nblocks, totals);
@@ -467,13 +653,14 @@
     const int bits = sizeof(K) == 8 ? 8 : sort_pass_bits(end_bit, max_bits);
     const int ipt = sizeof(K) == 8 ? 8 : sort_ipt(n, sizeof(K));
     if (sizeof(K) <= 4) npass = sort_passes(end_bit, max_bits);
+    const uint32_t G = sort_fold_g(n, sizeof(K), dev_n != nullptr);
     for (int p = 0; p < npass; p++) {
         const uint32_t* vin = (iota && p == 0) ? nullptr : vals[cur];
         const bool last = p == npass - 1;
         const uint2* ai = last ? aux_in : nullptr;
         uint2* ao = last ? aux_out : nullptr;
         const int shift = bits * p;
-#define SGR_PASS(B, I) sort_pass<K, B, I>(keys[cur], vin, keys[cur ^ 1], vals[cur ^ 1], n, shift, hist, ai, ao, aux16, s, dev_n)
+#define SGR_PASS(B, I) sort_pass<K, B, I>(keys[cur], vin, keys[cur ^ 1], vals[cur ^ 1], n, shift, hist, ai, ao, aux16, s, dev_n, G)
         if constexpr (sizeof(K) == 8) { SGR_PASS(8, 8); }
         else if (ipt == 16 && bits <= 8) {
             if (bits <= 5) SGR_PASS(5, 16); else if (bits == 6) SGR_PASS(6, 16); else if (bits == 7) SGR_PASS(7, 16); else SGR_PASS(8, 16);
```

Result: slower. 652.6 (-1.1%).
